# YuePanEdward/MULLS

Hardware: AMD Instinct MI355X
Metric: scan-pair registrations/sec (64-beam ~120k pts, 20 ICP iters); dT vs ref (higher is better)
Workload: dtype f32

## Files before the change

include/mulls_hip.h:

```cpp
#ifndef MULLS_HIP_H
#define MULLS_HIP_H

#include <stddef.h>
#include <stdint.h>

#ifdef __cplusplus
extern "C" {
#endif

#define MULLS_NCLASS 6
#define MULLS_POINT_BYTES 48

enum mulls_class
{
	MULLS_GROUND = 0,
	MULLS_PILLAR = 1,
	MULLS_FACADE = 2,
	MULLS_BEAM = 3,
	MULLS_ROOF = 4,
	MULLS_VERTEX = 5
};

enum mulls_error
{
	MULLS_OK = 0,
	MULLS_E_INVALID = -100,
	MULLS_E_HIP = -101,
	MULLS_E_NO_DEVICE = -102,
	MULLS_E_UNSUPPORTED = -103,
	MULLS_E_IO = -104,
	MULLS_E_NOMEM = -105
};

typedef struct mulls_cloud
{
	const void *pts;
	uint32_t n;
	uint32_t stride;
} mulls_cloud;

typedef struct mulls_pair
{
	mulls_cloud tgt[MULLS_NCLASS];
	mulls_cloud src[MULLS_NCLASS];
	mulls_cloud src_down[MULLS_NCLASS];
	double tgt_bound[6];
	double init_guess[16];
} mulls_pair;

typedef struct mulls_params
{
	int32_t max_iter_num;
	float dis_thre_unit;
	float converge_translation;
	float converge_rotation_d;
	float dis_thre_min;
	float dis_thre_update_rate;
	char used_feature_type[8];
	char weight_strategy[8];
	float z_xy_balanced_ratio;
	float pt2pt_residual_window;
	float pt2pl_residual_window;
	float pt2li_residual_window;
	uint8_t apply_intersection_filter;
	uint8_t apply_motion_undistortion;
	uint8_t normal_shooting_on;
	uint8_t use_more_points;
	float normal_bearing;
	uint8_t keep_less_source_points;
	uint8_t faithful;
	uint8_t rejector_strict;
	uint8_t reserved_;
	float sigma_thre;
	float min_neccessary_corr_ratio;
	float max_bearable_rotation_d;
	uint64_t rng_seed;
} mulls_params;

typedef struct mulls_iter_trace
{
	int32_t iter;
	uint32_t ncorr[MULLS_NCLASS];
	uint32_t nsrc[MULLS_NCLASS];
	float thr[MULLS_NCLASS];
	double atpa[36];
	double atpb[6];
	double x[6];
} mulls_iter_trace;

typedef struct mulls_result
{
	int32_t code;
	int32_t iters;
	double T[16];
	double info[36];
	float sigma;
	float confidence;
	uint32_t ncorr[MULLS_NCLASS];
	uint32_t nsrc0[MULLS_NCLASS];
	uint32_t ntgt0[MULLS_NCLASS];
	int32_t singular;
	int32_t cropped;
	double crop_box[6];
	float ms_total;
	mulls_iter_trace *trace;
	int32_t trace_cap;
	int32_t trace_len;
} mulls_result;

typedef struct mulls_profile
{
	double ms_setup;
	double ms_nn;
	double ms_filter;
	double ms_accum;
	double ms_residual;
	int32_t launches_nn;
	int32_t iterations;
	uint64_t nn_pair_evals;
	uint64_t nn_src_pts;
	uint64_t nn_tgt_pts;
	double ms_host_step;
	double ms_host_wait;
	double ms_host_launch;
	uint64_t nn_tgt_unique;
	uint64_t nn_corr_pts;
	double icp_fused_ms[6];
	double icp_search_ms[24];
	double icp_phase_ms[6];
	double ms_stage;
	double ms_stage_pack;
	uint64_t stage_bytes;
} mulls_profile;

typedef struct mulls_ctx mulls_ctx;
typedef struct mulls_batch mulls_batch;

void mulls_default_params(mulls_params *p);

int mulls_create(int device, mulls_ctx **out);
void mulls_destroy(mulls_ctx *ctx);
const char *mulls_last_error(const mulls_ctx *ctx);
int mulls_set_profiling(mulls_ctx *ctx, int on);
int mulls_get_profile(const mulls_ctx *ctx, mulls_profile *out);
int mulls_set_nn_mode(mulls_ctx *ctx, int mode);
enum mulls_option
{
	MULLS_OPT_HOST_STEP = 0,
	MULLS_OPT_FEW_LAUNCHES_MAX_PAIRS = 3,
	MULLS_OPT_SUBBATCHES = 4,
	MULLS_OPT_TWO_STREAMS = 5,
	MULLS_OPT_CERTIFICATES = 6,
	MULLS_OPT_CERT_SLACK_MIN = 7,
	MULLS_OPT_CERT_SLACK_MAX = 8,
	MULLS_OPT_CERT_SLACK_RATE = 9,
	MULLS_OPT_LDS_DEDUP = 10,
	MULLS_OPT_GRID_H0 = 11,
	MULLS_OPT_BM_H0 = 12,
	MULLS_OPT_LEAN_STAGING = 13,
	MULLS_OPT_DEBUG_STOP = 14,
	MULLS_OPT_DEBUG_TICK = 15,
	MULLS_OPT_SPLIT_MIN_PAIRS = 16,
	MULLS_OPT_SPLIT_MAX_PAIRS = 17,
	MULLS_OPT_FUSED_TGT_SETUP = 18,
	MULLS_OPT_STAGGER = 19,
	MULLS_OPT_STEP_LAUNCH_MAX_PAIRS = 20,
	MULLS_OPT_MIXED_TIERS = 21,
	MULLS_OPT_BIG_EARLY_SETS = 22,
	MULLS_OPT_KCERT = 23,
	MULLS_OPT_KCERT_MIN = 24,
	MULLS_OPT_ACCUM_WAVE_MIN_TRIPS = 25,
	MULLS_OPT_FIRST_DIRECT = 26,
	MULLS_OPT_SUM_STEP = 27,
	MULLS_OPT_COUNT = 28
};
int mulls_set_option(mulls_ctx *ctx, int option, double value);
int mulls_get_option(const mulls_ctx *ctx, int option, double *value);
void *mulls_stream(mulls_ctx *ctx);

int mulls_icp(mulls_ctx *ctx, const mulls_pair *pair, const mulls_params *params, mulls_result *result);

int mulls_icp_batch(mulls_ctx *ctx, const mulls_pair *pairs, int n, const mulls_params *params, mulls_result *results);

int mulls_icp_batch_sharded(mulls_ctx *const *ctxs, int n_ctx, const mulls_pair *pairs, int n, const mulls_params *params, mulls_result *results);

typedef struct mulls_pipe mulls_pipe;
int mulls_pipe_create(int device, int depth, mulls_pipe **out);
void mulls_pipe_destroy(mulls_pipe *pipe);
int mulls_pipe_depth(const mulls_pipe *pipe);
mulls_ctx *mulls_pipe_ctx(mulls_pipe *pipe, int lane);
int mulls_pipe_set_option(mulls_pipe *pipe, int option, double value);
int mulls_icp_batch_begin(mulls_pipe *pipe, const mulls_pair *pairs, int n, const mulls_params *params, mulls_result *results);
int mulls_icp_batch_end(mulls_pipe *pipe, int ticket);

void mulls_pack_results(const mulls_result *results, int n, double *table);

int mulls_batch_create(mulls_ctx *ctx, const mulls_pair *pairs, int n, mulls_batch **out);
int mulls_batch_run(mulls_ctx *ctx, mulls_batch *batch, const mulls_params *params, mulls_result *results);
void mulls_batch_destroy(mulls_ctx *ctx, mulls_batch *batch);


int mulls_icp_3dof_ground(mulls_ctx *ctx, const mulls_pair *pair, const mulls_params *params, mulls_result *result);
int mulls_icp_3dof_ground_batch(mulls_ctx *ctx, const mulls_pair *pairs, int n, const mulls_params *params, mulls_result *results);

int mulls_icp_4dof_global(mulls_ctx *ctx, const mulls_pair *pair, float heading_step_d, const double station[3], int max_iter_num,
						  float dis_thre_unit, float converge_translation, float converge_rotation_d, float dis_thre_min,
						  float dis_thre_update_rate, float max_bearable_rotation_d, mulls_result *result, int *success,
						  float *best_heading_d);

typedef struct mulls_map mulls_map;

typedef struct mulls_map_params
{
	float local_map_radius;
	int max_num_pts;
	int kept_vertex_num;
	float last_frame_reliable_radius;
	int map_based_dynamic_removal_on;
	char used_feature_type[8];
	float dynamic_removal_center_radius;
	float dynamic_dist_thre_min;
	float dynamic_dist_thre_max;
	float near_dist_thre;
	int recalculate_feature_on;
	uint64_t rng_seed;
	int tree_mode;
	char tree_used[8];
	double tree_box[6];
} mulls_map_params;

typedef struct mulls_map_report
{
	uint32_t n[6];
	uint32_t frame_n[6];
	int feature_point_num;
	int dynamic_removal_ran;
	double local_bound[6];
	double bound[6];
	float ms_total;
} mulls_map_report;

void mulls_map_default_params(mulls_map_params *p);
int mulls_map_create(mulls_ctx *ctx, mulls_map **out);
void mulls_map_destroy(mulls_ctx *ctx, mulls_map *map);
int mulls_map_set(mulls_ctx *ctx, mulls_map *map, const mulls_cloud clouds[6], const double pose_lo[16]);
int mulls_map_update(mulls_ctx *ctx, mulls_map *map, const mulls_cloud frame_down[6], const double frame_pose_lo[16],
					 const mulls_map_params *params, mulls_map_report *report);
int mulls_map_cloud(mulls_ctx *ctx, const mulls_map *map, int cls, mulls_cloud *out);
int mulls_map_pose(mulls_ctx *ctx, const mulls_map *map, double pose_lo[16]);
int mulls_map_download(mulls_ctx *ctx, const mulls_map *map, int cls, void *pts, uint32_t cap, uint32_t *n);
int mulls_map_frame_download(mulls_ctx *ctx, const mulls_map *map, int cls, void *pts, uint32_t cap, uint32_t *n);

int mulls_io_read_kitti_bin(const char *path, void *pts, uint32_t cap, uint32_t *n);
int mulls_io_read_pcd(const char *path, void *pts, uint32_t cap, uint32_t *n);
int mulls_io_write_pcd(const char *path, const void *pts, uint32_t n, uint32_t stride, int as_binary);
int mulls_io_write_pose(const char *path, const double T[16], int append);


typedef struct mulls_ground_params
{
	int32_t min_grid_pt_num;
	float grid_resolution;
	float max_height_difference;
	float neighbor_height_diff;
	float max_ground_height;
	int32_t ground_random_down_rate;
	int32_t ground_random_down_down_rate;
	int32_t nonground_random_down_rate;
	int32_t reliable_neighbor_grid_num_thre;
	int32_t estimate_ground_normal_method;
	int32_t distance_weight_downsampling_method;
	float standard_distance;
	uint8_t fixed_num_downsampling;
	uint8_t apply_grid_wise_outlier_filter;
	uint8_t reserved_[2];
	int32_t down_ground_fixed_num;
	float intensity_thre;
	float outlier_std_scale;
	float normal_estimation_radius;
	uint32_t reserved2_;
	uint64_t rng_seed;
} mulls_ground_params;

void mulls_ground_default_params(mulls_ground_params *p);

int mulls_ground_filter(mulls_ctx *ctx, const void *pts, uint32_t n, uint32_t stride, const mulls_ground_params *params, void *ground, uint32_t cap_ground,
						void *ground_down, uint32_t cap_ground_down, void *unground, uint32_t cap_unground, uint32_t n_out[3]);


typedef struct mulls_classify_params
{
	float neighbor_searching_radius;
	int32_t neighbor_k;
	int32_t neigh_k_min;
	int32_t pca_down_rate;
	float edge_thre, planar_thre;
	float edge_thre_down, planar_thre_down;
	int32_t extract_vertex_points_method;
	float curvature_thre;
	float vertex_curvature_non_max_radius;
	float linear_vertical_sin_high_thre, linear_vertical_sin_low_thre;
	float planar_vertical_sin_high_thre, planar_vertical_sin_low_thre;
	uint8_t fixed_num_downsampling;
	uint8_t sharpen_with_nms;
	uint8_t use_distance_adaptive_pca;
	uint8_t reserved_;
	int32_t pillar_down_fixed_num, facade_down_fixed_num, beam_down_fixed_num, roof_down_fixed_num, unground_down_fixed_num;
	float beam_height_max, roof_height_min;
	float feature_pts_ratio_guess;
	uint64_t rng_seed;
} mulls_classify_params;

void mulls_classify_default_params(mulls_classify_params *p);

enum mulls_classify_cloud
{
	MULLS_CL_PILLAR = 0,
	MULLS_CL_BEAM = 1,
	MULLS_CL_FACADE = 2,
	MULLS_CL_ROOF = 3,
	MULLS_CL_PILLAR_DOWN = 4,
	MULLS_CL_BEAM_DOWN = 5,
	MULLS_CL_FACADE_DOWN = 6,
	MULLS_CL_ROOF_DOWN = 7,
	MULLS_CL_VERTEX = 8,
	MULLS_CL_COUNT = 9
};
// ... 67 lines not shown
```

mulls_amd/abi.py:

```python
import ctypes as C

import numpy as np

NCLASS = 6
POINT_BYTES = 48
GROUND, PILLAR, FACADE, BEAM, ROOF, VERTEX = range(6)
CLASS_NAMES = ("ground", "pillar", "facade", "beam", "roof", "vertex")

MULLS_OK = 0
MULLS_E_INVALID = -100
MULLS_E_HIP = -101
MULLS_E_NO_DEVICE = -102
MULLS_E_UNSUPPORTED = -103
MULLS_E_IO = -104
MULLS_E_NOMEM = -105

(OPT_HOST_STEP, _OPT_RESERVED_1, _OPT_RESERVED_2, OPT_FEW_LAUNCHES_MAX_PAIRS, OPT_SUBBATCHES, OPT_TWO_STREAMS, OPT_CERTIFICATES, OPT_CERT_SLACK_MIN,
 OPT_CERT_SLACK_MAX, OPT_CERT_SLACK_RATE, OPT_LDS_DEDUP, OPT_GRID_H0, OPT_BM_H0, OPT_LEAN_STAGING, OPT_DEBUG_STOP, OPT_DEBUG_TICK, OPT_SPLIT_MIN_PAIRS, OPT_SPLIT_MAX_PAIRS,
 OPT_FUSED_TGT_SETUP, OPT_STAGGER, OPT_STEP_LAUNCH_MAX_PAIRS, OPT_MIXED_TIERS, OPT_BIG_EARLY_SETS, OPT_KCERT, OPT_KCERT_MIN, OPT_ACCUM_WAVE_MIN_TRIPS, OPT_FIRST_DIRECT, OPT_SUM_STEP, OPT_COUNT) = range(29)

POINT_DTYPE = np.dtype(
    {
        "names": ["x", "y", "z", "nx", "ny", "nz", "intensity", "curvature"],
        "formats": [np.float32] * 8,
        "offsets": [0, 4, 8, 16, 20, 24, 32, 36],
        "itemsize": POINT_BYTES,
    }
)


class Cloud(C.Structure):
    _fields_ = [("pts", C.c_void_p), ("n", C.c_uint32), ("stride", C.c_uint32)]


class Pair(C.Structure):
    _fields_ = [
        ("tgt", Cloud * NCLASS),
        ("src", Cloud * NCLASS),
        ("src_down", Cloud * NCLASS),
        ("tgt_bound", C.c_double * 6),
        ("init_guess", C.c_double * 16),
    ]


class Params(C.Structure):
    _fields_ = [
        ("max_iter_num", C.c_int32),
        ("dis_thre_unit", C.c_float),
        ("converge_translation", C.c_float),
        ("converge_rotation_d", C.c_float),
        ("dis_thre_min", C.c_float),
        ("dis_thre_update_rate", C.c_float),
        ("used_feature_type", C.c_char * 8),
        ("weight_strategy", C.c_char * 8),
        ("z_xy_balanced_ratio", C.c_float),
        ("pt2pt_residual_window", C.c_float),
        ("pt2pl_residual_window", C.c_float),
        ("pt2li_residual_window", C.c_float),
        ("apply_intersection_filter", C.c_uint8),
        ("apply_motion_undistortion", C.c_uint8),
        ("normal_shooting_on", C.c_uint8),
        ("use_more_points", C.c_uint8),
        ("normal_bearing", C.c_float),
        ("keep_less_source_points", C.c_uint8),
        ("faithful", C.c_uint8),
        ("rejector_strict", C.c_uint8),
        ("reserved_", C.c_uint8),
        ("sigma_thre", C.c_float),
        ("min_neccessary_corr_ratio", C.c_float),
        ("max_bearable_rotation_d", C.c_float),
        ("rng_seed", C.c_uint64),
    ]


class IterTrace(C.Structure):
    _fields_ = [
        ("iter", C.c_int32),
        ("ncorr", C.c_uint32 * NCLASS),
        ("nsrc", C.c_uint32 * NCLASS),
        ("thr", C.c_float * NCLASS),
        ("atpa", C.c_double * 36),
        ("atpb", C.c_double * 6),
        ("x", C.c_double * 6),
    ]


class Result(C.Structure):
    _fields_ = [
        ("code", C.c_int32),
        ("iters", C.c_int32),
        ("T", C.c_double * 16),
        ("info", C.c_double * 36),
        ("sigma", C.c_float),
        ("confidence", C.c_float),
        ("ncorr", C.c_uint32 * NCLASS),
        ("nsrc0", C.c_uint32 * NCLASS),
        ("ntgt0", C.c_uint32 * NCLASS),
        ("singular", C.c_int32),
        ("cropped", C.c_int32),
        ("crop_box", C.c_double * 6),
        ("ms_total", C.c_float),
        ("trace", C.POINTER(IterTrace)),
        ("trace_cap", C.c_int32),
        ("trace_len", C.c_int32),
    ]

    def T_matrix(self):
        return np.array(self.T[:], dtype=np.float64).reshape(4, 4).T.copy()

    def info_matrix(self):
        return np.array(self.info[:], dtype=np.float64).reshape(6, 6).T.copy()



class MapParams(C.Structure):
    _fields_ = [
        ("local_map_radius", C.c_float),
        ("max_num_pts", C.c_int32),
        ("kept_vertex_num", C.c_int32),
        ("last_frame_reliable_radius", C.c_float),
        ("map_based_dynamic_removal_on", C.c_int32),
        ("used_feature_type", C.c_char * 8),
        ("dynamic_removal_center_radius", C.c_float),
        ("dynamic_dist_thre_min", C.c_float),
        ("dynamic_dist_thre_max", C.c_float),
        ("near_dist_thre", C.c_float),
        ("recalculate_feature_on", C.c_int32),
        ("rng_seed", C.c_uint64),
        ("tree_mode", C.c_int32),
        ("tree_used", C.c_char * 8),
        ("tree_box", C.c_double * 6),
    ]


class MapReport(C.Structure):
    _fields_ = [
        ("n", C.c_uint32 * NCLASS),
        ("frame_n", C.c_uint32 * NCLASS),
        ("feature_point_num", C.c_int32),
        ("dynamic_removal_ran", C.c_int32),
        ("local_bound", C.c_double * 6),
        ("bound", C.c_double * 6),
        ("ms_total", C.c_float),
    ]


def map_params(**kw):
    p = MapParams()
    p.local_map_radius, p.max_num_pts, p.kept_vertex_num, p.last_frame_reliable_radius = 80.0, 20000, 800, 60.0
    p.map_based_dynamic_removal_on = 0
    p.used_feature_type = b"111110"
    p.dynamic_removal_center_radius, p.dynamic_dist_thre_min, p.dynamic_dist_thre_max, p.near_dist_thre = 30.0, 0.3, 3.0, 0.03
    p.recalculate_feature_on, p.rng_seed, p.tree_mode, p.tree_used = 0, 0, 0, b"000000"
    for k, v in kw.items():
        if k == "tree_box":
            for i in range(6):
                p.tree_box[i] = float(v[i])
        elif k in ("used_feature_type", "tree_used"):
            setattr(p, k, v.encode() if isinstance(v, str) else v)
        else:
            setattr(p, k, v)
    return p


def colmajor16(M):
    return (C.c_double * 16)(*np.asarray(M, dtype=np.float64).T.reshape(-1))

class GroundParams(C.Structure):
    _fields_ = [
        ("min_grid_pt_num", C.c_int32),
        ("grid_resolution", C.c_float),
        ("max_height_difference", C.c_float),
# ... 312 lines not shown
```

mulls_amd/csrc/accum.h:

```cpp
#pragma once
#include "device_util.h"

namespace
{
__device__ __forceinline__ float w_dist_adaptive(float dist, int iter_num)
{
	const float unit_dist = 30.0f, b_min = 0.7f, b_max = 1.3f, b_step = 0.05f;
	float t = b_min + b_step * iter_num;
	float b_current = (t < b_max) ? t : b_max;
	float temp = (float)(b_current + (1.0 - b_current) * dist / unit_dist);
	temp = (float)((temp > 0.01) ? (double)temp : 0.01);
	return temp;
}
__device__ __forceinline__ float w_intensity(float i1, float i2)
{
	float ratio = fabsf(i1 - i2) / 255.0f;
	return (float)exp(-1.0 * ratio);
}
__device__ __forceinline__ float w_residual(float res, float thre)
{
	return (res > thre) ? ((2 * res * thre + (1 * 1 - 2 * 1) * (thre * thre)) / res / res) : 1.0f;
}
__device__ __forceinline__ int metric_of(int cls) { return (cls == 1 || cls == 3) ? 1 : (cls == 5 ? 2 : 0); }
}
// ... 165 lines not shown
			ACC(1, 3.0);
		}
		return;
	}

	if (metric == 0)
	{
		float ntx = N.x, nty = N.y, ntz = N.z;
		float a = ntz * py - nty * pz;
		float b = ntx * pz - ntz * px;
		float c = nty * px - ntx * py;
		float dd = ntx * qx + nty * qy + ntz * qz - ntx * px - nty * py - ntz * pz;
		const float w = wpre ? *wpre : corr_weight(A, 0, P, Q, N, wi);
		wdg = w;
		ACC(0, w * ntx * ntx);
		ACC(1, w * ntx * nty);
		ACC(2, w * ntx * ntz);
		ACC(3, w * a * ntx);
		ACC(4, w * b * ntx);
		ACC(5, w * c * ntx);
		ACC(6, w * nty * nty);
		ACC(7, w * nty * ntz);
		ACC(8, w * a * nty);
		ACC(9, w * b * nty);
		ACC(10, w * c * nty);
		ACC(11, w * ntz * ntz);
		ACC(12, w * a * ntz);
		ACC(13, w * b * ntz);
		ACC(14, w * c * ntz);
		ACC(15, w * a * a);
		ACC(16, w * a * b);
		ACC(17, w * a * c);
		ACC(18, w * b * b);
		ACC(19, w * b * c);
		ACC(20, w * c * c);
		ACC(21, w * dd * ntx);
		ACC(22, w * dd * nty);
		ACC(23, w * dd * ntz);
		ACC(24, w * dd * a);
		ACC(25, w * dd * b);
		ACC(26, w * dd * c);
	}
	else if (metric == 1)
	{
		const float wx = wpre ? *wpre : corr_weight(A, 1, P, Q, N, wi);
		float vx = N.x, vy = N.y, vz = N.z;
		float dx = px - qx, dy = py - qy, dz = pz - qz;
		double A[3][6], bv[3];
		A[0][0] = 0;
		A[0][1] = -vz;
		A[0][2] = vy;
		A[0][3] = vy * py + vz * pz;
		A[0][4] = -vy * px;
		A[0][5] = -vz * px;
		A[1][0] = vz;
		A[1][1] = 0;
		A[1][2] = -vx;
		A[1][3] = -vx * py;
		A[1][4] = vz * pz + vx * px;
		A[1][5] = -vz * py;
		A[2][0] = -vy;
		A[2][1] = vx;
		A[2][2] = 0;
		A[2][3] = -vx * pz;
		A[2][4] = -vy * pz;
		A[2][5] = vx * px + vy * py;
		bv[0] = -vy * dz + vz * dy;
		bv[1] = -vz * dx + vx * dz;
		bv[2] = -vx * dy + vy * dx;
		wdg = wx;
		const double sw = (double)sqrtf(wx);
		for (int r = 0; r < 3; r++)
		{
			for (int c = 0; c < 6; c++)
				A[r][c] = sw * A[r][c];
			bv[r] = sw * bv[r];
		}
		int k = 0;
#pragma unroll
		for (int j = 0; j < 6; j++)
#pragma unroll
			for (int c = j; c < 6; c++)
				{
					ACC(k, (A[0][j] * A[0][c] + A[1][j] * A[1][c]) + A[2][j] * A[2][c]);
					k++;
				}
#pragma unroll
		for (int j = 0; j < 6; j++)
			ACC(21 + j, (A[0][j] * bv[0] + A[1][j] * bv[1]) + A[2][j] * bv[2]);
	}
	else
	{
		float dx = px - qx, dy = py - qy, dz = pz - qz;
		const float wx = wpre ? *wpre : corr_weight(A, 2, P, Q, N, wi);
		const float wy = wx, wz = wx;
		if (!faithful)
			wdg = wx;
		ACC(0, wx);
		ACC(4, wx * pz);
		ACC(5, (-wx * py));
		ACC(6, wy);
		ACC(8, (-wy * pz));
		ACC(10, wy * px);
		ACC(11, wz);
		ACC(12, wz * py);
		ACC(13, (-wz * px));
		ACC(15, wy * pz * pz + wz * py * py);
		ACC(16, (-wz * px * py));
		ACC(17, (-wy * px * pz));
		ACC(18, wx * pz * pz + wz * px * px);
		ACC(19, (-wx * py * pz));
		ACC(20, wx * py * py + wy * px * px);
		ACC(21, (-wx * dx));
		ACC(22, (-wy * dy));
		ACC(23, (-wz * dz));
		ACC(24, wy * pz * dy - wz * py * dz);
		ACC(25, wz * px * dz - wx * pz * dx);
		ACC(26, wx * py * dx - wy * px * dy);
	}
}
#undef ACC

#define MULLS_ACC_LANES 1024
#define MULLS_RED_BYTES ((size_t)27 * MULLS_ACC_LANES * sizeof(float))
#define MULLS_RED_BYTES_HALF ((size_t)14 * MULLS_ACC_LANES * sizeof(float))

namespace
{
template <int CTRL>
__device__ __forceinline__ double dpp_add_f64(double v)
{
	const unsigned long long b = (unsigned long long)__double_as_longlong(v);
	const uint32_t lo = (uint32_t)__builtin_amdgcn_update_dpp(0, (int)(uint32_t)b, CTRL, 0xf, 0xf, false);
	const uint32_t hi = (uint32_t)__builtin_amdgcn_update_dpp(0, (int)(uint32_t)(b >> 32), CTRL, 0xf, 0xf, false);
	return v + __longlong_as_double((long long)(((unsigned long long)hi << 32) | lo));
}
template <int CTRL, int ROWS>
__device__ __forceinline__ double dpp_add_f64_rows(double v)
{
	const unsigned long long b = (unsigned long long)__double_as_longlong(v);
	const uint32_t lo = (uint32_t)__builtin_amdgcn_update_dpp(0, (int)(uint32_t)b, CTRL, ROWS, 0xf, false);
	const uint32_t hi = (uint32_t)__builtin_amdgcn_update_dpp(0, (int)(uint32_t)(b >> 32), CTRL, ROWS, 0xf, false);
	return v + __longlong_as_double((long long)(((unsigned long long)hi << 32) | lo));
}
__device__ __forceinline__ double readlane_f64(double v, int lane)
{
	const unsigned long long b = (unsigned long long)__double_as_longlong(v);
	const uint32_t lo = (uint32_t)__builtin_amdgcn_readlane((int)(uint32_t)b, lane);
	const uint32_t hi = (uint32_t)__builtin_amdgcn_readlane((int)(uint32_t)(b >> 32), lane);
	return __longlong_as_double((long long)(((unsigned long long)hi << 32) | lo));
}
}

template <typename TS, int T0, int NT, int MODE = 0, int LANES = MULLS_ACC_LANES>
__device__ __forceinline__ void slot_terms(const AccumCtx &A, const double *x, bool valid, const float4 P, const float4 Q, const float4 N, float wi, float &wdg, TS *R)
{
	static_assert(sizeof(TS) * NT * LANES <= MULLS_RED_BYTES, "the term buffer holds NT terms of LANES slots");
	TS t[NT];
#pragma unroll
	for (int k = 0; k < NT; k++)
		t[k] = (TS)0;
	if (valid)
		point_terms<TS, T0, NT, MODE>(A, x, P, Q, N, wi, wdg, t);
#pragma unroll
	for (int k = 0; k < NT; k++)
		R[k * LANES + threadIdx.x] = t[k];
}
template <typename TS, int T0, int NT, int MODE = 0, int LANES = MULLS_ACC_LANES>
__device__ __forceinline__ void reduce_terms(const TS *R, double *part)
{
	const int lane = threadIdx.x & 63, wave = threadIdx.x >> 6;
#pragma unroll
	for (int k0 = 0; k0 < NT; k0 += LANES / 64)
	{
		const int k = k0 + wave;
		if (k < NT)
		{
			const TS *r = R + k * LANES;
			double sum = (double)r[lane];
#pragma unroll
			for (int i = 1; i < LANES / 64; i++)
				sum += (double)r[lane + 64 * i];
			sum = dpp_add_f64<0xB1>(sum);
			sum = dpp_add_f64<0x4E>(sum);
			sum = dpp_add_f64<0x141>(sum);
			sum = dpp_add_f64<0x140>(sum);
			const double r0 = readlane_f64(sum, 0), r1 = readlane_f64(sum, 16), r2 = readlane_f64(sum, 32), r3 = readlane_f64(sum, 48);
			if (lane == 0)
				part[MODE == 1 ? li_term(T0 + k) : T0 + k] = (r0 + r1) + (r2 + r3);
		}
	}
}

template <bool HALF = false, int LANES = MULLS_ACC_LANES>
__device__ __forceinline__ void trip_sum_regs(const AccumCtx &A, const double *x, bool valid, const float4 P, const float4 Q, const float4 N, float &wdg, void *R,
											   double *part)
{
	const float wi = (valid && A.inten_w && !A.residual_pass) ? point_wi(P, Q) : 1.0f;
	if (A.residual_pass)
	{
		__syncthreads();
		slot_terms<double, 0, 2, 0, LANES>(A, x, valid, P, Q, N, wi, wdg, static_cast<double *>(R));
		__syncthreads();
		reduce_terms<double, 0, 2, 0, LANES>(static_cast<const double *>(R), part);
		if (threadIdx.x >= 2 && threadIdx.x < MULLS_NTERM)
			part[threadIdx.x] = 0.0;
	}
	else if (A.li_diag)
	{
		__syncthreads();
		if (threadIdx.x < 21 && li_slot((int)threadIdx.x) < 0)
			part[threadIdx.x] = 0.0;
		if (HALF)
		{
			slot_terms<double, 0, 6, 1, LANES>(A, x, valid, P, Q, N, wi, wdg, static_cast<double *>(R));
			__syncthreads();
			reduce_terms<double, 0, 6, 1, LANES>(static_cast<const double *>(R), part);
			__syncthreads();
			slot_terms<double, 6, 6, 1, LANES>(A, x, valid, P, Q, N, wi, wdg, static_cast<double *>(R));
			__syncthreads();
			reduce_terms<double, 6, 6, 1, LANES>(static_cast<const double *>(R), part);
		}
		else
		{
			slot_terms<double, 0, 12, 1, LANES>(A, x, valid, P, Q, N, wi, wdg, static_cast<double *>(R));
			__syncthreads();
			reduce_terms<double, 0, 12, 1, LANES>(static_cast<const double *>(R), part);
		}
	}
	else if (A.metric == 1 && HALF)
	{
		__syncthreads();
		slot_terms<double, 0, 7, 0, LANES>(A, x, valid, P, Q, N, wi, wdg, static_cast<double *>(R));
		__syncthreads();
		reduce_terms<double, 0, 7, 0, LANES>(static_cast<const double *>(R), part);
		__syncthreads();
		slot_terms<double, 7, 7, 0, LANES>(A, x, valid, P, Q, N, wi, wdg, static_cast<double *>(R));
		__syncthreads();
		reduce_terms<double, 7, 7, 0, LANES>(static_cast<const double *>(R), part);
		__syncthreads();
		slot_terms<double, 14, 7, 0, LANES>(A, x, valid, P, Q, N, wi, wdg, static_cast<double *>(R));
		__syncthreads();
		reduce_terms<double, 14, 7, 0, LANES>(static_cast<const double *>(R), part);
		__syncthreads();
		slot_terms<double, 21, 6, 0, LANES>(A, x, valid, P, Q, N, wi, wdg, static_cast<double *>(R));
		__syncthreads();
		reduce_terms<double, 21, 6, 0, LANES>(static_cast<const double *>(R), part);
	}
	else if (A.metric == 1)
	{
		__syncthreads();
		slot_terms<double, 0, 13, 0, LANES>(A, x, valid, P, Q, N, wi, wdg, static_cast<double *>(R));
		__syncthreads();
		reduce_terms<double, 0, 13, 0, LANES>(static_cast<const double *>(R), part);
		__syncthreads();
		slot_terms<double, 13, 13, 0, LANES>(A, x, valid, P, Q, N, wi, wdg, static_cast<double *>(R));
		__syncthreads();
		reduce_terms<double, 13, 13, 0, LANES>(static_cast<const double *>(R), part);
		__syncthreads();
		slot_terms<double, 26, 1, 0, LANES>(A, x, valid, P, Q, N, wi, wdg, static_cast<double *>(R));
		__syncthreads();
		reduce_terms<double, 26, 1, 0, LANES>(static_cast<const double *>(R), part);
	}
	else if (HALF)
	{
		__syncthreads();
		slot_terms<float, 0, 14, 0, LANES>(A, x, valid, P, Q, N, wi, wdg, static_cast<float *>(R));
		__syncthreads();
		reduce_terms<float, 0, 14, 0, LANES>(static_cast<const float *>(R), part);
		__syncthreads();
		slot_terms<float, 14, 13, 0, LANES>(A, x, valid, P, Q, N, wi, wdg, static_cast<float *>(R));
		__syncthreads();
		reduce_terms<float, 14, 13, 0, LANES>(static_cast<const float *>(R), part);
	}
	else
	{
		__syncthreads();
		slot_terms<float, 0, 27, 0, LANES>(A, x, valid, P, Q, N, wi, wdg, static_cast<float *>(R));
		__syncthreads();
		reduce_terms<float, 0, 27, 0, LANES>(static_cast<const float *>(R), part);
	}
	__syncthreads();
}

template <bool HALF = false, int LANES = MULLS_ACC_LANES>
__device__ __forceinline__ void trip_sum(const AccumCtx &A, const double *x, const CloudDesc &d, uint32_t trip0, const float4 *__restrict__ spos,
										  const float4 *__restrict__ mq, const uint8_t *__restrict__ flag, float *__restrict__ wd, void *R, double *part)
{
	const uint32_t s = trip0 + threadIdx.x;
	bool valid = false;
	float4 P = make_float4(0.0f, 0.0f, 0.0f, 0.0f), Q = P, N = P;
	float w = 0.0f, w0 = 0.0f;
	uint32_t g = 0;
	if (s < d.src_n)
	{
		g = d.src_off + s;
		const uint32_t f = flag[g];
		P = spos[g], Q = mq[2u * g], N = mq[2u * g + 1u];
		w = w0 = wd[g];
		valid = (f & (MULLS_F_ALIVE | MULLS_F_VALID)) == (MULLS_F_ALIVE | MULLS_F_VALID);
	}
	trip_sum_regs<HALF, LANES>(A, x, valid, P, Q, N, w, R, part);
	if (valid && __float_as_uint(w) != __float_as_uint(w0))
		wd[g] = w;
}

// ... 45 lines not shown
```

mulls_amd/csrc/batch.cpp:

```cpp
#include "batch.h"

namespace mulls_drv
{
void rows12(const double colmajor[16], double out[12])
{
	for (int r = 0; r < 3; r++)
		for (int c = 0; c < 4; c++)
			out[r * 4 + c] = colmajor[r + 4 * c];
}


void fill_crop_box(const RunParams &rp, const double tgt_bound[6], const uint32_t keys[6], mulls_result &R)
{
	R.cropped = rp.crop ? 1 : 0;
	for (int k = 0; k < 3 && rp.crop; k++)
	{
		const uint32_t kmin = keys[k], kmax = keys[3 + k];
		const bool none = kmin == 0xffffffffu && kmax == 0u;
		const double mmin = none ? 1.7976931348623157e308 : (double)ord_to_float(kmin);
		const double mmax = none ? -1.7976931348623157e308 : (double)ord_to_float(kmax);
		const double b1min = tgt_bound[k], b1max = tgt_bound[3 + k];
		const float pad = 1.0f;
		R.crop_box[k] = ((b1min > mmin) ? b1min : mmin) - pad;
		R.crop_box[3 + k] = ((b1max < mmax) ? b1max : mmax) + pad;
	}
}

int check_params(mulls_ctx *ctx, const mulls_params *P)
{
	if (!P)
		return MULLS_E_INVALID;
	if (std::strlen(P->used_feature_type) < 6 || std::strlen(P->weight_strategy) < 4)
	{
		ctx->err = "used_feature_type needs 6 characters and weight_strategy 4";
		return MULLS_E_INVALID;
	}
	return MULLS_OK;
}

void init_cert(const mulls_ctx *ctx, RunParams &rp)
{
	rp.cert = ctx->opt[MULLS_OPT_CERTIFICATES] != 0.0 ? 1u : 0u;
	rp.cert_slack_min = (float)ctx->opt[MULLS_OPT_CERT_SLACK_MIN];
	rp.cert_slack_max = (float)ctx->opt[MULLS_OPT_CERT_SLACK_MAX];
	rp.cert_slack_rate = (float)ctx->opt[MULLS_OPT_CERT_SLACK_RATE];
	rp.kcert = rp.cert && ctx->opt[MULLS_OPT_KCERT] != 0.0 ? 1u : 0u;
	rp.kcert_min = (uint32_t)ctx->opt[MULLS_OPT_KCERT_MIN];
}

int subbatch_count(const mulls_ctx *ctx, int n)
{
	int nsub = n >= 2048 ? 2 : 1;
	if (ctx->opt[MULLS_OPT_SUBBATCHES] >= 1.0)
		nsub = std::max(1, std::min(2, (int)ctx->opt[MULLS_OPT_SUBBATCHES]));
	return n < 2 ? 1 : nsub;
}

bool option_value_ok(int option, double *value)
{
	const double v = *value;
	if (!(v == v) || v > 1.0e15 || v < -1.0e15)
		return false;
	switch (option)
	{
	case MULLS_OPT_STAGGER:
		if (v < 0.0 || v > 65536.0)
			return false;
		*value = (double)((uint64_t)v & ~(uint64_t)255);
		return true;
	case MULLS_OPT_GRID_H0:
	case MULLS_OPT_BM_H0:
		return v >= 0.0 && v <= 1.0e4;
	case MULLS_OPT_CERT_SLACK_MIN:
	case MULLS_OPT_CERT_SLACK_MAX:
		return v >= 0.0 && v <= 1.0e3;
	case MULLS_OPT_CERT_SLACK_RATE:
		return v >= 0.0 && v <= 1.0e3;
	case MULLS_OPT_DEBUG_TICK:
		return v >= 0.0 && v <= 4294967295.0;
	default:
		return v >= 0.0 && v <= 2147483647.0;
	}
}

}
int SegCopier::flush(hipStream_t st)
{
	using namespace mulls;
	size_t total = 0;
	for (const Pending &h : host)
		total += (h.bytes + 255u) & ~(size_t)255;
	bool direct = false;
	for (const Pending &h : host)
		direct = direct || (h.bytes & 3u) || ((uintptr_t)h.dst & 15u) || h.bytes > 0xfffffff0ull;
	for (const CopySeg &g : segs)
		direct = direct || (g.bytes & 3u) || (g.dst & 15ull) || (g.src & 15ull);
	if (direct)
	{
		for (const CopySeg &g : segs)
			HIPCHK(ctx, hipMemcpyAsync((void *)(uintptr_t)g.dst, (const void *)(uintptr_t)g.src, g.bytes, hipMemcpyDeviceToDevice, st));
		for (const Pending &h : host)
			HIPCHK(ctx, hipMemcpyAsync(h.dst, h.src, h.bytes, hipMemcpyHostToDevice, st));
		segs.clear(), host.clear();
		return MULLS_OK;
	}
	if (total > ctx->mail_cap)
	{
		HIPCHK(ctx, hipStreamSynchronize(st));
		if (ctx->mail_h)
			(void)hipHostFree(ctx->mail_h);
		ctx->mail_h = nullptr, ctx->mail_cap = 0;
		const size_t want = std::max<size_t>(total + total / 2, (size_t)1 << 20);
		HIPCHK(ctx, hipHostMalloc((void **)&ctx->mail_h, want, hipHostMallocMapped));
		ctx->mail_cap = want;
	}
	unsigned char *mail_d = nullptr;
	if (total)
		HIPCHK(ctx, hipHostGetDevicePointer((void **)&mail_d, ctx->mail_h, 0));
	size_t off = 0;
	for (const Pending &h : host)
	{
		std::memcpy(ctx->mail_h + off, h.src, h.bytes);
		segs.push_back({(unsigned long long)(uintptr_t)h.dst, (unsigned long long)(uintptr_t)(mail_d + off), (uint32_t)h.bytes, 0u});
		off += (h.bytes + 255u) & ~(size_t)255;
	}
	if (!segs.empty())
	{
		launch_copy_segs(st, segs.data(), (uint32_t)segs.size());
		HIPCHK(ctx, hipGetLastError());
	}
	segs.clear(), host.clear();
	return MULLS_OK;
}
namespace mulls_drv
{
void options_init(mulls_ctx *ctx)
{
	double *o = ctx->opt;
	o[MULLS_OPT_HOST_STEP] = 0, o[MULLS_OPT_FEW_LAUNCHES_MAX_PAIRS] = 640;
	o[MULLS_OPT_SUBBATCHES] = 0, o[MULLS_OPT_TWO_STREAMS] = 0, o[MULLS_OPT_CERTIFICATES] = 1;
	o[MULLS_OPT_CERT_SLACK_MIN] = 0.02, o[MULLS_OPT_CERT_SLACK_MAX] = 0.10, o[MULLS_OPT_CERT_SLACK_RATE] = 1.0;
	o[MULLS_OPT_SPLIT_MIN_PAIRS] = 96, o[MULLS_OPT_SPLIT_MAX_PAIRS] = 1 << 30, o[MULLS_OPT_FUSED_TGT_SETUP] = 1, o[MULLS_OPT_STAGGER] = 4352, o[MULLS_OPT_STEP_LAUNCH_MAX_PAIRS] = 640, o[MULLS_OPT_LDS_DEDUP] = 1, o[MULLS_OPT_GRID_H0] = 0, o[MULLS_OPT_BM_H0] = 0, o[MULLS_OPT_LEAN_STAGING] = 0, o[MULLS_OPT_DEBUG_STOP] = 0, o[MULLS_OPT_DEBUG_TICK] = 0, o[MULLS_OPT_MIXED_TIERS] = 1, o[MULLS_OPT_BIG_EARLY_SETS] = 5, o[MULLS_OPT_KCERT] = 1, o[MULLS_OPT_KCERT_MIN] = 64, o[MULLS_OPT_ACCUM_WAVE_MIN_TRIPS] = 768;
	o[MULLS_OPT_FIRST_DIRECT] = 1;
	o[MULLS_OPT_SUM_STEP] = 1;
	static const struct
	{
		const char *name;
		int opt;
	} env[] = {{"MULLS_HOST_STEP", MULLS_OPT_HOST_STEP}, {"MULLS_FEW_LAUNCHES_MAX_PAIRS", MULLS_OPT_FEW_LAUNCHES_MAX_PAIRS}, {"MULLS_SUBBATCHES", MULLS_OPT_SUBBATCHES}, {"MULLS_TWO_STREAMS", MULLS_OPT_TWO_STREAMS},
			   {"MULLS_CERTIFICATES", MULLS_OPT_CERTIFICATES}, {"MULLS_LDS_DEDUP", MULLS_OPT_LDS_DEDUP}, {"MULLS_GRID_H0", MULLS_OPT_GRID_H0}, {"MULLS_BM_H0", MULLS_OPT_BM_H0},
			   {"MULLS_LEAN_STAGING", MULLS_OPT_LEAN_STAGING}, {"MULLS_FUSED_TGT_SETUP", MULLS_OPT_FUSED_TGT_SETUP}, {"MULLS_STAGGER", MULLS_OPT_STAGGER}, {"MULLS_STEP_LAUNCH_MAX_PAIRS", MULLS_OPT_STEP_LAUNCH_MAX_PAIRS}, {"MULLS_SPLIT_MIN_PAIRS", MULLS_OPT_SPLIT_MIN_PAIRS}, {"MULLS_SPLIT_MAX_PAIRS", MULLS_OPT_SPLIT_MAX_PAIRS}, {"MULLS_DEBUG_STOP", MULLS_OPT_DEBUG_STOP}, {"MULLS_DEBUG_TICK", MULLS_OPT_DEBUG_TICK}, {"MULLS_MIXED_TIERS", MULLS_OPT_MIXED_TIERS}, {"MULLS_BIG_EARLY_SETS", MULLS_OPT_BIG_EARLY_SETS}, {"MULLS_KCERT", MULLS_OPT_KCERT}, {"MULLS_KCERT_MIN", MULLS_OPT_KCERT_MIN}, {"MULLS_ACCUM_WAVE_MIN_TRIPS", MULLS_OPT_ACCUM_WAVE_MIN_TRIPS}, {"MULLS_FIRST_DIRECT", MULLS_OPT_FIRST_DIRECT}, {"MULLS_SUM_STEP", MULLS_OPT_SUM_STEP}};
	for (const auto &e : env)
		if (const char *v = std::getenv(e.name))
		{
			double x = std::strtod(v, nullptr);
			if (option_value_ok(e.opt, &x))
				o[e.opt] = x;
		}
	if (std::getenv("MULLS_NO_CERT"))
		o[MULLS_OPT_CERTIFICATES] = 0;
	if (std::getenv("MULLS_NO_LDS_DEDUP"))
		o[MULLS_OPT_LDS_DEDUP] = 0;
	if (const char *e = std::getenv("MULLS_CERT_SLACK"))
	{
		float a = 0, b = 0, c = 0;
		if (std::sscanf(e, "%f,%f,%f", &a, &b, &c) == 3 && a >= 0.0f && b >= a && c >= 0.0f)
			o[MULLS_OPT_CERT_SLACK_MIN] = a, o[MULLS_OPT_CERT_SLACK_MAX] = b, o[MULLS_OPT_CERT_SLACK_RATE] = c;
	}
}

uint32_t lds_dedup_max_pts()
{
	const long room = 160L * 1024L - 64L - (long)MULLS_LDS_CELL_RESERVE - (long)MULLS_LDS_QCHUNK * 16L - (long)MULLS_LDS_AUX - 2L * (4096L + 8L);
	return (uint32_t)((room / 18L) & ~7L);
}

void assign_tiers(mulls_batch *B, const uint8_t used[MULLS_NC], int mode)
{
	B->lclouds_h.clear();
	B->tier_mode = mode;
	uint32_t n_used = 0;
	for (int c = 0; c < MULLS_NC; c++)
		n_used += used[c] ? 1u : 0u;
	const uint32_t s_max = lds_dedup_max_pts();
	for (int p = 0; p < B->n; p++)
	{
		uint64_t src_small = 0, src_big = 0;
		for (int c = 0; c < MULLS_NC && mode == 3; c++)
		{
			const CloudDesc &d = B->descs_h[(size_t)p * MULLS_NC + c];
			if (used[c])
				((d.tgt_n0 <= s_max && d.src_cap <= MULLS_SMALL_SRC_MAX) ? src_small : src_big) += d.src_cap;
		}
		const bool all_big = src_big >= 4u * src_small && src_big > 0;
		uint32_t rank = 0;
		for (int c = 0; c < MULLS_NC; c++)
		{
			CloudDesc &d = B->descs_h[(size_t)p * MULLS_NC + c];
			uint32_t t = (uint32_t)mode;
			if (mode == 3)
			{
				if (used[c])
					t = (d.tgt_n0 <= s_max && d.src_cap <= MULLS_SMALL_SRC_MAX && !all_big) ? MULLS_TIER_LDS : MULLS_TIER_BM;
				else
					t = d.tgt_n0 <= MULLS_LDS_MAXPTS ? MULLS_TIER_LDS : MULLS_TIER_BM;
			}
			d.tier = t;
			d.grid_slot = (uint32_t)p * n_used + rank;
			if (t == MULLS_TIER_BM)
			{
				d.grid_slot = used[c] ? (uint32_t)B->lclouds_h.size() : 0u;
				if (used[c])
					B->lclouds_h.push_back((uint32_t)p * MULLS_NC + (uint32_t)c);
			}
			rank += used[c] ? 1u : 0u;
		}
	}
}

void build_jobs(mulls_batch *B, const mulls_params *P, int nsub, int mode)
{
	std::string key(P->used_feature_type, 6);
	key += (char)('0' + nsub);
	key += (char)('a' + mode);
	if (key == B->jobs_key)
		return;
	uint8_t used[MULLS_NC];
	for (int c = 0; c < MULLS_NC; c++)
		used[c] = P->used_feature_type[c] == '1';
	assign_tiers(B, used, mode);
	B->nsub = nsub;
	B->jobs_h.clear();
	for (int p = 0; p < B->n; p++)
		for (int c = 0; c < MULLS_NC; c++)
		{
			CloudDesc &d = B->descs_h[p * MULLS_NC + c];
			d.job_begin = (uint32_t)B->jobs_h.size();
			if (P->used_feature_type[c] == '1')
				for (uint32_t s = 0; s < d.src_cap; s += MULLS_SRC_PER_BLOCK)
				{
					Job j = {(uint32_t)p, (uint32_t)c, s, 0};
					B->jobs_h.push_back(j);
				}
			d.job_end = (uint32_t)B->jobs_h.size();
		}
	B->cjobs_h.clear();
	for (int p = 0; p < B->n; p++)
		for (int c = 0; c < MULLS_NC; c++)
		{
			const CloudDesc &d = B->descs_h[p * MULLS_NC + c];
			if (used[c] && d.src_cap > 0 && d.tier == MULLS_TIER_LDS)
			{
				Job j = {(uint32_t)p, (uint32_t)c, 0u, d.src_cap};
				B->cjobs_h.push_back(j);
			}
		}
	uint32_t max_src_cap = 0;
	for (const Job &j : B->cjobs_h)
		max_src_cap = std::max(max_src_cap, j.count);
	if (mode == 2 && ((B->cjobs_h.size() < 512 && max_src_cap > 4096u) || max_src_cap > 65534u))
	{
		B->cjobs_h.clear();
		for (int p = 0; p < B->n; p++)
			for (int c = 0; c < MULLS_NC; c++)
				if (P->used_feature_type[c] == '1')
					for (uint32_t s = 0; s < B->descs_h[p * MULLS_NC + c].src_cap; s += MULLS_SRC_PER_BLOCK)
					{
						Job j = {(uint32_t)p, (uint32_t)c, s, MULLS_SRC_PER_BLOCK};
						B->cjobs_h.push_back(j);
					}
	}
	B->bjobs_h.clear();
	B->fjobs_h.clear();
	B->ejobs_h.clear();
	bool any_class_job = false;
	for (int p = 0; p < B->n; p++)
		for (int c = 0; c < MULLS_NC; c++)
		{
			const CloudDesc &d = B->descs_h[p * MULLS_NC + c];
			if (!used[c] || d.src_cap == 0 || d.tier != MULLS_TIER_BM)
				continue;
			const bool whole = mode == 3 && d.src_cap <= MULLS_BIG_CLASS_MAX;
			if (whole)
			{
				Job j = {(uint32_t)p, (uint32_t)c, 0u, d.src_cap | MULLS_JOB_CLASS};
				B->bjobs_h.push_back(j);
				any_class_job = true;
			}
			for (uint32_t s = 0; s < d.src_cap; s += MULLS_SRC_PER_BLOCK)
			{
				Job j = {(uint32_t)p, (uint32_t)c, s, MULLS_SRC_PER_BLOCK};
				B->ejobs_h.push_back(j);
				if (!whole)
				{
					B->bjobs_h.push_back(j);
					B->fjobs_h.push_back(j);
				}
			}
		}
	if (!any_class_job)
		B->ejobs_h.clear();
	B->cjobs_dev_h = B->cjobs_h;
	{
		auto first_of = [&](uint32_t pair) {
// ... 612 lines not shown
```

mulls_amd/csrc/device_types.h:

```cpp
#pragma once
#include <stdint.h>

#define MULLS_NC 6
#define MULLS_NTERM 27
#define MULLS_BLOCK 256
#define MULLS_SRC_PER_THREAD 2
#define MULLS_SRC_PER_BLOCK (MULLS_BLOCK * MULLS_SRC_PER_THREAD)
#define MULLS_NN_BLOCK 128
#define MULLS_NN_PTS 4
#define MULLS_TILE 2048

#define MULLS_MAXCELLS 65536u
#define MULLS_BM_MAXWORDS (1u << 22)
#define MULLS_BM_TOTALWORDS (1u << 28)
#define MULLS_BM_H0 0.25f
#define MULLS_LDS_BLOCK 1024
#define MULLS_LDS_MAXPTS 9728u
#define MULLS_ACC_BLOCK 128
#define MULLS_LDS_QCHUNK 1024u
#define MULLS_LDS_AUX (320u + 2u * MULLS_LDS_QCHUNK)
#define MULLS_CERT_BLOCK 512
#define MULLS_CERT_SMALL 64u
#define MULLS_CERT_SMALL_LOCKSTEP 512u
#define MULLS_LDS_CELL_RESERVE 9216
#ifndef MULLS_LDS_GROUP
#define MULLS_LDS_GROUP 8u
#endif
#define MULLS_BIG_CLOUD 16384u
#define MULLS_BIG_SRC_SIDE 0x100u
#define MULLS_SEG 4096u
#define MULLS_GRID_GROUP 16u
#define MULLS_BIG_BLOCK 512
#define MULLS_BIG_CLASS_MAX (3u * MULLS_BIG_BLOCK)
#define MULLS_JOB_CLASS 0x80000000u
#define MULLS_SMALL_SRC_MAX 4096u
#define MULLS_TIER_BRUTE 0u
#define MULLS_TIER_BM 1u
#define MULLS_TIER_LDS 2u
#define MULLS_GRID_H0 1.3f

#define MULLS_F_ALIVE 1u
#define MULLS_F_VALID 2u

struct CloudDesc
{
	uint32_t src_stage;
	uint32_t tgt_stage;
	uint32_t src_n0;
	uint32_t tgt_n0;
	uint32_t src_off;
	uint32_t tgt_off;
	uint32_t src_n;
	uint32_t tgt_n;
	uint32_t alive_cur;
	uint32_t alive_next;
	uint32_t n_matched;
	uint32_t valid_next;
	uint32_t n_valid;
	uint32_t job_begin;
	uint32_t job_end;
	uint32_t sd_stage;
	uint32_t sd_n0;
	uint32_t src_cap;
	uint32_t big_slot;
	uint32_t src_big_slot;
	uint32_t n_search;
	uint32_t stage_fmt;
	uint32_t tier;
	uint32_t grid_slot;
};
#define MULLS_STAGE_AOS48 0u
#define MULLS_STAGE_PACK32 1u
#define MULLS_STAGE_PACK28 2u

struct GridDesc
{
	float ox, oy, oz;
	float inv_h, h;
	uint32_t nx, ny, nz;
	uint32_t ncell;
	uint32_t cell_off;
	uint32_t wpr;
	uint32_t nocc;
};

struct PairState
{
	double T[12];
	double x[6];
	float thr[MULLS_NC];
	int32_t iter;
	int32_t active;
	int32_t want_residual;
	int32_t pad_[3];
};

struct PairSetup
{
	double guess[12];
	double tgt_bound[6];
	double inv_q[4];
	double inv_t[4];
};

#define MULLS_NTERM_PAD 28
struct PairOut
{
	double sums[MULLS_NC][MULLS_NTERM_PAD];
	double comb[MULLS_NTERM_PAD];
	uint32_t n_valid[MULLS_NC];
	uint32_t n_alive[MULLS_NC];
	uint32_t src_n[MULLS_NC];
	uint32_t tgt_n[MULLS_NC];
	uint32_t bbox[6];
	uint32_t pad_[2];
};

struct IcpOut
{
	double T[16];
	double info[36];
	double sigma2;
	unsigned long long src_pts, tgt_pts, corr_pts;
	float ratio;
	int32_t code, iters, singular, trace_len;
	uint32_t ncorr[MULLS_NC], nsrc0[MULLS_NC], ntgt0[MULLS_NC], bbox[6];
	uint32_t pad_;
	unsigned long long tgt_job_pts, pair_evals;
};

struct Job
{
	uint32_t pair;
	uint32_t cls;
	uint32_t start;
	uint32_t count;
};

#define MULLS_COPY_SEGS 24
struct CopySeg
{
	unsigned long long dst, src;
	uint32_t bytes, pad_;
};
struct CopyArgs
{
	CopySeg seg[MULLS_COPY_SEGS];
};

struct RunParams
{
	uint8_t used[MULLS_NC];
	uint8_t w_balance, w_resid, w_dist, w_inten;
	uint8_t crop;
	uint8_t undistort;
	uint8_t normal_shooting;
	uint8_t faithful;
	uint8_t rej_strict;
	float z_xy_ratio;
	float win_pt, win_pl, win_li;
	uint8_t force_class_w;
	uint8_t bm_auto;
	float class_w_value;
	double cos_bearing;
	int32_t resid_from_iter;
	uint32_t debug_stop;
	uint32_t cell_stride;
	uint32_t grid_maxcells;
	float grid_h0;
	float bm_h0;
	uint32_t bm_maxwords;
	uint32_t bm_stride;
	uint32_t pull_comb;
	uint32_t lds_dedup;
	uint32_t tick_base;
	uint32_t cert;
	float cert_slack_min, cert_slack_max, cert_slack_rate;
	uint32_t kcert;
	uint32_t kcert_min;
	uint4 *cand;
	const float4 *tgt_stage;
	const uint16_t *tgt_map;
	unsigned long long *dbg_ticks;
};
```

mulls_amd/csrc/k_reduce.hip:

```cpp
#include "device_util.h"
#include "accum.h"
#include "solve_wave.h"

template <int LANES, int MIN_WG>
__global__ __launch_bounds__(LANES, MIN_WG) void k_accum(const uint32_t *__restrict__ leaders, const Job *__restrict__ jobs, const CloudDesc *__restrict__ descs,
														 const PairState *__restrict__ states, RunParams rp, const float4 *__restrict__ spos,
														 const float4 *__restrict__ mq, const uint8_t *__restrict__ flag, float *__restrict__ wd,
														 double *__restrict__ partial)
{
	extern __shared__ __attribute__((aligned(16))) unsigned char lds_raw[];
	__shared__ double part[MULLS_NTERM_PAD];
	const uint32_t job_idx = leaders[xcd_job(blockIdx.x, gridDim.x)];
	const Job job = jobs[job_idx];
	const PairState &ps = states[job.pair];
	if (!ps.active && !ps.want_residual)
		return;
	const CloudDesc *pd = descs + job.pair * MULLS_NC;
	const bool residual_pass = ps.want_residual != 0;
	int cnt[MULLS_NC];
	for (int c = 0; c < MULLS_NC; c++)
		cnt[c] = (int)(class_called(rp, pd[c], c) ? pd[c].valid_next : pd[c].n_valid);
	const AccumCtx A = accum_ctx(rp, job.cls, ps.iter, residual_pass, class_weight(rp, job.cls, residual_pass, cnt));
	trip_sum<true, LANES>(A, ps.x, pd[job.cls], job.start, spos, mq, flag, wd, lds_raw, part);
	if (threadIdx.x < MULLS_NTERM)
		partial[(size_t)job_idx * MULLS_NTERM + threadIdx.x] = part[threadIdx.x];
}

namespace
{
template <typename TS, int W0, int WIN, int MODE, int METRIC, int A0>
__device__ __forceinline__ void add_window(const AccumCtx &A, const double *x, const float4 P, const float4 Q, const float4 N, float wi, float &w, double *acc, const float *wpre)
{
	TS t[WIN];
#pragma unroll
	for (int k = 0; k < WIN; k++)
		t[k] = (TS)0;
	point_terms<TS, W0, WIN, MODE, METRIC>(A, x, P, Q, N, wi, w, t, wpre);
#pragma unroll
	for (int k = 0; k < WIN; k++)
		acc[W0 - A0 + k] += (double)t[k];
}
#ifndef MULLS_ACCW_WIN
#define MULLS_ACCW_WIN 9
#endif
#ifndef MULLS_ACCW_WIN_D
#define MULLS_ACCW_WIN_D 12
#endif
template <typename TS, int W0, int REM, int MODE, int METRIC, int A0>
__device__ __forceinline__ void add_windows(const AccumCtx &A, const double *x, const float4 P, const float4 Q, const float4 N, float wi, float &w, double *acc, const float *wpre)
{
	constexpr int WMAX = sizeof(TS) == 8 ? MULLS_ACCW_WIN_D : MULLS_ACCW_WIN;
	constexpr int WIN = REM < WMAX ? REM : WMAX;
	add_window<TS, W0, WIN, MODE, METRIC, A0>(A, x, P, Q, N, wi, w, acc, wpre);
	if constexpr (REM > WIN)
		add_windows<TS, W0 + WIN, REM - WIN, MODE, METRIC, A0>(A, x, P, Q, N, wi, w, acc, wpre);
}
template <typename TS, int NT, int MODE, int METRIC, int T0, int NTW>
__device__ __forceinline__ void wave_trip(const AccumCtx &A, const double *x, const CloudDesc &d, uint32_t trip0, const float4 *__restrict__ spos, const float4 *__restrict__ mq,
										   const uint8_t *__restrict__ flag, float *__restrict__ wd, double *__restrict__ out, bool owner)
{
	const uint32_t lane = threadIdx.x & 63u;
	const uint32_t src_n = d.src_n, src_off = d.src_off;
	const uint32_t n_here = min(src_n - trip0, (uint32_t)MULLS_ACC_LANES), iters = (n_here + 63u) >> 6;
	const uint32_t last = src_off + src_n - 1u;
	struct Rec
	{
		uint32_t f;
		float4 P, Q;
		float3 N;
		float w;
	};
	const bool need_w = A.residual_pass, writes_w = !A.residual_pass && (METRIC != 2 || !A.faithful);
	auto load = [&](uint32_t i) {
		Rec r;
		const uint32_t g = min(src_off + trip0 + lane + 64u * i, last);
		r.f = flag[g];
		r.P = spos[g], r.Q = mq[2u * g], r.N = *reinterpret_cast<const float3 *>(mq + 2u * g + 1u);
		r.w = need_w ? wd[g] : 0.0f;
		return r;
	};
	double acc[NTW];
#pragma unroll
	for (int k = 0; k < NTW; k++)
		acc[k] = -0.0;
#define MULLS_PIN_REC(r) asm volatile("" : "+v"((r).f), "+v"((r).P.x), "+v"((r).Q.x), "+v"((r).N.x), "+v"((r).w))
#if MULLS_ACCW_PREFETCH
	Rec cur = load(0);
#endif
	for (uint32_t i = 0; i < iters; i++)
	{
#if MULLS_ACCW_PREFETCH
		MULLS_PIN_REC(cur);
		Rec nxt = cur;
		if (i + 1u < iters)
			nxt = load(i + 1u);
#else
		Rec cur = load(i);
		MULLS_PIN_REC(cur);
#endif
		const uint32_t s = trip0 + lane + 64u * i;
		const bool valid = s < src_n && (cur.f & (MULLS_F_ALIVE | MULLS_F_VALID)) == (MULLS_F_ALIVE | MULLS_F_VALID);
		if (valid)
		{
			float w = cur.w;
			const float4 N4 = make_float4(cur.N.x, cur.N.y, cur.N.z, 0.0f);
			const float wi = (A.inten_w && !A.residual_pass) ? point_wi(cur.P, cur.Q) : 1.0f;
			const float wpre = A.residual_pass ? 0.0f : corr_weight(A, METRIC, cur.P, cur.Q, N4, wi);
			add_windows<TS, T0, NTW, MODE, METRIC, T0>(A, x, cur.P, cur.Q, N4, wi, w, acc, A.residual_pass ? nullptr : &wpre);
			if (owner && writes_w)
				wd[src_off + s] = w;
		}
#if MULLS_ACCW_PREFETCH
		cur = nxt;
#endif
	}
	if (NTW == NT && lane < MULLS_NTERM)
	{
		const bool has = MODE == 1 ? li_slot((int)lane) >= 0 : (int)lane < NT;
		if (!has)
			out[lane] = 0.0;
	}
#pragma unroll
	for (int k = 0; k < NTW; k++)
	{
		double sum = acc[k];
		sum = dpp_add_f64<0xB1>(sum);
		sum = dpp_add_f64<0x4E>(sum);
		sum = dpp_add_f64<0x141>(sum);
		sum = dpp_add_f64<0x140>(sum);
		sum = dpp_add_f64_rows<0x142, 0xa>(sum);
		sum = dpp_add_f64_rows<0x143, 0xc>(sum);
		acc[k] = sum;
	}
	if (lane == 63u)
	{
#pragma unroll
		for (int k = 0; k < NTW; k++)
			out[MODE == 1 ? li_term(T0 + k) : T0 + k] = acc[k];
	}
}
}

#ifndef MULLS_ACCW_SPLIT
#define MULLS_ACCW_SPLIT 1
#endif
#ifndef MULLS_ACCW_PREFETCH
#define MULLS_ACCW_PREFETCH 0
#endif
#ifndef MULLS_ACCW_OCC
#define MULLS_ACCW_OCC 4
#endif
#define MULLS_ACCW_WAVES 4
__global__ __launch_bounds__(64 * MULLS_ACCW_WAVES, MULLS_ACCW_OCC) void k_accum_wave(const uint32_t *__restrict__ leaders, uint32_t n_trips, const Job *__restrict__ jobs,
																					   const CloudDesc *__restrict__ descs, const PairState *__restrict__ states, RunParams rp,
																					   const float4 *__restrict__ spos, const float4 *__restrict__ mq, const uint8_t *__restrict__ flag,
																					   float *__restrict__ wd, double *__restrict__ partial)
{
	const uint32_t wave = threadIdx.x >> 6, part = wave % MULLS_ACCW_SPLIT;
	const uint32_t trip = blockIdx.x * (MULLS_ACCW_WAVES / MULLS_ACCW_SPLIT) + wave / MULLS_ACCW_SPLIT;
	if (trip >= n_trips)
		return;
	const uint32_t job_idx = leaders[trip];
	const Job job = jobs[job_idx];
	const PairState &ps = states[job.pair];
	if (!ps.active && !ps.want_residual)
		return;
	const CloudDesc *pd = descs + job.pair * MULLS_NC;
	const bool residual_pass = ps.want_residual != 0;
	int cnt[MULLS_NC];
	for (int c = 0; c < MULLS_NC; c++)
		cnt[c] = (int)(class_called(rp, pd[c], c) ? pd[c].valid_next : pd[c].n_valid);
	const AccumCtx A = accum_ctx(rp, job.cls, ps.iter, residual_pass, class_weight(rp, job.cls, residual_pass, cnt));
	const CloudDesc &d = pd[job.cls];
	double *out = partial + (size_t)job_idx * MULLS_NTERM;
	if (d.src_n <= job.start)
	{
		if (part == 0u && (threadIdx.x & 63u) < MULLS_NTERM)
			out[threadIdx.x & 63u] = 0.0;
		return;
	}
	if (residual_pass || A.metric == 1)
	{
		if (part)
			return;
		if (!residual_pass)
			wave_trip<double, 12, 1, 1, 0, 12>(A, ps.x, d, job.start, spos, mq, flag, wd, out, true);
		else if (A.metric == 0)
			wave_trip<double, 2, 0, 0, 0, 2>(A, ps.x, d, job.start, spos, mq, flag, wd, out, true);
		else if (A.metric == 1)
			wave_trip<double, 2, 0, 1, 0, 2>(A, ps.x, d, job.start, spos, mq, flag, wd, out, true);
		else
			wave_trip<double, 2, 0, 2, 0, 2>(A, ps.x, d, job.start, spos, mq, flag, wd, out, true);
	}
#if MULLS_ACCW_SPLIT == 2
	else if (A.metric == 0)
	{
		if (part == 0u)
			wave_trip<float, 27, 0, 0, 0, 14>(A, ps.x, d, job.start, spos, mq, flag, wd, out, true);
		else
			wave_trip<float, 27, 0, 0, 14, 13>(A, ps.x, d, job.start, spos, mq, flag, wd, out, false);
	}
	else
	{
		if (part == 0u)
			wave_trip<float, 27, 0, 2, 0, 14>(A, ps.x, d, job.start, spos, mq, flag, wd, out, true);
		else
			wave_trip<float, 27, 0, 2, 14, 13>(A, ps.x, d, job.start, spos, mq, flag, wd, out, false);
	}
#else
	else if (A.metric == 0)
		wave_trip<float, 27, 0, 0, 0, 27>(A, ps.x, d, job.start, spos, mq, flag, wd, out, true);
	else
		wave_trip<float, 27, 0, 2, 0, 27>(A, ps.x, d, job.start, spos, mq, flag, wd, out, true);
#endif
}

namespace
{
struct FinishLds
{
	double sums[MULLS_NC][MULLS_NTERM_PAD], comb[MULLS_NTERM_PAD];
	uint32_t cnt[32];
};
__device__ __forceinline__ void finish_pair(CloudDesc *pd, const PairState &ps, const RunParams &rp, const double *__restrict__ partial,
											 PairOut &o, const uint32_t *__restrict__ pair_bbox, FinishLds *M = nullptr)
{
	if (threadIdx.x >= 192 && threadIdx.x < 198)
	{
		const uint32_t v = pair_bbox[threadIdx.x - 192];
		o.bbox[threadIdx.x - 192] = v;
		if (M)
			M->cnt[24 + threadIdx.x - 192] = v;
	}
	if (threadIdx.x < MULLS_NC * MULLS_NTERM)
	{
		const int c = threadIdx.x / MULLS_NTERM, t = threadIdx.x % MULLS_NTERM;
		if (rp.used[c])
		{
			constexpr uint32_t STEP = MULLS_ACC_LANES / MULLS_SRC_PER_BLOCK;
			double sum = 0.0;
			uint32_t j = pd[c].job_begin;
			const uint32_t je = pd[c].job_end;
			for (; j + 32u * STEP <= je; j += 32u * STEP)
			{
				double v[32];
#pragma unroll
				for (uint32_t k = 0; k < 32u; k++)
					v[k] = partial[(size_t)(j + k * STEP) * MULLS_NTERM + t];
#pragma unroll
				for (uint32_t k = 0; k < 32u; k++)
					sum += v[k];
			}
			for (; j + 16u * STEP <= je; j += 16u * STEP)
			{
				double v[16];
#pragma unroll
				for (uint32_t k = 0; k < 16u; k++)
					v[k] = partial[(size_t)(j + k * STEP) * MULLS_NTERM + t];
#pragma unroll
				for (uint32_t k = 0; k < 16u; k++)
					sum += v[k];
			}
			for (; j < je; j += STEP)
				sum += partial[(size_t)j * MULLS_NTERM + t];
			o.sums[c][t] = sum;
			if (M)
				M->sums[c][t] = sum;
		}
	}
	__syncthreads();
	if (rp.pull_comb && threadIdx.x >= 64 && threadIdx.x < 64 + MULLS_NTERM)
	{
		if (M)
		{
			combine_rows(rp, ps.want_residual != 0, M->sums, M->comb, (int)threadIdx.x - 64);
			o.comb[threadIdx.x - 64] = M->comb[threadIdx.x - 64];
		}
		else
			combine_rows(rp, ps.want_residual != 0, o.sums, o.comb, (int)threadIdx.x - 64);
	}
	if (threadIdx.x < MULLS_NC)
	{
		const int c = threadIdx.x;
		CloudDesc &d = pd[c];
		if (ps.active)
		{
			if (class_called(rp, d, c))
			{
				d.n_valid = d.valid_next;
				d.alive_cur = d.alive_next;
			}
			d.alive_next = 0;
			d.valid_next = 0;
			d.n_matched = 0;
		}
		o.n_valid[c] = d.n_valid;
		o.n_alive[c] = d.alive_cur;
		o.src_n[c] = d.src_n;
		o.tgt_n[c] = d.tgt_n;
		if (M)
			M->cnt[c] = d.n_valid, M->cnt[6 + c] = d.alive_cur, M->cnt[12 + c] = d.src_n, M->cnt[18 + c] = d.tgt_n;
	}
}
__device__ __forceinline__ void finish_pair_wave(CloudDesc *pd, const PairState &ps, const RunParams &rp, const double *__restrict__ partial, PairOut &o,
												  const uint32_t *__restrict__ pair_bbox, FinishLds &M)
{
	const uint32_t l = threadIdx.x;
	constexpr uint32_t STEP = MULLS_ACC_LANES / MULLS_SRC_PER_BLOCK;
	if (l >= 32u && l < 38u)
	{
		const uint32_t v = pair_bbox[l - 32u];
		o.bbox[l - 32u] = v;
		M.cnt[24u + l - 32u] = v;
	}
	double sum[3] = {0.0, 0.0, 0.0};
	uint32_t j[3], je[3];
	bool on[3];
#pragma unroll
	for (int u = 0; u < 3; u++)
	{
		const uint32_t idx = l + 64u * (uint32_t)u, c = idx / MULLS_NTERM;
		on[u] = idx < MULLS_NC * MULLS_NTERM && rp.used[c < MULLS_NC ? c : 0u];
		j[u] = on[u] ? pd[c].job_begin : 0u;
		je[u] = on[u] ? pd[c].job_end : 0u;
	}
	double v[3][4];
#pragma unroll
	for (int u = 0; u < 3; u++)
	{
		const uint32_t t = (l + 64u * (uint32_t)u) % MULLS_NTERM;
#pragma unroll
		for (uint32_t k = 0; k < 4u; k++)
			v[u][k] = j[u] + k * STEP < je[u] ? partial[(size_t)(j[u] + k * STEP) * MULLS_NTERM + t] : 0.0;
// ... 598 lines not shown
```

mulls_amd/csrc/k_search.hip:

```cpp
#include "device_util.h"
#include "lds_tier.h"
#include "big_tier.h"

template <int NPTS>
__device__ __forceinline__ void nn_scan_group(const float *__restrict__ X, const float *__restrict__ Y, const float *__restrict__ Z, uint32_t j,
											   const float (&px)[NPTS], const float (&py)[NPTS], const float (&pz)[NPTS], float (&best)[NPTS],
											   uint32_t (&grp)[NPTS], uint32_t gidx)
{
	const float4 x0 = *reinterpret_cast<const float4 *>(X + j), x1 = *reinterpret_cast<const float4 *>(X + j + 4);
	const float4 y0 = *reinterpret_cast<const float4 *>(Y + j), y1 = *reinterpret_cast<const float4 *>(Y + j + 4);
	const float4 z0 = *reinterpret_cast<const float4 *>(Z + j), z1 = *reinterpret_cast<const float4 *>(Z + j + 4);
	const float tx[8] = {x0.x, x0.y, x0.z, x0.w, x1.x, x1.y, x1.z, x1.w};
	const float ty[8] = {y0.x, y0.y, y0.z, y0.w, y1.x, y1.y, y1.z, y1.w};
	const float tz[8] = {z0.x, z0.y, z0.z, z0.w, z1.x, z1.y, z1.z, z1.w};
#pragma unroll
	for (int u = 0; u < NPTS; u++)
	{
		float dd[8];
#pragma unroll
		for (int v = 0; v < 8; v++)
		{
			const float dx = px[u] - tx[v], dy = py[u] - ty[v], dz = pz[u] - tz[v];
			dd[v] = (dx * dx + dy * dy) + dz * dz;
		}
// ... 47 lines not shown
	}
	if (!called)
		return;

	const float INF = __builtin_inff();
	float best[MULLS_NN_PTS];
	uint32_t grp[MULLS_NN_PTS];
#pragma unroll
	for (int u = 0; u < MULLS_NN_PTS; u++)
	{
		best[u] = INF;
		grp[u] = 0;
	}

	for (uint32_t base = 0; base < tgt_n; base += MULLS_TILE)
	{
		const uint32_t nt = min((uint32_t)MULLS_TILE, tgt_n - base);
		const uint32_t nt8 = (nt + 7u) & ~7u;
		__syncthreads();
		for (uint32_t k = threadIdx.x; k < nt8; k += MULLS_NN_BLOCK)
		{
			const float4 t = (k < nt) ? tpos[d.tgt_off + base + k] : make_float4(INF, INF, INF, 0.0f);
			tileX[k] = t.x;
			tileY[k] = t.y;
			tileZ[k] = t.z;
		}
		__syncthreads();
		for (uint32_t j = 0; j < nt8; j += 8)
			nn_scan_group<MULLS_NN_PTS>(tileX, tileY, tileZ, j, px, py, pz, best, grp, base + j);
	}

	const float r = 2.5f * ps.thr[job.cls];
	const double maxd = (double)r;
	const double max_dist_sqr = maxd * maxd;
	const bool gate = alive_cur >= 500u;
	const unsigned long long key_hi = (unsigned long long)(0xffffffffu - (rp.tick_base + (uint32_t)ps.iter)) << 32;
	uint32_t matched_cnt = 0;
#pragma unroll
	for (int u = 0; u < MULLS_NN_PTS; u++)
	{
		if (!alive[u])
			continue;
		int idx = -1;
		for (int v = 7; v >= 0; v--)
		{
			const uint32_t t = grp[u] + v;
			if (t < tgt_n)
			{
				float ddx = px[u] - tp[4 * t], ddy = py[u] - tp[4 * t + 1], ddz = pz[u] - tp[4 * t + 2];
				float dist = (ddx * ddx + ddy * ddy) + ddz * ddz;
				if (dist == best[u])
					idx = (int)t;
			}
		}
		const bool matched = idx >= 0 && !((double)best[u] > max_dist_sqr);
		nn_idx[d.src_off + s[u]] = matched ? idx : -1;
		nn_d2[d.src_off + s[u]] = best[u];
		if (matched)
		{
			matched_cnt++;
			if (gate)
				atomicMin(&winner[d.tgt_off + idx], key_hi | (unsigned long long)s[u]);
		}
	}
	for (int off = 32; off > 0; off >>= 1)
		matched_cnt += __shfl_down(matched_cnt, off);
	if ((threadIdx.x & 63) == 0 && matched_cnt)
		atomicAdd(&d.n_matched, matched_cnt);
}

__global__ __launch_bounds__(MULLS_BIG_BLOCK, 4) void k_cert_big(const Job *__restrict__ jobs, CloudDesc *__restrict__ descs, const PairState *__restrict__ states, RunParams rp,
																 float4 *__restrict__ spos, float4 *__restrict__ snrm, const GridDesc *__restrict__ grids,
																 const unsigned long long *__restrict__ bm, const uint32_t *__restrict__ pf, const uint32_t *__restrict__ cs,
																 const float4 *__restrict__ tsorted, uint8_t *flag, int32_t *__restrict__ nn_idx, float *__restrict__ nn_d2,
																 unsigned long long *__restrict__ winner, uint32_t split, const float4 *__restrict__ tpos,
																 const float4 *__restrict__ tnrm, int32_t *__restrict__ nn_hint, int32_t *__restrict__ match, float *__restrict__ wd,
																 float4 *__restrict__ mq)
{
	__shared__ BigLds<MULLS_BIG_BLOCK * 3> s_big;
	const uint32_t wg = xcd_job(blockIdx.x, gridDim.x);
	const Job job = jobs[wg / split];
	const uint32_t part = wg % split;
	const PairState &ps = states[job.pair];
	if (!ps.active || (rp.normal_shooting && (job.cls == 0 || job.cls == 2 || job.cls == 4)))
		return;
	const uint32_t ci = job.pair * MULLS_NC + job.cls;
	CloudDesc &d = descs[ci];
	const bool class_level = (job.count & MULLS_JOB_CLASS) != 0u;
	const uint32_t cnt = (job.count & ~MULLS_JOB_CLASS) ? (job.count & ~MULLS_JOB_CLASS) : (uint32_t)MULLS_SRC_PER_BLOCK;
	uint32_t q0, q1;
	if (class_level)
	{
		if (part)
			return;
		q0 = 0u, q1 = min(d.src_n, cnt);
	}
	else
	{
		const uint32_t per = cnt / split;
		q0 = job.start + part * per, q1 = min(d.src_n, q0 + per);
		if (q0 >= q1)
			return;
	}
	const GridDesc g = grids[ci];
	const BmGrid B = {bm + g.cell_off, pf + g.cell_off, cs + d.tgt_off + ci};
	cert_big<MULLS_BIG_BLOCK, 3>(s_big, rp, ps, job.cls, q0, q1, class_level, d, g, B, tsorted + d.tgt_off, spos, snrm, flag, nn_idx, nn_d2, winner, tnrm, match, wd, tpos,
								 reinterpret_cast<int2 *>(nn_hint), mq);
}

__global__ __launch_bounds__(MULLS_BLOCK) void k_filter(const Job *__restrict__ jobs, CloudDesc *__restrict__ descs,
														 const PairState *__restrict__ states, RunParams rp,
														 const float4 *__restrict__ snrm, const float4 *__restrict__ tnrm, uint8_t *__restrict__ flag,
														 const int32_t *__restrict__ nn_idx, const float *__restrict__ nn_d2,
														 int32_t *__restrict__ match, float *__restrict__ wd,
														 const unsigned long long *__restrict__ winner, const float4 *__restrict__ tpos,
														 float4 *__restrict__ mq, uint32_t big)
{
	__shared__ uint32_t red4[4];
	const Job job = jobs[xcd_job(blockIdx.x, gridDim.x)];
	const PairState &ps = states[job.pair];
	if (!ps.active)
		return;
	CloudDesc &d = descs[job.pair * MULLS_NC + job.cls];
	if (!class_called(rp, d, job.cls))
		return;
	const float thr = ps.thr[job.cls];
	const FilterCtx F = {d.alive_cur >= 500u, d.n_matched > 0u, job.cls != 5, rp.lds_dedup != 0u && !big, rp.rej_strict != 0, thr * thr, rp.cos_bearing,
						 (unsigned long long)(0xffffffffu - (rp.tick_base + (uint32_t)ps.iter)) << 32, big ? nullptr : rp.tgt_stage, big ? nullptr : rp.tgt_map};
	uint32_t n_alive = 0, n_valid = 0;
#pragma unroll
	for (int u = 0; u < MULLS_SRC_PER_THREAD; u++)
	{
		const uint32_t s = job.start + threadIdx.x + u * MULLS_BLOCK;
		if (s < d.src_n)
			filter_point(F, d, s, snrm, tnrm, flag, nn_idx, nn_d2, match, wd, winner, tpos, mq, n_alive, n_valid);
	}
	const uint32_t ta = block_sum_u32(n_alive, red4);
	const uint32_t tv = block_sum_u32(n_valid, red4);
	if (threadIdx.x == 0)
	{
		if (ta)
			atomicAdd(&d.alive_next, ta);
		if (tv)
			atomicAdd(&d.valid_next, tv);
	}
}


__device__ __forceinline__ bool first_goes_direct(const RunParams &rp, const CloudDesc &d, int cls)
{
	return class_called(rp, d, cls);
}

template <int BLK, int SMALL, bool PARK = false, int FLAT_TRIPS = (BLK == 512 ? 3 : 2)>
__device__ __forceinline__ bool cert_job(CertLds<SMALL> &CL, const RunParams &rp, const PairState &ps, const Job &job, CloudDesc &d, const GridDesc &g, uint32_t *W, float4 *__restrict__ spos,
										  float4 *__restrict__ snrm, const uint32_t *__restrict__ cell_start, const float4 *__restrict__ tsorted, uint8_t *flag,
										  int32_t *__restrict__ nn_idx, float *__restrict__ nn_d2, unsigned long long *__restrict__ winner, const float4 *__restrict__ tnrm,
										  int32_t *__restrict__ match, float *__restrict__ wd, const float4 *__restrict__ tpos, int32_t *__restrict__ nn_hint,
										  float4 *__restrict__ mq, uint32_t *park = nullptr)
{
	const bool flat = rp.lds_dedup != 0u && rp.debug_stop != 9u && job.start == 0u && job.count >= d.src_n && d.src_n <= (uint32_t)(BLK * FLAT_TRIPS) && class_called(rp, d, job.cls);
	return flat ? cert_class_flat<BLK, FLAT_TRIPS, true, SMALL, PARK>(CL, rp, ps, job, d, g, W, spos, snrm, cell_start, tsorted, flag, nn_idx, nn_d2, winner, tnrm, match, wd, tpos, nn_hint, mq, park)
				: cert_class<BLK, true, SMALL>(CL, rp, ps, job, d, g, W, spos, snrm, cell_start, tsorted, flag, nn_idx, nn_d2, winner, tnrm, match, wd, tpos, nn_hint, mq);
}

template <int BLK, int TRIPS = (BLK == 512 ? 3 : 2), int SMALL = MULLS_CERT_SMALL_LOCKSTEP>
__global__ __launch_bounds__(BLK, BLK == 512 ? 8 : 4) void k_cert(const Job *__restrict__ cjobs, CloudDesc *__restrict__ descs,
															const PairState *__restrict__ states, RunParams rp, float4 *__restrict__ spos,
															float4 *__restrict__ snrm, const GridDesc *__restrict__ grids,
															const uint32_t *__restrict__ cell_start, const float4 *__restrict__ tsorted, uint8_t *flag,
															int32_t *__restrict__ nn_idx, float *__restrict__ nn_d2, unsigned long long *__restrict__ winner,
															const float4 *__restrict__ tnrm, int32_t *__restrict__ match, float *__restrict__ wd,
															const float4 *__restrict__ tpos, int32_t *__restrict__ nn_hint, float4 *__restrict__ mq,
															uint32_t *__restrict__ wl, uint32_t *__restrict__ wl_ctr, uint32_t parity)
{
	extern __shared__ __attribute__((aligned(16))) unsigned char lds_raw[];
	uint32_t *W = reinterpret_cast<uint32_t *>(lds_raw);
	if (blockIdx.x == 0 && threadIdx.x == 0)
		wl_ctr[2u * (parity ^ 1u)] = wl_ctr[2u * (parity ^ 1u) + 1u] = 0u;
	const Job job = cjobs[blockIdx.x];
	const PairState &ps = states[job.pair];
	if (!ps.active || (rp.normal_shooting && (job.cls == 0 || job.cls == 2 || job.cls == 4)))
		return;
	CloudDesc &d = descs[job.pair * MULLS_NC + job.cls];
	const GridDesc g = grids[job.pair * MULLS_NC + job.cls];
	__shared__ CertLds<SMALL> s_cert;
	constexpr bool PARK = BLK == 512;
	__shared__ uint32_t s_park[PARK ? 2 * TRIPS * BLK : 1];
	if (!cert_job<BLK, SMALL, PARK, TRIPS>(s_cert, rp, ps, job, d, g, W, spos, snrm, cell_start, tsorted, flag, nn_idx, nn_d2, winner, tnrm, match, wd, tpos, nn_hint, mq, s_park))
		if (threadIdx.x == 0)
			wl[atomicAdd(&wl_ctr[2u * parity], 1u)] = blockIdx.x;
}

#define MULLS_FUSED_PARK_BYTES (2u * 3u * MULLS_LDS_BLOCK * 4u)
__device__ __forceinline__ uint32_t *fused_park(unsigned char *lds_raw, uint32_t cap) { return reinterpret_cast<uint32_t *>(lds_raw + (((size_t)cap * 2u + 15u) & ~(size_t)15)); }

__global__ __launch_bounds__(MULLS_LDS_BLOCK) void k_cert_nn(const Job *__restrict__ cjobs, CloudDesc *__restrict__ descs, const PairState *__restrict__ states,
															  RunParams rp, float4 *__restrict__ spos, float4 *__restrict__ snrm, const GridDesc *__restrict__ grids,
															  const uint32_t *__restrict__ cell_start, const float4 *__restrict__ tsorted, uint8_t *flag,
															  int32_t *__restrict__ nn_idx, float *__restrict__ nn_d2, unsigned long long *__restrict__ winner,
															  const float4 *__restrict__ tnrm, int32_t *__restrict__ match, float *__restrict__ wd,
															  const float4 *__restrict__ tpos, int32_t *__restrict__ nn_hint, float4 *__restrict__ mq, uint32_t cap, uint32_t first)
{
	extern __shared__ __attribute__((aligned(16))) unsigned char lds_raw[];
	const Job job = cjobs[blockIdx.x];
	const PairState &ps = states[job.pair];
	if (!ps.active || (rp.normal_shooting && (job.cls == 0 || job.cls == 2 || job.cls == 4)))
		return;
	CloudDesc &d = descs[job.pair * MULLS_NC + job.cls];
	const GridDesc g = grids[job.pair * MULLS_NC + job.cls];
	__shared__ CertLds<MULLS_CERT_SMALL> s_cert;
	const bool direct = first && first_goes_direct(rp, d, job.cls);
	if (!direct)
	{
		if (cert_job<MULLS_LDS_BLOCK, MULLS_CERT_SMALL, true, 3>(s_cert, rp, ps, job, d, g, reinterpret_cast<uint32_t *>(lds_raw), spos, snrm, cell_start, tsorted, flag, nn_idx, nn_d2, winner,
																 tnrm, match, wd, tpos, nn_hint, mq, fused_park(lds_raw, cap)))
			return;
		__syncthreads();
	}
	lds_search_class(rp, ps, job, d, g, lds_layout(lds_raw, cap, rp.grid_maxcells), lds_raw, spos, snrm, cell_start, tsorted, flag, nn_idx, nn_d2, winner, tnrm, match,
					 wd, tpos, nn_hint, mq, direct);
}

__global__ __launch_bounds__(MULLS_LDS_BLOCK) void k_cert_mixed(uint32_t n_lds, const Job *__restrict__ cjobs, const Job *__restrict__ bjobs, uint32_t split,
																 CloudDesc *__restrict__ descs, const PairState *__restrict__ states, RunParams rp, float4 *__restrict__ spos,
																 float4 *__restrict__ snrm, const GridDesc *__restrict__ grids, const uint32_t *__restrict__ cell_start,
																 const unsigned long long *__restrict__ bm, const uint32_t *__restrict__ pf, const uint32_t *__restrict__ cs,
																 const float4 *__restrict__ tsorted, uint8_t *flag, int32_t *__restrict__ nn_idx, float *__restrict__ nn_d2,
																 unsigned long long *__restrict__ winner, const float4 *__restrict__ tnrm, int32_t *__restrict__ match,
																 float *__restrict__ wd, const float4 *__restrict__ tpos, int32_t *__restrict__ nn_hint, float4 *__restrict__ mq, uint32_t cap,
																 uint32_t first)
{
	extern __shared__ __attribute__((aligned(16))) unsigned char lds_raw[];
	if (blockIdx.x < n_lds)
	{
		const Job job = cjobs[blockIdx.x];
		const PairState &ps = states[job.pair];
		if (!ps.active)
			return;
		CloudDesc &d = descs[job.pair * MULLS_NC + job.cls];
		const GridDesc g = grids[job.pair * MULLS_NC + job.cls];
		__shared__ CertLds<MULLS_CERT_SMALL> s_cert;
		const bool direct = first && first_goes_direct(rp, d, job.cls);
		if (!direct)
		{
			if (cert_job<MULLS_LDS_BLOCK, MULLS_CERT_SMALL, true, 3>(s_cert, rp, ps, job, d, g, reinterpret_cast<uint32_t *>(lds_raw), spos, snrm, cell_start, tsorted, flag, nn_idx, nn_d2,
																	 winner, tnrm, match, wd, tpos, nn_hint, mq, fused_park(lds_raw, cap)))
				return;
			__syncthreads();
		}
		lds_search_class(rp, ps, job, d, g, lds_layout(lds_raw, cap, rp.grid_maxcells), lds_raw, spos, snrm, cell_start, tsorted, flag, nn_idx, nn_d2, winner, tnrm, match, wd, tpos,
						 nn_hint, mq, direct);
		return;
	}
	if (threadIdx.x >= MULLS_BIG_BLOCK)
		return;
	const uint32_t wg = blockIdx.x - n_lds;
	const Job job = bjobs[wg / split];
	const uint32_t part = wg % split;
	const PairState &ps = states[job.pair];
	if (!ps.active)
		return;
	const uint32_t ci = job.pair * MULLS_NC + job.cls;
	CloudDesc &d = descs[ci];
	const bool class_level = (job.count & MULLS_JOB_CLASS) != 0u;
	const uint32_t cnt = (job.count & ~MULLS_JOB_CLASS) ? (job.count & ~MULLS_JOB_CLASS) : (uint32_t)MULLS_SRC_PER_BLOCK;
	uint32_t q0, q1;
	if (class_level)
	{
		if (part)
			return;
		q0 = 0u, q1 = min(d.src_n, cnt);
	}
	else
	{
		const uint32_t per = cnt / split;
		q0 = job.start + part * per, q1 = min(d.src_n, q0 + per);
		if (q0 >= q1)
			return;
	}
	const GridDesc g = grids[ci];
	const BmGrid B = {bm + g.cell_off, pf + g.cell_off, cs + d.tgt_off + ci};
	cert_big<MULLS_BIG_BLOCK, 3>(*reinterpret_cast<BigLds<MULLS_BIG_BLOCK * 3> *>(lds_raw), rp, ps, job.cls, q0, q1, class_level, d, g, B, tsorted + d.tgt_off, spos, snrm, flag, nn_idx,
								 nn_d2, winner, tnrm, match, wd, tpos, reinterpret_cast<int2 *>(nn_hint), mq);
}

__global__ __launch_bounds__(MULLS_LDS_BLOCK) void k_nn_lds(const Job *__restrict__ cjobs, CloudDesc *__restrict__ descs,
															 const PairState *__restrict__ states, RunParams rp, const float4 *__restrict__ spos,
															 const float4 *__restrict__ snrm, const GridDesc *__restrict__ grids,
															 const uint32_t *__restrict__ cell_start, const float4 *__restrict__ tsorted,
															 uint8_t *flag, int32_t *__restrict__ nn_idx, float *__restrict__ nn_d2,
															 unsigned long long *__restrict__ winner, const float4 *__restrict__ tnrm, int32_t *__restrict__ match,
															 float *__restrict__ wd, const float4 *__restrict__ tpos, int32_t *__restrict__ nn_hint, float4 *__restrict__ mq,
															 uint32_t cap, const uint32_t *__restrict__ wl, uint32_t *__restrict__ wl_ctr, uint32_t parity, uint32_t first_njobs)
{
	extern __shared__ __attribute__((aligned(16))) unsigned char lds_raw[];
	const LdsLayout Y = lds_layout(lds_raw, cap, rp.grid_maxcells);

	const uint32_t n_queued = first_njobs ? first_njobs : wl_ctr[2u * parity];
	for (;;)
	{
		__syncthreads();
		if (threadIdx.x == 0)
			Y.HIST[65] = atomicAdd(&wl_ctr[2u * parity + 1u], 1u);
		__syncthreads();
		const uint32_t ticket = Y.HIST[65];
		if (ticket >= n_queued)
			return;
		const Job job = cjobs[first_njobs ? ticket : wl[ticket]];
		CloudDesc &d = descs[job.pair * MULLS_NC + job.cls];
		if (first_njobs && !(states[job.pair].active && first_goes_direct(rp, d, job.cls)))
			continue;
		lds_search_class(rp, states[job.pair], job, d, grids[job.pair * MULLS_NC + job.cls], Y, lds_raw, spos, snrm, cell_start, tsorted, flag, nn_idx, nn_d2, winner, tnrm,
						 match, wd, tpos, nn_hint, mq, first_njobs != 0u);
	}
}

__global__ __launch_bounds__(MULLS_BLOCK) void k_nn_shoot(const Job *__restrict__ jobs, CloudDesc *__restrict__ descs,
														   const PairState *__restrict__ states, RunParams rp, float4 *__restrict__ spos,
														   float4 *__restrict__ snrm, const float4 *__restrict__ tpos,
														   const uint8_t *__restrict__ flag, int32_t *__restrict__ nn_idx, float *__restrict__ nn_d2,
														   unsigned long long *__restrict__ winner)
{
	__shared__ float4 tile[1024];
	const Job job = jobs[blockIdx.x];
	if (!(job.cls == 0 || job.cls == 2 || job.cls == 4))
		return;
	const PairState &ps = states[job.pair];
	if (!ps.active)
		return;
	CloudDesc &d = descs[job.pair * MULLS_NC + job.cls];
	const uint32_t src_n = d.src_n, tgt_n = d.tgt_n, alive_cur = d.alive_cur;
	const bool called = class_called(rp, d, job.cls);
	const float r = 2.5f * ps.thr[job.cls];
	const double max_distance = (double)r;
	const bool gate = alive_cur >= 500u;
	const unsigned long long key_hi = (unsigned long long)(0xffffffffu - (rp.tick_base + (uint32_t)ps.iter)) << 32;
	uint32_t matched_cnt = 0;
	for (int u = 0; u < MULLS_SRC_PER_THREAD; u++)
	{
		const uint32_t s = job.start + threadIdx.x + u * MULLS_BLOCK;
		const bool alive = s < src_n && (flag[d.src_off + s] & MULLS_F_ALIVE);
		float px = 0, py = 0, pz = 0, nx = 0, ny = 0, nz = 0;
		if (alive)
		{
			const float4 p = spos[d.src_off + s], n = snrm[d.src_off + s];
			const double *T = ps.T;
			const double x = p.x, y = p.y, z = p.z, ax = n.x, ay = n.y, az = n.z;
			px = (float)(T[0] * x + T[1] * y + T[2] * z + T[3]);
			py = (float)(T[4] * x + T[5] * y + T[6] * z + T[7]);
			pz = (float)(T[8] * x + T[9] * y + T[10] * z + T[11]);
			nx = (float)(T[0] * ax + T[1] * ay + T[2] * az);
			ny = (float)(T[4] * ax + T[5] * ay + T[6] * az);
			nz = (float)(T[8] * ax + T[9] * ay + T[10] * az);
			spos[d.src_off + s] = make_float4(px, py, pz, p.w);
			snrm[d.src_off + s] = make_float4(nx, ny, nz, n.w);
		}
		if (!called)
			continue;
		float kd[10];
		int ki[10];
#pragma unroll
		for (int j = 0; j < 10; j++)
		{
			kd[j] = __builtin_inff();
			ki[j] = 0x7fffffff;
		}
		for (uint32_t base = 0; base < tgt_n; base += 1024)
		{
			const uint32_t nt = min(1024u, tgt_n - base);
			__syncthreads();
			for (uint32_t k = threadIdx.x; k < nt; k += MULLS_BLOCK)
				tile[k] = tpos[d.tgt_off + base + k];
			__syncthreads();
			for (uint32_t j = 0; j < nt; j++)
			{
				const float4 t = tile[j];
				const float dx = px - t.x, dy = py - t.y, dz = pz - t.z;
				float dist = (dx * dx + dy * dy) + dz * dz;
				int idx = (int)(base + j);
				if (dist < kd[9])
				{
#pragma unroll
					for (int q = 0; q < 10; q++)
					{
						const bool lt = dist < kd[q];
						const float td = kd[q];
						const int ti = ki[q];
						kd[q] = lt ? dist : td;
						ki[q] = lt ? idx : ti;
						dist = lt ? td : dist;
						idx = lt ? ti : idx;
					}
				}
			}
		}
		if (!alive)
			continue;
		double min_dist = 1.7976931348623157e308;
		int min_index = 0;
		int found = 0;
#pragma unroll
		for (int j = 0; j < 10; j++)
			found += ki[j] != 0x7fffffff ? 1 : 0;
#pragma unroll
		for (int j = 0; j < 10; j++)
			if (j < found)
			{
				const float4 t = tpos[d.tgt_off + (uint32_t)ki[j]];
				const float ptx = px - t.x, pty = py - t.y, ptz = pz - t.z;
				const double Vx = ptx, Vy = pty, Vz = ptz, Nx = nx, Ny = ny, Nz = nz;
				const double cx = Ny * Vz - Nz * Vy, cy = Nz * Vx - Nx * Vz, cz = Nx * Vy - Ny * Vx;
				const double dist = cx * cx + cy * cy + cz * cz;
				if (dist < min_dist)
				{
					min_dist = dist;
					min_index = j;
				}
			}
		float sel_d = 0.0f;
		int sel_i = -1;
#pragma unroll
		for (int j = 0; j < 10; j++)
			if (j == min_index)
			{
				sel_d = kd[j];
				sel_i = ki[j];
			}
		const bool matched = found > 0 && !(min_dist > max_distance);
		nn_idx[d.src_off + s] = matched ? sel_i : -1;
		nn_d2[d.src_off + s] = sel_d;
		if (matched)
		{
			matched_cnt++;
			if (gate)
				atomicMin(&winner[d.tgt_off + sel_i], key_hi | (unsigned long long)s);
		}
	}
	for (int off = 32; off > 0; off >>= 1)
		matched_cnt += __shfl_down(matched_cnt, off);
	if ((threadIdx.x & 63) == 0 && matched_cnt)
		atomicAdd(&d.n_matched, matched_cnt);
}

#include "launch.h"

static size_t fused_lds_bytes(uint32_t cap, uint32_t maxcells, bool dedup)
{
	const size_t heavy = nn_lds_bytes(cap, maxcells, dedup), light = (((size_t)cap * 2u + 15u) & ~(size_t)15) + MULLS_FUSED_PARK_BYTES;
	return heavy > light ? heavy : light;
}
size_t nn_lds_bytes(uint32_t cap, uint32_t maxcells, bool dedup)
{
	return (size_t)MULLS_LDS_QCHUNK * 16u + (size_t)MULLS_LDS_AUX + (size_t)cap * 14u + (((size_t)maxcells + 8u) & ~(size_t)1) * 2u + (dedup ? (size_t)cap * 4u : 0u);
}

int launch_nn_lds(hipStream_t st, uint32_t njobs, const Job *jobs, CloudDesc *descs, const PairState *states, const RunParams &rp, float4 *spos,
				  float4 *snrm, const GridDesc *grids, const uint32_t *cell_start, const float4 *tsorted, uint8_t *flag, int32_t *nn_idx,
				  float *nn_d2, unsigned long long *winner, const float4 *tnrm, int32_t *match, float *wd, const float4 *tpos, int32_t *nn_hint, float4 *mq, uint32_t cap, uint32_t maxcells,
				  uint32_t *wl, uint32_t *wl_ctr, uint32_t parity, bool first)
{
	const DevLaunch D = dev_launch<0>([](DevLaunch &d) {
		if (hipFuncSetAttribute(reinterpret_cast<const void *>(k_nn_lds), hipFuncAttributeMaxDynamicSharedMemorySize, 160 * 1024) != hipSuccess)
			return false;
		hipFuncAttributes fa;
		d.dyn_max[0] = 1;
		d.dyn_max[1] = 0;
		if (hipFuncGetAttributes(&fa, reinterpret_cast<const void *>(k_cert<MULLS_CERT_BLOCK, 3, 768>)) == hipSuccess)
			d.dyn_max[1] = fa.sharedSizeBytes;
		if (hipFuncGetAttributes(&fa, reinterpret_cast<const void *>(k_cert_nn)) == hipSuccess && fa.sharedSizeBytes < 160u * 1024u)
		{
			const size_t room = 160u * 1024u - fa.sharedSizeBytes;
			if (hipFuncSetAttribute(reinterpret_cast<const void *>(k_cert_nn), hipFuncAttributeMaxDynamicSharedMemorySize, (int)room) == hipSuccess)
				d.dyn_max[0] = room;
		}
		return true;
	});
	if (!D.ok)
		return -1;
	const uint32_t n_cu = D.n_cu;
	const size_t fused_dyn_max = D.dyn_max[0];
	if (!njobs)
		return 0;
	const bool dedup = rp.lds_dedup != 0u;
	if (njobs <= 2u * n_cu && rp.debug_stop != 10u && fused_lds_bytes(cap, maxcells, dedup) <= fused_dyn_max)
	{
		hipLaunchKernelGGL(k_cert_nn, dim3(njobs), dim3(MULLS_LDS_BLOCK), fused_lds_bytes(cap, maxcells, dedup), st, jobs, descs, states, rp, spos, snrm, grids, cell_start,
						   tsorted, flag, nn_idx, nn_d2, winner, tnrm, match, wd, tpos, nn_hint, mq, cap, first ? 1u : 0u);
		return 0;
	}
	if (first)
		;
	else if (njobs <= 2u * n_cu)
		hipLaunchKernelGGL(k_cert<1024>, dim3(njobs), dim3(1024), dedup ? ((size_t)cap * 2u + 3u) & ~(size_t)3 : 0u, st, jobs, descs, states, rp, spos, snrm, grids, cell_start, tsorted,
						   flag, nn_idx, nn_d2, winner, tnrm, match, wd, tpos, nn_hint, mq, wl, wl_ctr, parity & 1u);
	else if (dedup && MULLS_CERT_BLOCK == 512 && D.dyn_max[1] && (((size_t)cap * 2u + 3u) & ~(size_t)3) + D.dyn_max[1] <= 40u * 1024u)
		hipLaunchKernelGGL((k_cert<MULLS_CERT_BLOCK, 3, 768>), dim3(njobs), dim3(MULLS_CERT_BLOCK), ((size_t)cap * 2u + 3u) & ~(size_t)3, st, jobs, descs, states, rp, spos, snrm, grids,
						   cell_start, tsorted, flag, nn_idx, nn_d2, winner, tnrm, match, wd, tpos, nn_hint, mq, wl, wl_ctr, parity & 1u);
	else
		hipLaunchKernelGGL(k_cert<MULLS_CERT_BLOCK>, dim3(njobs), dim3(MULLS_CERT_BLOCK), dedup ? ((size_t)cap * 2u + 3u) & ~(size_t)3 : 0u, st, jobs, descs, states, rp, spos, snrm, grids,
						   cell_start, tsorted, flag, nn_idx, nn_d2, winner, tnrm, match, wd, tpos, nn_hint, mq, wl, wl_ctr, parity & 1u);
	hipLaunchKernelGGL(k_nn_lds, dim3(njobs < n_cu ? njobs : n_cu), dim3(MULLS_LDS_BLOCK), nn_lds_bytes(cap, maxcells, dedup), st, jobs, descs, states, rp, spos, snrm,
					   grids, cell_start, tsorted, flag, nn_idx, nn_d2, winner, tnrm, match, wd, tpos, nn_hint, mq, cap, wl, wl_ctr, parity & 1u, first ? njobs : 0u);
	return 0;
}

int launch_cert_mixed(hipStream_t st, uint32_t n_lds, const Job *cjobs, uint32_t n_big, const Job *bjobs, uint32_t max_wgs, uint32_t rounds, CloudDesc *descs, const PairState *states,
					  const RunParams &rp, float4 *spos, float4 *snrm, const GridDesc *grids, const uint32_t *cell_start, const unsigned long long *bm, const uint32_t *pf,
					  const uint32_t *cs, const float4 *tsorted, uint8_t *flag, int32_t *nn_idx, float *nn_d2, unsigned long long *winner, const float4 *tnrm, int32_t *match,
					  float *wd, const float4 *tpos, int32_t *nn_hint, float4 *mq, uint32_t cap, uint32_t maxcells, bool first)
{
	const DevLaunch D = dev_launch<1>([](DevLaunch &d) {
		hipFuncAttributes fa;
		d.dyn_max[0] = 1;
		if (hipFuncGetAttributes(&fa, reinterpret_cast<const void *>(k_cert_mixed)) == hipSuccess && fa.sharedSizeBytes < 160u * 1024u)
		{
			const size_t room = 160u * 1024u - fa.sharedSizeBytes;
			if (hipFuncSetAttribute(reinterpret_cast<const void *>(k_cert_mixed), hipFuncAttributeMaxDynamicSharedMemorySize, (int)room) == hipSuccess)
				d.dyn_max[0] = room;
		}
		return true;
	});
	const size_t dyn_max = D.dyn_max[0];
	const uint32_t n_cu = D.n_cu;
	if (!n_lds || !n_big || rp.normal_shooting || rp.debug_stop == 10u || rp.debug_stop == 22u)
		return 0;
	uint32_t split = 1;
	while (split < 16 && n_big * split * 2u <= max_wgs)
		split <<= 1;
	if (n_lds + n_big > n_cu)
		rounds = 1u;
	while (split > 1 && n_lds + n_big * split > n_cu * rounds)
		split >>= 1;
	const bool dedup = rp.lds_dedup != 0u;
	const size_t dyn = fused_lds_bytes(cap, maxcells, dedup) > sizeof(BigLds<MULLS_BIG_BLOCK * 3>) ? fused_lds_bytes(cap, maxcells, dedup) : sizeof(BigLds<MULLS_BIG_BLOCK * 3>);
	if (n_lds + n_big * split > n_cu * rounds || n_lds > n_cu || dyn > dyn_max)
		return 0;
	hipLaunchKernelGGL(k_cert_mixed, dim3(n_lds + n_big * split), dim3(MULLS_LDS_BLOCK), dyn, st, n_lds, cjobs, bjobs, split, descs, states, rp, spos, snrm, grids, cell_start, bm, pf, cs,
					   tsorted, flag, nn_idx, nn_d2, winner, tnrm, match, wd, tpos, nn_hint, mq, cap, first ? 1u : 0u);
	return 1;
}

void launch_cert_big(hipStream_t st, uint32_t njobs, const Job *jobs, uint32_t max_wgs, CloudDesc *descs, const PairState *states, const RunParams &rp, float4 *spos, float4 *snrm,
					 const GridDesc *grids, const unsigned long long *bm, const uint32_t *pf, const uint32_t *cs, const float4 *tsorted, uint8_t *flag, int32_t *nn_idx,
					 float *nn_d2, unsigned long long *winner, const float4 *tpos, const float4 *tnrm, int32_t *nn_hint, int32_t *match, float *wd, float4 *mq)
{
	if (!njobs)
		return;
	uint32_t split = 1;
	while (split < 16 && njobs * split * 2u <= max_wgs)
		split <<= 1;
	hipLaunchKernelGGL(k_cert_big, dim3(njobs * split), dim3(MULLS_BIG_BLOCK), 0, st, jobs, descs, states, rp, spos, snrm, grids, bm, pf, cs, tsorted, flag, nn_idx, nn_d2, winner,
					   split, tpos, tnrm, nn_hint, match, wd, mq);
}

void launch_nn(hipStream_t st, uint32_t njobs, const Job *jobs, CloudDesc *descs, const PairState *states, const RunParams &rp, float4 *spos,
			   float4 *snrm, const float4 *tpos, const uint8_t *flag, int32_t *nn_idx, float *nn_d2, unsigned long long *winner)
{
	if (njobs)
		hipLaunchKernelGGL(k_nn, dim3(njobs), dim3(MULLS_NN_BLOCK), 0, st, jobs, descs, states, rp, spos, snrm, tpos, flag, nn_idx, nn_d2, winner);
}

void launch_nn_shoot(hipStream_t st, uint32_t njobs, const Job *jobs, CloudDesc *descs, const PairState *states, const RunParams &rp,
					 float4 *spos, float4 *snrm, const float4 *tpos, const uint8_t *flag, int32_t *nn_idx, float *nn_d2, unsigned long long *winner)
{
	if (njobs)
		hipLaunchKernelGGL(k_nn_shoot, dim3(njobs), dim3(MULLS_BLOCK), 0, st, jobs, descs, states, rp, spos, snrm, tpos, flag, nn_idx, nn_d2,
						   winner);
}

void launch_filter(hipStream_t st, uint32_t njobs, const Job *jobs, CloudDesc *descs, const PairState *states, const RunParams &rp,
				   const float4 *snrm, const float4 *tnrm, uint8_t *flag, const int32_t *nn_idx, const float *nn_d2, int32_t *match, float *wd,
				   const unsigned long long *winner, const float4 *tpos, float4 *mq, bool big)
{
	if (njobs)
		hipLaunchKernelGGL(k_filter, dim3(njobs), dim3(MULLS_BLOCK), 0, st, jobs, descs, states, rp, snrm, tnrm, flag, nn_idx, nn_d2, match, wd,
						   winner, tpos, mq, big ? 1u : 0u);
}
```

mulls_amd/csrc/launch.h:

```cpp
#pragma once
#include <hip/hip_runtime_api.h>
#include <stdint.h>

#include "device_types.h"

#include <hip/hip_vector_types.h>
#include <mutex>

struct DevLaunch
{
	bool ready = false, ok = false;
	size_t dyn_max[2] = {0, 0};
	uint32_t n_cu = 256;
};
template <int TAG, class Init>
inline DevLaunch dev_launch(Init init)
{
	static std::mutex mu;
	static DevLaunch table[64];
	int dev = 0;
	if (hipGetDevice(&dev) != hipSuccess || dev < 0 || dev >= 64)
		dev = 0;
	std::lock_guard<std::mutex> lock(mu);
	DevLaunch &D = table[dev];
	if (!D.ready)
	{
		int cus = 0;
		if (hipDeviceGetAttribute(&cus, hipDeviceAttributeMultiprocessorCount, dev) == hipSuccess && cus > 0)
			D.n_cu = (uint32_t)cus;
		D.ok = init(D);
		D.ready = true;
	}
	return D;
}
void launch_clone_src(hipStream_t st, uint32_t njobs, const Job *jobs, const CloudDesc *descs, const PairSetup *setup, const float4 *stage,
					  float4 *tmp_pos, float4 *tmp_nrm, uint32_t *bbox, const RunParams &rp);
void launch_crop(hipStream_t st, uint32_t npairs, CloudDesc *descs, const PairSetup *setup, const uint32_t *bbox, const float4 *stage,
				 const float4 *tmp_pos, const float4 *tmp_nrm, float4 *spos, float4 *snrm, float4 *tpos, float4 *tnrm, uint8_t *flag,
				 int32_t *match, float *wd, const RunParams &rp, GridDesc *grids, uint32_t nbig_segs, const Job *big_segs, uint32_t nbig_clouds,
				 const Job *big_clouds, uint32_t *seg_cnt, uint32_t *big_box);
void launch_copy_segs(hipStream_t st, const CopySeg *segs, uint32_t n);
void launch_motion_comp(hipStream_t st, float4 *recs, uint32_t n, const double q[4], const double t[3], float thre);
void launch_thin(hipStream_t st, uint32_t npairs, CloudDesc *descs, const uint8_t *src_keep, const uint8_t *tgt_keep, float4 *spos, float4 *snrm,
				 float4 *tpos, float4 *tnrm);
int launch_tgt_grid(hipStream_t st, uint32_t npairs, CloudDesc *descs, const PairSetup *setup, const uint32_t *bbox, const float4 *stage, const RunParams &rp,
					GridDesc *grids, uint16_t *tmap, uint32_t *cell_start, float4 *tsorted);
void launch_grid_build_sort(hipStream_t st, uint32_t npairs, const CloudDesc *descs, GridDesc *grids, const RunParams &rp, const float4 *tpos, uint32_t *cell_start,
							float4 *tsorted);
void launch_bm_build(hipStream_t st, uint32_t nl, const uint32_t *lclouds, uint32_t ntjobs, const Job *tjobs, const CloudDesc *descs, GridDesc *grids, const float4 *tpos,
					 unsigned long long *bm, uint32_t *pf, uint32_t *cnt, uint32_t *cs, float4 *tsorted, uint32_t *rank);
size_t nn_lds_bytes(uint32_t cap, uint32_t maxcells, bool dedup);
int launch_nn_lds(hipStream_t st, uint32_t njobs, const Job *jobs, CloudDesc *descs, const PairState *states, const RunParams &rp, float4 *spos,
				  float4 *snrm, const GridDesc *grids, const uint32_t *cell_start, const float4 *tsorted, uint8_t *flag, int32_t *nn_idx,
				  float *nn_d2, unsigned long long *winner, const float4 *tnrm, int32_t *match, float *wd, const float4 *tpos, int32_t *nn_hint, float4 *mq, uint32_t cap, uint32_t maxcells,
				  uint32_t *wl, uint32_t *wl_ctr, uint32_t parity, bool first = false);
int launch_cert_mixed(hipStream_t st, uint32_t n_lds, const Job *cjobs, uint32_t n_big, const Job *bjobs, uint32_t max_wgs, uint32_t rounds, CloudDesc *descs, const PairState *states,
					  const RunParams &rp, float4 *spos, float4 *snrm, const GridDesc *grids, const uint32_t *cell_start, const unsigned long long *bm, const uint32_t *pf,
					  const uint32_t *cs, const float4 *tsorted, uint8_t *flag, int32_t *nn_idx, float *nn_d2, unsigned long long *winner, const float4 *tnrm, int32_t *match,
					  float *wd, const float4 *tpos, int32_t *nn_hint, float4 *mq, uint32_t cap, uint32_t maxcells, bool first = false);
void launch_cert_big(hipStream_t st, uint32_t njobs, const Job *jobs, uint32_t max_wgs, CloudDesc *descs, const PairState *states, const RunParams &rp, float4 *spos, float4 *snrm,
					 const GridDesc *grids, const unsigned long long *bm, const uint32_t *pf, const uint32_t *cs, const float4 *tsorted, uint8_t *flag, int32_t *nn_idx,
					 float *nn_d2, unsigned long long *winner, const float4 *tpos, const float4 *tnrm, int32_t *nn_hint, int32_t *match, float *wd, float4 *mq);
void launch_nn(hipStream_t st, uint32_t njobs, const Job *jobs, CloudDesc *descs, const PairState *states, const RunParams &rp, float4 *spos,
			   float4 *snrm, const float4 *tpos, const uint8_t *flag, int32_t *nn_idx, float *nn_d2, unsigned long long *winner);
void launch_nn_shoot(hipStream_t st, uint32_t njobs, const Job *jobs, CloudDesc *descs, const PairState *states, const RunParams &rp,
					 float4 *spos, float4 *snrm, const float4 *tpos, const uint8_t *flag, int32_t *nn_idx, float *nn_d2, unsigned long long *winner);
void launch_filter(hipStream_t st, uint32_t njobs, const Job *jobs, CloudDesc *descs, const PairState *states, const RunParams &rp,
				   const float4 *snrm, const float4 *tnrm, uint8_t *flag, const int32_t *nn_idx, const float *nn_d2, int32_t *match, float *wd,
				   const unsigned long long *winner, const float4 *tpos, float4 *mq, bool big = false);
void launch_accum(hipStream_t st, const uint32_t *leaders, const uint32_t split[4], const Job *jobs, const CloudDesc *descs, const PairState *states, const RunParams &rp,
				  const float4 *spos, const float4 *mq, const uint8_t *flag, float *wd, double *partial, bool single = false, uint32_t wave_min_trips = 0);
void launch_finish(hipStream_t st, uint32_t npairs, CloudDesc *descs, const PairState *states, const RunParams &rp, const double *partial,
				   PairOut *out, PairOut *out_host, const uint32_t *bbox, uint32_t *ticket, volatile uint32_t *host_epoch, uint32_t epoch,
				   uint32_t pair_base);
void launch_push_states(hipStream_t st, const PairState *host_states, PairState *dev_states, uint32_t npairs);
namespace mulls
{
struct IcpConst;
struct StepState;
}
void launch_step_init(hipStream_t st, uint32_t npairs, const PairSetup *setup, const mulls::IcpConst &K, mulls::StepState *steps, PairState *states);
void launch_finish_step(hipStream_t st, uint32_t pair_base, uint32_t npairs, CloudDesc *descs, PairState *states, const RunParams &rp, const mulls::IcpConst &K, const double *partial,
						PairOut *out, const uint32_t *bbox, mulls::StepState *steps, IcpOut *results, unsigned long long *host_word, uint32_t epoch, int brute,
						uint32_t *ticket = nullptr, bool sum_step = false);
void launch_transform_aos(hipStream_t st, float4 *recs, uint32_t n, const double *T12);
void launch_transform_clouds(hipStream_t st, float4 *const recs[], const uint32_t n[], int count, const double T12[12]);
void launch_set_corr(hipStream_t st, uint32_t src_off, const int32_t *cs, const int32_t *ct, const float *cd, uint32_t n, uint8_t *flag,
					 int32_t *match, float *wd, uint32_t tgt_off, const float4 *tpos, const float4 *tnrm, float4 *mq);
```

mulls_amd/csrc/lds_tier.h:

```cpp
#pragma once
#include "device_util.h"
struct FilterCtx
{
	bool gate, any_match, normal_check, dedup_done, strict;
	float max_sqr;
	double cos_thre;
	unsigned long long key_hi;
	const float4 *tgt_stage;
	const uint16_t *tgt_map;
};
__device__ __forceinline__ void filter_point(const FilterCtx &F, const CloudDesc &d, uint32_t s, const float4 *__restrict__ snrm,
											  const float4 *__restrict__ tnrm, uint8_t *__restrict__ flag, const int32_t *__restrict__ nn_idx,
											  const float *__restrict__ nn_d2, int32_t *__restrict__ match, float *__restrict__ wd,
											  const unsigned long long *__restrict__ winner, const float4 *__restrict__ tpos,
											  float4 *__restrict__ mq, uint32_t &n_alive, uint32_t &n_valid)
{
	const uint32_t g = d.src_off + s;
	const uint32_t f = flag[g];
	if (!(f & MULLS_F_ALIVE))
		return;
	bool alive = true, valid, fresh = false;
	int m;
	float4 n2 = make_float4(0.0f, 0.0f, 0.0f, 0.0f);
	if (F.any_match)
	{
		m = nn_idx[g];
		valid = m >= 0;
		if (F.gate && (m < 0 || (!F.dedup_done && winner[d.tgt_off + m] != (F.key_hi | (unsigned long long)s))))
		{
			alive = false;
			valid = false;
		}
		if (valid)
		{
			const float dist = nn_d2[g];
			valid = F.strict ? dist < F.max_sqr : !(dist > F.max_sqr);
			if (valid)
			{
				wd[g] = dist;
				if (match[g] == m)
					n2 = mq[2u * g + 1u];
				else
				{
					match[g] = m;
					float4 q2;
					tgt_record(F.tgt_stage, F.tgt_map, d, (uint32_t)m, tpos, tnrm, q2, n2);
					mq[2u * g] = q2;
					mq[2u * g + 1u] = n2;
				}
				fresh = true;
			}
		}
	}
	else if (F.gate)
	{
		alive = false;
		valid = false;
		m = -1;
	}
	else
	{
		valid = (f & MULLS_F_VALID) != 0;
		m = match[g];
	}
	if (valid && F.normal_check)
	{
		const float4 n1 = snrm[g];
		if (!fresh)
			n2 = mq[2u * g + 1u];
		const double dot = (double)n1.x * (double)n2.x + (double)n1.y * (double)n2.y + (double)n1.z * (double)n2.z;
		const float c = (float)fabs(dot);
		if ((double)c < F.cos_thre)
			valid = false;
	}
	flag[g] = (uint8_t)((alive ? MULLS_F_ALIVE : 0u) | (valid ? MULLS_F_VALID : 0u));
	n_alive += alive ? 1u : 0u;
	n_valid += valid ? 1u : 0u;
}
namespace
{
typedef unsigned long long nnkey;
#define NNKEY_NONE 0x7f800000ffffffffull
__device__ __forceinline__ nnkey nn_key(float dist, uint32_t idx) { return ((nnkey)__float_as_uint(dist) << 32) | idx; }
__device__ __forceinline__ float key_dist(nnkey k) { return __uint_as_float((uint32_t)(k >> 32)); }
__device__ __forceinline__ bool key_found(nnkey k) { return (uint32_t)k != 0xffffffffu; }

struct LdsGrid
{
	const float *P;
	const uint16_t *IDX, *CS;
	__device__ __forceinline__ uint32_t cs(uint32_t i) const { return CS[i]; }
	__device__ __forceinline__ void cand(uint32_t t, float &x, float &y, float &z, uint32_t &i) const
	{
		const float *p = P + 3u * t;
		x = p[0], y = p[1], z = p[2];
		i = IDX[t];
	}
};
struct GlobGrid
{
	const float4 *ts;
	const uint16_t *CS;
	__device__ __forceinline__ uint32_t cs(uint32_t i) const { return CS[i]; }
	__device__ __forceinline__ void cand(uint32_t t, float &x, float &y, float &z, uint32_t &i) const
	{
		const float4 v = ts[t];
		x = v.x, y = v.y, z = v.z;
		i = __float_as_uint(v.w);
	}
};

template <int CTRL>
__device__ __forceinline__ void dpp_min_step(nnkey &bk)
{
	const uint32_t oh = (uint32_t)__builtin_amdgcn_update_dpp(0, (int)(uint32_t)(bk >> 32), CTRL, 0xf, 0xf, false);
	const uint32_t ol = (uint32_t)__builtin_amdgcn_update_dpp(0, (int)(uint32_t)bk, CTRL, 0xf, 0xf, false);
	const nnkey o = ((nnkey)oh << 32) | ol;
	bk = o < bk ? o : bk;
}
#define MULLS_LDS_GSH (MULLS_LDS_GROUP == 16u ? 4 : (MULLS_LDS_GROUP == 8u ? 3 : 2))
template <int GSH>
__device__ __forceinline__ uint32_t sub_lanes(uint32_t gsh) { return GSH >= 0 ? (1u << (GSH >= 0 ? GSH : 0)) : (1u << gsh); }
template <int GSH = MULLS_LDS_GSH>
__device__ __forceinline__ void row16_min(nnkey &bk, uint32_t gsh = 0u)
{
	const uint32_t GL = sub_lanes<GSH>(gsh);
	dpp_min_step<0xB1>(bk);
	if (GL >= 4u)
		dpp_min_step<0x4E>(bk);
	if (GL >= 8u)
		dpp_min_step<0x141>(bk);
	if (GL >= 16u)
		dpp_min_step<0x140>(bk);
}
template <int CTRL>
__device__ __forceinline__ void dpp_fmin_step(float &v)
{
	const float o = __int_as_float(__builtin_amdgcn_update_dpp(0, __float_as_int(v), CTRL, 0xf, 0xf, false));
	v = fminf(o, v);
}
template <int GSH = MULLS_LDS_GSH>
__device__ __forceinline__ void row16_min2(nnkey &bk, float &sec, uint32_t gsh = 0u)
{
	const uint32_t GL = sub_lanes<GSH>(gsh);
	nnkey g = bk;
	row16_min<GSH>(g, gsh);
	float c = (bk == g) ? sec : key_dist(bk);
	dpp_fmin_step<0xB1>(c);
	if (GL >= 4u)
		dpp_fmin_step<0x4E>(c);
	if (GL >= 8u)
		dpp_fmin_step<0x141>(c);
	if (GL >= 16u)
		dpp_fmin_step<0x140>(c);
// ... 692 lines not shown
	{
		const uint32_t c = CL.red[w];
		base += w < wave ? c : 0u;
		total += c;
	}
	if (keep)
	{
		const uint32_t k = base + (uint32_t)__popcll(bal & ((1ull << lane) - 1ull));
		CL.uq[k] = e;
		CL.us[k] = es;
	}
	__syncthreads();
	return total;
}

template <int BLK, bool W16, int SMALL>
__device__ __forceinline__ bool cert_class(CertLds<SMALL> &CL, const RunParams &rp, const PairState &ps, const Job &job, CloudDesc &d, const GridDesc &g, uint32_t *W,
											float4 *__restrict__ spos, float4 *__restrict__ snrm, const uint32_t *__restrict__ cell_start,
											const float4 *__restrict__ tsorted, uint8_t *flag, int32_t *__restrict__ nn_idx, float *__restrict__ nn_d2,
											unsigned long long *__restrict__ winner, const float4 *__restrict__ tnrm, int32_t *__restrict__ match,
											float *__restrict__ wd, const float4 *__restrict__ tpos, int32_t *__restrict__ nn_hint, float4 *__restrict__ mq)
{
	float4 *uq = CL.uq;
	uint32_t *us = CL.us, *red = CL.red;
	uint32_t &ucount = CL.ucount;
	int2 *__restrict__ hint2 = reinterpret_cast<int2 *>(nn_hint);

	const uint32_t src_n = d.src_n, tgt_n = d.tgt_n;
	const bool called = class_called(rp, d, job.cls);
	const ClassCtx C = class_ctx(rp, ps, g, job.cls, d.alive_cur, called);
	const bool have_prev = ps.iter > 0;
	const bool use_hint = called && have_prev;
	const bool kc = CertLds<SMALL>::LOOK && rp.kcert != 0u && use_hint && C.cand != nullptr;
	const uint32_t q_end = min(src_n, job.start + (job.count ? job.count : (uint32_t)MULLS_SRC_PER_BLOCK));
	if (C.dedup)
		dedup_init<W16>(W, tgt_n, BLK);
	if (threadIdx.x == 0)
		ucount = 0u;
	__syncthreads();

	uint32_t matched_cnt = 0;
	for (uint32_t s = job.start + threadIdx.x; s < q_end; s += BLK)
	{
		const uint32_t gi = d.src_off + s;
		const uint32_t fl = flag[gi];
		const float4 p = spos[gi], n = snrm[gi];
		const int2 h = hint2[gi];
		const int32_t pm0 = match[gi];
		const float4 q0 = mq[2u * gi];
		if (!(fl & MULLS_F_ALIVE))
			continue;
		uint32_t hv = 0xffffu;
		float lb = 0.0f;
		int32_t pm = -1;
		if (have_prev)
		{
			lb = __int_as_float(h.y);
			if (use_hint)
			{
				hv = (uint32_t)h.x;
				pm = pm0;
			}
		}
		const uint32_t hj = hv & 0xffffu;
		float4 tj = make_float4(0.0f, 0.0f, 0.0f, 0.0f);
		if (hj < tgt_n)
			tj = (int32_t)hj == pm ? q0 : tgt_point(rp.tgt_stage, rp.tgt_map, d, hj, tpos);
		const double *T = ps.T;
		const double x = p.x, y = p.y, z = p.z, nx = n.x, ny = n.y, nz = n.z;
		float4 out;
		out.x = (float)(T[0] * x + T[1] * y + T[2] * z + T[3]);
		out.y = (float)(T[4] * x + T[5] * y + T[6] * z + T[7]);
		out.z = (float)(T[8] * x + T[9] * y + T[10] * z + T[11]);
		const float onx = (float)(T[0] * nx + T[1] * ny + T[2] * nz);
		const float ony = (float)(T[4] * nx + T[5] * ny + T[6] * nz);
		const float onz = (float)(T[8] * nx + T[9] * ny + T[10] * nz);
		spos[gi] = make_float4(out.x, out.y, out.z, p.w);
		snrm[gi] = make_float4(onx, ony, onz, n.w);
		const float mx = out.x - p.x, my = out.y - p.y, mz = out.z - p.z;
		const float moved = sqrtf((mx * mx + my * my) + mz * mz);
		const float lb_next = lb - moved * 1.00001f;
		if (!called)
		{
			nn_hint[2u * gi + 1u] = __float_as_int(have_prev ? lb_next : 0.0f);
			continue;
		}
		out.w = __builtin_inff();
		bool certified = false;
		if (hj < tgt_n)
		{
			const float dx = out.x - tj.x, dy = out.y - tj.y, dz = out.z - tj.z;
			const float d0 = (dx * dx + dy * dy) + dz * dz;
			if (d0 >= 0.0f)
			{
				const float dh = sqrtf(d0);
				certified = rp.cert != 0u && (dh * 1.00001f + moved * 1.00001f < lb * 0.99999f);
				out.w = dh + fminf(fmaxf(rp.cert_slack_rate * moved, rp.cert_slack_min), rp.cert_slack_max);
				if (certified)
				{
					const bool matched = !((double)d0 > C.max_dist_sqr);
					nn_idx[gi] = matched ? (int32_t)hj : -1;
					nn_d2[gi] = d0;
					hint2[gi] = make_int2((int32_t)hj, __float_as_int(lb_next));
					if (matched)
					{
						matched_cnt++;
						if (C.dedup)
							dedup_min<W16>(W, hj, s);
						else if (C.gate)
							atomicMin(&winner[d.tgt_off + hj], C.key_hi | (unsigned long long)s);
					}
				}
			}
		}
		if (!certified)
		{
			nn_idx[gi] = MULLS_NEEDS_SEARCH;
			nn_d2[gi] = out.w;
			const uint32_t k = atomicAdd(&ucount, 1u);
			if (k < (uint32_t)SMALL)
			{
				const bool second = kc && hj < tgt_n;
				uq[k] = out;
				us[k] = second ? s | MULLS_US_KCERT : s;
				if (CertLds<SMALL>::LOOK)
					CL.um[k] = moved;
			}
		}
	}
	if (!called)
		return true;
	__syncthreads();
	uint32_t U = ucount;
	if (kc && U >= rp.kcert_min && U <= (uint32_t)SMALL)
		U = kcert_list<BLK, W16, SMALL>(CL, rp, ps, C, d, U, nn_idx, nn_d2, hint2, W, winner, tpos, matched_cnt);
	if (U > (uint32_t)SMALL)
		return false;
	const GlobGrid L = {tsorted + d.tgt_off, reinterpret_cast<const uint16_t *>(cell_start) + g.cell_off};
	const uint32_t sub = threadIdx.x & (MULLS_LDS_GROUP - 1u), grp = threadIdx.x / MULLS_LDS_GROUP;
	for (uint32_t i = grp; i < U; i += BLK / MULLS_LDS_GROUP)
	{
		nnkey bk;
		float sec, Rfin;
		uint32_t trips;
		CandOut co = {0xffffffffu, 0xffffffffu, 0.0f};
		search_query<MULLS_GLOB_CHUNK>(g, L, uq[i], C.r, C.m, sub, bk, sec, Rfin, trips, co);
		if (sub == 0 && commit_search<W16>(C, d, us[i] & ~MULLS_US_KCERT, bk, sec, Rfin, trips, co, nn_idx, nn_d2, hint2, W, winner))
			matched_cnt++;
	}
	class_tail<BLK, W16>(rp, ps, C, d, job, q_end, matched_cnt, U, W, red, snrm, tnrm, flag, nn_idx, nn_d2, match, wd, winner, tpos, mq);
	return true;
}

template <int BLK, int TRIPS, bool W16, int SMALL, bool PARK = false>
__device__ __forceinline__ bool cert_class_flat(CertLds<SMALL> &CL, const RunParams &rp, const PairState &ps, const Job &job, CloudDesc &d, const GridDesc &g, uint32_t *W,
												 float4 *__restrict__ spos, float4 *__restrict__ snrm, const uint32_t *__restrict__ cell_start,
												 const float4 *__restrict__ tsorted, uint8_t *flag, int32_t *__restrict__ nn_idx, float *__restrict__ nn_d2,
												 unsigned long long *__restrict__ winner, const float4 *__restrict__ tnrm, int32_t *__restrict__ match,
												 float *__restrict__ wd, const float4 *__restrict__ tpos, int32_t *__restrict__ nn_hint, float4 *__restrict__ mq, uint32_t *park = nullptr)
{
	float4 *uq = CL.uq;
	uint32_t *us = CL.us, *red = CL.red;
	uint32_t &ucount = CL.ucount;
	int2 *__restrict__ hint2 = reinterpret_cast<int2 *>(nn_hint);
	const uint32_t src_n = d.src_n, tgt_n = d.tgt_n;
	const ClassCtx C = class_ctx(rp, ps, g, job.cls, d.alive_cur, true);
	const bool have_prev = ps.iter > 0;
	const bool normal_check = job.cls != 5;
	const bool kc = CertLds<SMALL>::LOOK && rp.kcert != 0u && have_prev && C.cand != nullptr;
	const uint32_t q_end = src_n;
	unsigned long long t_prev = rp.dbg_ticks ? wall_clock64() : 0ull;
#define FLAT_TICK(k)                                                  \
	if (rp.dbg_ticks)                                                 \
	{                                                                 \
		const unsigned long long now_ = wall_clock64();               \
		if (threadIdx.x == 0)                                         \
			atomicAdd(&rp.dbg_ticks[k], now_ - t_prev);               \
		t_prev = now_;                                                \
	}

	struct Rec
	{
		uint32_t fl;
		int32_t pm;
		float3 p, n, q, t;
		int2 h;
	};
	const uint32_t last = d.src_off + (q_end ? q_end - 1u : 0u);
	auto load = [&](int k) {
		Rec r;
		const uint32_t gi = min(d.src_off + threadIdx.x + (uint32_t)k * BLK, last);
		r.fl = flag[gi];
		r.p = *reinterpret_cast<const float3 *>(spos + gi), r.n = *reinterpret_cast<const float3 *>(snrm + gi);
		r.h = hint2[gi];
		r.pm = match[gi];
		r.q = *reinterpret_cast<const float3 *>(mq + 2u * gi), r.t = *reinterpret_cast<const float3 *>(mq + 2u * gi + 1u);
		return r;
	};
	uint32_t STr[PARK ? 1 : TRIPS];
	int32_t Mr[PARK ? 1 : TRIPS];
	float D0r[PARK ? 1 : TRIPS];
	auto setSM = [&](int k, uint32_t st, int32_t m) {
		if (PARK)
			park[(uint32_t)k * BLK + threadIdx.x] = (st << 24) | (uint32_t)(m + 2);
		else
			STr[PARK ? 0 : k] = st, Mr[PARK ? 0 : k] = m;
	};
	auto getST = [&](int k) -> uint32_t { return PARK ? park[(uint32_t)k * BLK + threadIdx.x] >> 24 : STr[PARK ? 0 : k]; };
	auto getM = [&](int k) -> int32_t { return PARK ? (int32_t)(park[(uint32_t)k * BLK + threadIdx.x] & 0xffffffu) - 2 : Mr[PARK ? 0 : k]; };
	auto setD0 = [&](int k, float v) {
		if (PARK)
			park[(uint32_t)(TRIPS + k) * BLK + threadIdx.x] = __float_as_uint(v);
		else
			D0r[PARK ? 0 : k] = v;
	};
	auto getD0 = [&](int k) -> float { return PARK ? __uint_as_float(park[(uint32_t)(TRIPS + k) * BLK + threadIdx.x]) : D0r[PARK ? 0 : k]; };
	auto waits = [&](int k) -> bool { return PARK ? (getST(k) & MULLS_FS_SEARCH) != 0u : getM(k) == MULLS_NEEDS_SEARCH; };
	uint32_t matched_cnt = 0;
	auto cert = [&](int k, const Rec &r) {
		const uint32_t s = threadIdx.x + (uint32_t)k * BLK, gi = d.src_off + s;
		uint32_t st_k = 0u;
		int32_t m_k = -1;
		setSM(k, 0u, -1), setD0(k, 0.0f);
		if (s >= q_end || !(r.fl & MULLS_F_ALIVE))
			return;
		st_k = r.fl & (MULLS_FS_ALIVE | MULLS_FS_VALID);
		const float3 p = r.p, n = r.n;
		uint32_t hv = 0xffffu;
		float lb = 0.0f;
		int32_t pm = -1;
		if (have_prev)
		{
			lb = __int_as_float(r.h.y);
			hv = (uint32_t)r.h.x;
			pm = r.pm;
		}
		const uint32_t hj = hv & 0xffffu;
		float4 tj = make_float4(0.0f, 0.0f, 0.0f, 0.0f);
		if (hj < tgt_n)
			tj = (int32_t)hj == pm ? make_float4(r.q.x, r.q.y, r.q.z, 0.0f) : tgt_point(rp.tgt_stage, rp.tgt_map, d, hj, tpos);
		const double *T = ps.T;
		const double x = p.x, y = p.y, z = p.z, nx = n.x, ny = n.y, nz = n.z;
		float4 out;
		out.x = (float)(T[0] * x + T[1] * y + T[2] * z + T[3]);
		out.y = (float)(T[4] * x + T[5] * y + T[6] * z + T[7]);
		out.z = (float)(T[8] * x + T[9] * y + T[10] * z + T[11]);
		const float onx = (float)(T[0] * nx + T[1] * ny + T[2] * nz);
		const float ony = (float)(T[4] * nx + T[5] * ny + T[6] * nz);
		const float onz = (float)(T[8] * nx + T[9] * ny + T[10] * nz);
		*reinterpret_cast<float3 *>(spos + gi) = make_float3(out.x, out.y, out.z);
		*reinterpret_cast<float3 *>(snrm + gi) = make_float3(onx, ony, onz);
		{
			const double dot = (double)onx * (double)r.t.x + (double)ony * (double)r.t.y + (double)onz * (double)r.t.z;
			const float c = (float)fabs(dot);
			if (!((double)c < rp.cos_bearing))
				st_k |= MULLS_FS_DIR_OK;
		}
		const float mx = out.x - p.x, my = out.y - p.y, mz = out.z - p.z;
		const float moved = sqrtf((mx * mx + my * my) + mz * mz);
		const float lb_next = lb - moved * 1.00001f;
		out.w = __builtin_inff();
		bool certified = false;
		if (hj < tgt_n)
		{
			const float dx = out.x - tj.x, dy = out.y - tj.y, dz = out.z - tj.z;
			const float d0 = (dx * dx + dy * dy) + dz * dz;
			if (d0 >= 0.0f)
			{
				const float dh = sqrtf(d0);
				certified = rp.cert != 0u && (dh * 1.00001f + moved * 1.00001f < lb * 0.99999f);
				out.w = dh + fminf(fmaxf(rp.cert_slack_rate * moved, rp.cert_slack_min), rp.cert_slack_max);
				if (certified)
				{
					const bool matched = !((double)d0 > C.max_dist_sqr);
					m_k = matched ? (int32_t)hj : -1;
					setD0(k, d0);
					hint2[gi] = make_int2((int32_t)hj, __float_as_int(lb_next));
					if (matched)
					{
						matched_cnt++;
						if ((int32_t)hj == r.pm)
							st_k |= MULLS_FS_STANDING;
						if (C.dedup)
							dedup_min<W16>(W, hj, s);
					}
				}
			}
		}
		if (!certified)
		{
			setD0(k, out.w);
			if (PARK)
			{
				st_k |= MULLS_FS_SEARCH;
				m_k = r.pm;
			}
			else
			{
				m_k = MULLS_NEEDS_SEARCH;
				nn_idx[gi] = MULLS_NEEDS_SEARCH;
				nn_d2[gi] = out.w;
			}
			const uint32_t u = atomicAdd(&ucount, 1u);
			if (u < (uint32_t)SMALL)
			{
				const bool second = kc && hj < tgt_n;
				uq[u] = out;
				us[u] = second ? s | MULLS_US_KCERT : s;
				if (CertLds<SMALL>::LOOK)
					CL.um[u] = moved;
			}
		}
		setSM(k, st_k, m_k);
	};

	static_assert(TRIPS == 2 || TRIPS == 3, "two trips' loads in flight");
	Rec r0 = load(0), r1 = load(1);
	if (C.dedup)
		dedup_init<W16>(W, tgt_n, BLK);
	if (threadIdx.x == 0)
		ucount = 0u;
	__syncthreads();
	FLAT_TICK(0)
	{
		const bool third = TRIPS == 3 && q_end > 2u * (uint32_t)BLK;
		cert(0, r0);
		if (third)
		{
			r0 = load(2);
			cert(1, r1);
			cert(2, r0);
		}
		else
		{
			cert(1, r1);
			if (TRIPS == 3)
				setSM(2, 0u, -1), setD0(2, 0.0f);
		}
	}
	__syncthreads();
	FLAT_TICK(2)
	uint32_t U = ucount;
	const uint32_t U0 = U;
	if (kc && U >= rp.kcert_min && U <= (uint32_t)SMALL)
		U = kcert_list<BLK, W16, SMALL>(CL, rp, ps, C, d, U, nn_idx, nn_d2, hint2, W, winner, tpos, matched_cnt);
	FLAT_TICK(1)
	if (rp.dbg_ticks && threadIdx.x == 0)
	{
		atomicAdd(&rp.dbg_ticks[13], (unsigned long long)U0);
		atomicAdd(&rp.dbg_ticks[7], (unsigned long long)U);
	}
	if (U > (uint32_t)SMALL)
	{
#pragma unroll
		for (int k = 0; k < TRIPS; k++)
			if ((getST(k) & MULLS_FS_ALIVE) && (PARK || !waits(k)))
			{
				const uint32_t gi = d.src_off + threadIdx.x + (uint32_t)k * BLK;
				nn_idx[gi] = waits(k) ? MULLS_NEEDS_SEARCH : getM(k);
				nn_d2[gi] = getD0(k);
			}
		return false;
	}
	if (U)
	{
		const GlobGrid L = {tsorted + d.tgt_off, reinterpret_cast<const uint16_t *>(cell_start) + g.cell_off};
		const uint32_t sub = threadIdx.x & (MULLS_LDS_GROUP - 1u), grp = threadIdx.x / MULLS_LDS_GROUP;
		for (uint32_t i = grp; i < U; i += BLK / MULLS_LDS_GROUP)
		{
			nnkey bk;
			float sec, Rfin;
			uint32_t trips;
			CandOut co = {0xffffffffu, 0xffffffffu, 0.0f};
			search_query<MULLS_GLOB_CHUNK>(g, L, uq[i], C.r, C.m, sub, bk, sec, Rfin, trips, co);
			if (sub == 0 && (PARK ? commit_search_park<W16, BLK * TRIPS>(C, d, us[i] & ~MULLS_US_KCERT, bk, sec, Rfin, trips, co, hint2, W, park)
								  : commit_search<W16>(C, d, us[i] & ~MULLS_US_KCERT, bk, sec, Rfin, trips, co, nn_idx, nn_d2, hint2, W, winner)))
				matched_cnt++;
		}
	}
	for (int off = 32; off > 0; off >>= 1)
		matched_cnt += __shfl_down(matched_cnt, off);
	if ((threadIdx.x & 63) == 0)
		red[threadIdx.x >> 6] = matched_cnt;
	__threadfence_block();
	__syncthreads();
	uint32_t total_matched = 0;
	for (int w = 0; w < BLK / 64; w++)
		total_matched += red[w];
	FLAT_TICK(3)

	const float thr = ps.thr[job.cls], max_sqr = thr * thr;
	const bool any_match = total_matched > 0u, strict = rp.rej_strict != 0;
	uint32_t n_alive = 0, n_valid = 0;
#pragma unroll
	for (int k = 0; k < TRIPS; k++)
	{
		const uint32_t st = getST(k);
		if (!(st & MULLS_FS_ALIVE))
			continue;
		const uint32_t s = threadIdx.x + (uint32_t)k * BLK, gi = d.src_off + s;
		int32_t m = getM(k);
		float dist = getD0(k);
		bool standing = (st & MULLS_FS_STANDING) != 0;
		if (PARK ? (st & MULLS_FS_SEARCH) != 0u : m == MULLS_NEEDS_SEARCH)
		{
			m = nn_idx[gi];
			dist = nn_d2[gi];
			standing = m >= 0 && match[gi] == m;
		}
		if (C.dedup && m >= 0 && !dedup_holds<W16>(W, (uint32_t)m, s))
			m = -1;
		bool alive = true, valid, dir_ok = (st & MULLS_FS_DIR_OK) != 0;
		if (any_match)
		{
			valid = m >= 0;
			if (C.gate && m < 0)
			{
				alive = false;
				valid = false;
			}
			if (valid)
			{
				if (!standing)
				{
					match[gi] = m;
					float4 q2, n2;
					tgt_record(rp.tgt_stage, rp.tgt_map, d, (uint32_t)m, tpos, tnrm, q2, n2);
					mq[2u * gi] = q2;
					mq[2u * gi + 1u] = n2;
					if (normal_check)
					{
						const float3 n1 = *reinterpret_cast<const float3 *>(snrm + gi);
						const double dot = (double)n1.x * (double)n2.x + (double)n1.y * (double)n2.y + (double)n1.z * (double)n2.z;
						const float c = (float)fabs(dot);
						dir_ok = !((double)c < rp.cos_bearing);
					}
				}
				valid = strict ? dist < max_sqr : !(dist > max_sqr);
				if (valid)
					wd[gi] = dist;
			}
		}
		else if (C.gate)
		{
			alive = false;
			valid = false;
		}
		else
			valid = (st & MULLS_FS_VALID) != 0;
		if (valid && normal_check && !dir_ok)
			valid = false;
		const uint32_t nf = (alive ? MULLS_F_ALIVE : 0u) | (valid ? MULLS_F_VALID : 0u);
		if (nf != (st & (MULLS_FS_ALIVE | MULLS_FS_VALID)))
			flag[gi] = (uint8_t)nf;
		n_alive += alive ? 1u : 0u;
		n_valid += valid ? 1u : 0u;
	}
	for (int off = 32; off > 0; off >>= 1)
	{
		n_alive += __shfl_down(n_alive, off);
		n_valid += __shfl_down(n_valid, off);
	}
	if ((threadIdx.x & 63) == 0)
	{
		red[BLK / 64 + (threadIdx.x >> 6)] = n_alive;
		red[2 * (BLK / 64) + (threadIdx.x >> 6)] = n_valid;
	}
	__syncthreads();
	if (threadIdx.x == 0)
	{
		uint32_t ta = 0, tv = 0;
		for (int w = 0; w < BLK / 64; w++)
		{
			ta += red[BLK / 64 + w];
			tv += red[2 * (BLK / 64) + w];
		}
		d.n_matched = total_matched;
		d.alive_next = ta;
		d.valid_next = tv;
		d.n_search = U;
	}
	FLAT_TICK(4)
	if (rp.dbg_ticks && threadIdx.x == 0)
		atomicAdd(&rp.dbg_ticks[6], 1ull);
#undef FLAT_TICK
	return true;
}

struct LdsLayout
{
	float4 *qpos;
	uint32_t *HIST;
	uint16_t *ORDER;
	float *P;
	uint16_t *IDX;
	uint16_t *CS;
	uint32_t *W;
};
__device__ __forceinline__ LdsLayout lds_layout(unsigned char *lds_raw, uint32_t cap, uint32_t grid_maxcells)
{
	LdsLayout L;
	L.qpos = reinterpret_cast<float4 *>(lds_raw);
	L.HIST = reinterpret_cast<uint32_t *>(L.qpos + MULLS_LDS_QCHUNK);
	L.ORDER = reinterpret_cast<uint16_t *>(L.HIST + 80);
	L.P = reinterpret_cast<float *>(reinterpret_cast<unsigned char *>(L.HIST) + MULLS_LDS_AUX);
	L.IDX = reinterpret_cast<uint16_t *>(L.P + 3u * cap);
	L.CS = L.IDX + cap;
	L.W = reinterpret_cast<uint32_t *>(L.CS + ((grid_maxcells + 8u) & ~1u));
	return L;
}

__device__ __forceinline__ void lds_search_class(const RunParams &rp, const PairState &ps, const Job &job, CloudDesc &d, const GridDesc &g,
												  const LdsLayout &Y, unsigned char *lds_raw, const float4 *__restrict__ spos,
												  const float4 *__restrict__ snrm, const uint32_t *__restrict__ cell_start,
												  const float4 *__restrict__ tsorted, uint8_t *flag, int32_t *__restrict__ nn_idx, float *__restrict__ nn_d2,
												  unsigned long long *__restrict__ winner, const float4 *__restrict__ tnrm, int32_t *__restrict__ match,
												  float *__restrict__ wd, const float4 *__restrict__ tpos, int32_t *__restrict__ nn_hint, float4 *__restrict__ mq,
												  bool first = false)
{
	unsigned long long t_prev = rp.dbg_ticks ? wall_clock64() : 0ull;
#define HEAVY_TICK(k)                                                 \
	if (rp.dbg_ticks)                                                 \
	{                                                                 \
		const unsigned long long now_ = wall_clock64();               \
		if (threadIdx.x == 0)                                         \
			atomicAdd(&rp.dbg_ticks[k], now_ - t_prev);               \
		t_prev = now_;                                                \
	}
	float4 *qpos = Y.qpos;
	uint32_t *HIST = Y.HIST;
	uint16_t *ORDER = Y.ORDER;
	float *P = Y.P;
	uint16_t *IDX = Y.IDX, *CS = Y.CS;
	uint32_t *W = Y.W;
	int2 *__restrict__ hint2 = reinterpret_cast<int2 *>(nn_hint);
	const uint32_t src_n = d.src_n, tgt_n = d.tgt_n;
	const ClassCtx C = class_ctx(rp, ps, g, job.cls, d.alive_cur, true);
	const uint32_t q_end = min(src_n, job.start + (job.count ? job.count : (uint32_t)MULLS_SRC_PER_BLOCK));
	const uint32_t q_cnt = q_end > job.start ? q_end - job.start : 0u, n_chunks = (q_cnt + MULLS_LDS_QCHUNK - 1u) / MULLS_LDS_QCHUNK;
	const uint32_t q_step = n_chunks ? (q_cnt + n_chunks - 1u) / n_chunks : 1u;

	float4 pf_p = make_float4(0.0f, 0.0f, 0.0f, 0.0f);
	float pf_w = 0.0f;
	uint32_t pf_hv = 0u, pf_f = 0u;
	int32_t pf_i = -1;
	auto prefetch = [&](uint32_t chunk) {
		const uint32_t s = chunk + threadIdx.x, gi = d.src_off + s;
		pf_f = 0u;
		pf_i = -1;
		if (chunk < q_end && s < min(q_end, chunk + q_step))
		{
			pf_f = flag[gi];
			pf_p = spos[gi];
			if (first)
				pf_i = MULLS_NEEDS_SEARCH, pf_w = __builtin_inff(), pf_hv = 0u;
			else
			{
				pf_i = nn_idx[gi];
				pf_w = nn_d2[gi];
				pf_hv = (uint32_t)hint2[gi].x;
			}
		}
	};
	prefetch(job.start);

	{
		const float4 *__restrict__ ts = tsorted + d.tgt_off;
		for (uint32_t k0 = threadIdx.x; k0 < tgt_n; k0 += 8 * MULLS_LDS_BLOCK)
		{
			float4 t[8];
#pragma unroll
			for (int u = 0; u < 8; u++)
			{
				const uint32_t k = k0 + u * MULLS_LDS_BLOCK;
				if (k < tgt_n)
					t[u] = ts[k];
			}
#pragma unroll
			for (int u = 0; u < 8; u++)
			{
				const uint32_t k = k0 + u * MULLS_LDS_BLOCK;
				if (k < tgt_n)
				{
					P[3u * k] = t[u].x;
					P[3u * k + 1u] = t[u].y;
					P[3u * k + 2u] = t[u].z;
					IDX[k] = (uint16_t)__float_as_int(t[u].w);
				}
			}
		}
		const uint4 *__restrict__ cs4 = reinterpret_cast<const uint4 *>(reinterpret_cast<const uint16_t *>(cell_start) + g.cell_off);
		const uint32_t nw = (g.ncell + 1u + 7u) >> 3;
		for (uint32_t w0 = threadIdx.x; w0 < nw; w0 += 2 * MULLS_LDS_BLOCK)
		{
			const uint32_t w1 = w0 + MULLS_LDS_BLOCK;
			const uint4 va = cs4[w0], vb = cs4[min(w1, nw - 1u)];
			reinterpret_cast<uint4 *>(CS)[w0] = va;
			if (w1 < nw)
				reinterpret_cast<uint4 *>(CS)[w1] = vb;
		}
	}
	if (C.dedup)
		for (uint32_t t = threadIdx.x; t < tgt_n; t += MULLS_LDS_BLOCK)
			W[t] = 0xffffffffu;
	const LdsGrid L = {P, IDX, CS};
	const uint32_t sub = threadIdx.x & (MULLS_LDS_GROUP - 1u);
	uint32_t matched_cnt = 0, searched = 0;

	if (threadIdx.x < 32u)
		HIST[threadIdx.x] = 0u;
	for (uint32_t chunk = job.start; chunk < q_end; chunk += q_step)
	{
		__syncthreads();
		HEAVY_TICK(chunk == job.start ? 8 : 10)
		uint32_t bucket = 0, rank = 0xffffffffu;
		if (threadIdx.x < MULLS_LDS_QCHUNK && (pf_f & MULLS_F_ALIVE))
		{
			if (pf_i == MULLS_NEEDS_SEARCH)
			{
				qpos[threadIdx.x] = make_float4(pf_p.x, pf_p.y, pf_p.z, pf_w);
				bucket = 31u - ((pf_hv >> 16) & 31u);
				if (!(pf_w < __builtin_inff()))
				{
					const uint32_t c = grid_cell_id(g, pf_p.x, pf_p.y, pf_p.z);
					bucket = CS[c + 1u] > CS[c] ? 8u : 0u;
				}
				rank = atomicAdd(&HIST[bucket], 1u);
			}
			else if (pf_i >= 0)
			{
				matched_cnt++;
				if (C.dedup)
					atomicMin(&W[pf_i], chunk + threadIdx.x);
			}
// ... 64 lines not shown
```

mulls_amd/csrc/loop.cpp:

```cpp
#include "batch.h"

using namespace mulls_drv;

namespace
{
struct Run
{
	mulls_ctx *ctx;
	mulls_batch *B;
	const mulls_params *P;
	mulls_result *results;
	int n;
	hipStream_t st;
	std::chrono::steady_clock::time_point wall0;
	EvTimer evt;
	RunParams rp;
	mulls::IcpConst K;
	uint32_t lds_cap = 0;
	uint32_t max_big_tgt = 0;
	int tier = 0;
	bool use_grid = false, dstep = false;
};
#define RUN_ALIASES \
	mulls_ctx *ctx = R.ctx; \
// ... 40 lines not shown
	rp.win_pt = P->pt2pt_residual_window;
	rp.win_pl = P->pt2pl_residual_window;
	rp.win_li = P->pt2li_residual_window;
	rp.cos_bearing = std::cos(P->normal_bearing / 180.0 * M_PI);
	rp.resid_from_iter = 2;
	init_cert(ctx, rp);
	if ((rc = take_epochs(ctx, B, (uint32_t)std::max(P->max_iter_num, 0) + 2u, rp)) != MULLS_OK)
		return rc;
	rp.debug_stop = (uint32_t)ctx->opt[MULLS_OPT_DEBUG_STOP];

	bool dstep = P->max_iter_num > 0;
	for (int p = 0; p < n && dstep; p++)
		dstep = !(results[p].trace && results[p].trace_cap > 0);
	dstep = dstep && ctx->opt[MULLS_OPT_HOST_STEP] == 0.0;
	uint32_t lds_cap = 0;
	int tier = 0;
	const int dstep_nsub = (ctx->profiling == 0 && n >= (int)ctx->opt[MULLS_OPT_SPLIT_MIN_PAIRS] && n <= (int)ctx->opt[MULLS_OPT_SPLIT_MAX_PAIRS]) ? 2 : 1;
	rc = prepare_run(ctx, B, P, rp, &lds_cap, &tier, dstep ? dstep_nsub : 0, true);
	if (rc != MULLS_OK)
		return rc;
	const bool use_grid = tier != 0;
	R.lds_cap = lds_cap, R.tier = tier, R.use_grid = use_grid, R.dstep = dstep;
	R.max_big_tgt = 0;
	if (tier == 3)
		for (const CloudDesc &d : B->descs_h)
			if (d.tier == MULLS_TIER_BM)
				R.max_big_tgt = std::max(R.max_big_tgt, d.tgt_n0);

	bool fused_tgt = tier == 2 && ctx->opt[MULLS_OPT_FUSED_TGT_SETUP] != 0.0 && !P->keep_less_source_points && !rp.normal_shooting && B->n_big_tgt == 0;
	for (size_t k = 0; k < B->descs_h.size() && fused_tgt; k++)
		fused_tgt = B->descs_h[k].tgt_n0 <= MULLS_LDS_MAXPTS;
	fused_tgt = fused_tgt || tier == 3;
	if (fused_tgt)
	{
		rp.tgt_stage = B->stage;
		rp.tgt_map = B->tmap;
		rp.grid_maxcells = std::min(rp.grid_maxcells, 32767u);
	}

	if (rp.debug_stop == 20u || rp.debug_stop == 21u)
	{
		if (!B->dbg && dmalloc(ctx, &B->dbg, 16) != MULLS_OK)
			return MULLS_E_HIP;
		HIPCHK(ctx, hipMemsetAsync(B->dbg, 0, 16 * sizeof(unsigned long long), st));
		rp.dbg_ticks = B->dbg;
	}

	evt.begin(&ctx->prof.ms_setup);
	launch_clone_src(st, (uint32_t)B->setup_jobs_h.size(), B->setup_jobs, B->descs, B->setup, B->stage, B->tmp_pos, B->tmp_nrm, B->bbox, rp);
	launch_crop(st, (uint32_t)n, B->descs, B->setup, B->bbox, B->stage, B->tmp_pos, B->tmp_nrm, B->spos, B->snrm, B->tpos, B->tnrm, B->flag,
				B->match, B->wd, rp, B->grids, (uint32_t)B->big_segs_h.size(), B->big_segs, (uint32_t)B->big_clouds_h.size(), B->big_clouds, B->seg_cnt,
				B->big_box);
	if (P->keep_less_source_points && !rp.undistort)
	{
		std::vector<CloudDesc> back(B->descs_h.size());
		HIPCHK(ctx, hipMemcpyAsync(back.data(), B->descs, sizeof(CloudDesc) * back.size(), hipMemcpyDeviceToHost, st));
		HIPCHK(ctx, hipStreamSynchronize(st));
		std::vector<uint8_t> skeep(std::max<size_t>(B->n_src, 1), 1), tkeep(std::max<size_t>(B->n_tgt, 1), 1);
		for (int p = 0; p < n; p++)
		{
			const CloudDesc *pd = &back[(size_t)p * MULLS_NC];
			auto T = [&](int c, int keep) { return thin_mask(tkeep.data() + pd[c].tgt_off, pd[c].tgt_n, keep, P->rng_seed, 0 * 6 + c); };
			auto S = [&](int c, int keep) { return thin_mask(skeep.data() + pd[c].src_off, pd[c].src_n, keep, P->rng_seed, 1 * 6 + c); };
			const uint32_t tg = T(MULLS_GROUND, (int)(pd[MULLS_GROUND].tgt_n / 2));
			const uint32_t tf = T(MULLS_FACADE, (int)(pd[MULLS_FACADE].tgt_n / 2));
			S(MULLS_GROUND, (int)(tg / 4));
			S(MULLS_FACADE, (int)(tf / 2));
			S(MULLS_PILLAR, (int)pd[MULLS_PILLAR].tgt_n);
			S(MULLS_BEAM, (int)pd[MULLS_BEAM].tgt_n);
			S(MULLS_ROOF, (int)pd[MULLS_ROOF].tgt_n);
			S(MULLS_VERTEX, (int)pd[MULLS_VERTEX].tgt_n);
		}
		uint8_t *d_sk = nullptr, *d_tk = nullptr;
		if (dmalloc(ctx, &d_sk, skeep.size()) != MULLS_OK || dmalloc(ctx, &d_tk, tkeep.size()) != MULLS_OK)
			return MULLS_E_HIP;
		hipError_t e = hipMemcpyAsync(d_sk, skeep.data(), skeep.size(), hipMemcpyHostToDevice, st);
		if (e == hipSuccess)
			e = hipMemcpyAsync(d_tk, tkeep.data(), tkeep.size(), hipMemcpyHostToDevice, st);
		if (e == hipSuccess)
		{
			launch_thin(st, (uint32_t)n, B->descs, d_sk, d_tk, B->spos, B->snrm, B->tpos, B->tnrm);
			e = hipStreamSynchronize(st);
		}
		(void)hipFree(d_sk);
		(void)hipFree(d_tk);
		if (e != hipSuccess)
		{
			ctx->err = std::string("keep_less_source_points: ") + hipGetErrorString(e);
			return MULLS_E_HIP;
		}
	}
	if (fused_tgt)
		(void)launch_tgt_grid(st, (uint32_t)n, B->descs, B->setup, B->bbox, B->stage, rp, B->grids, B->tmap, B->cell_start, B->tsorted);
	else if (tier == 2)
		launch_grid_build_sort(st, (uint32_t)n, B->descs, B->grids, rp, B->tpos, B->cell_start, B->tsorted);
	launch_bm_build(st, (uint32_t)B->lclouds_h.size(), B->lclouds, (uint32_t)B->tjobs_h.size(), B->tjobs, B->descs, B->grids, B->tpos, B->bm, B->pf, B->cell_cnt, B->bm_cs,
					B->tsorted, B->bm_rank);
	evt.end();

	R.K = icp_const(P);
	return MULLS_OK;
}

struct Slice
{
	uint32_t job_lo = 0, job_n = 0, cjob_lo = 0, cjob_n = 0, bjob_lo = 0, bjob_n = 0, fjob_lo = 0, fjob_n = 0, ejob_lo = 0, ejob_n = 0;
	const uint32_t *ajob_split = nullptr;
};
Slice slice_of(const mulls_batch *B, int lo, int hi, int k)
{
	auto first_of = [](const std::vector<Job> &v, uint32_t pair) {
		return (uint32_t)(std::lower_bound(v.begin(), v.end(), pair, [](const Job &j, uint32_t q) { return j.pair < q; }) - v.begin());
	};
	Slice L;
	L.job_lo = first_of(B->jobs_h, (uint32_t)lo);
	L.job_n = first_of(B->jobs_h, (uint32_t)hi) - L.job_lo;
	L.cjob_lo = first_of(B->cjobs_h, (uint32_t)lo);
	L.cjob_n = first_of(B->cjobs_h, (uint32_t)hi) - L.cjob_lo;
	L.bjob_lo = first_of(B->bjobs_h, (uint32_t)lo);
	L.bjob_n = first_of(B->bjobs_h, (uint32_t)hi) - L.bjob_lo;
	L.fjob_lo = first_of(B->fjobs_h, (uint32_t)lo);
	L.fjob_n = first_of(B->fjobs_h, (uint32_t)hi) - L.fjob_lo;
	L.ejob_lo = first_of(B->ejobs_h, (uint32_t)lo);
	L.ejob_n = first_of(B->ejobs_h, (uint32_t)hi) - L.ejob_lo;
	L.ajob_split = B->ajob_split[k];
	return L;
}

int launch_search(Run &R, hipStream_t sst, const Slice &L, uint32_t *wl, uint32_t *wl_ctr, uint32_t parity, EvTimer &ev, int iter)
{
RUN_ALIASES
	const Job *jobs = B->jobs + L.job_lo;
	ev.begin(&ctx->prof.ms_nn);
	if (tier == 0)
		launch_nn(sst, L.job_n, jobs, B->descs, B->states, rp, B->spos, B->snrm, B->tpos, B->flag, B->nn_idx, B->nn_d2, B->winner);
	const bool early = L.ejob_n && (iter < (int)ctx->opt[MULLS_OPT_BIG_EARLY_SETS] || (L.bjob_n - L.fjob_n < 64u && R.max_big_tgt > 100000u));
	const uint32_t max_wgs = iter < std::max(3, (int)ctx->opt[MULLS_OPT_BIG_EARLY_SETS]) ? 2048u : 512u;
#ifndef MULLS_MIXED_WIDE_ITERS
#define MULLS_MIXED_WIDE_ITERS 2
#endif
#ifndef MULLS_MIXED_ROUNDS
#define MULLS_MIXED_ROUNDS 3u
#endif
	const uint32_t mixed_rounds = early && iter < MULLS_MIXED_WIDE_ITERS ? MULLS_MIXED_ROUNDS : 1u;
	const uint32_t big_n = early ? L.ejob_n : L.bjob_n;
	const Job *big_jobs = early ? B->ejobs + L.ejob_lo : B->bjobs + L.bjob_lo;
	const bool first = iter == 0 && rp.lds_dedup != 0u && !rp.normal_shooting && ctx->opt[MULLS_OPT_FIRST_DIRECT] != 0.0;
	const bool together = tier == 3 && L.cjob_n && big_n &&
						  launch_cert_mixed(sst, L.cjob_n, B->cjobs + L.cjob_lo, big_n, big_jobs, max_wgs, mixed_rounds, B->descs, B->states, rp, B->spos, B->snrm, B->grids, B->cell_start, B->bm,
											B->pf, B->bm_cs, B->tsorted, B->flag, B->nn_idx, B->nn_d2, B->winner, B->tnrm, B->match, B->wd, B->tpos, B->nn_hint, B->mq, lds_cap,
											rp.grid_maxcells, first) != 0;
	if (!together && L.cjob_n &&
		launch_nn_lds(sst, L.cjob_n, B->cjobs + L.cjob_lo, B->descs, B->states, rp, B->spos, B->snrm, B->grids, B->cell_start, B->tsorted, B->flag, B->nn_idx, B->nn_d2, B->winner,
					  B->tnrm, B->match, B->wd, B->tpos, B->nn_hint, B->mq, lds_cap, rp.grid_maxcells, wl, wl_ctr, parity, first) != 0)
	{
		ctx->err = "could not raise the dynamic LDS limit of k_nn_lds";
		return MULLS_E_HIP;
	}
	if (together)
		;
	else if (early)
		launch_cert_big(sst, L.ejob_n, B->ejobs + L.ejob_lo, max_wgs, B->descs, B->states, rp, B->spos, B->snrm, B->grids, B->bm, B->pf, B->bm_cs, B->tsorted, B->flag, B->nn_idx,
						B->nn_d2, B->winner, B->tpos, B->tnrm, B->nn_hint, B->match, B->wd, B->mq);
	else if (L.bjob_n)
		launch_cert_big(sst, L.bjob_n, B->bjobs + L.bjob_lo, max_wgs, B->descs, B->states, rp, B->spos, B->snrm, B->grids, B->bm, B->pf, B->bm_cs, B->tsorted, B->flag, B->nn_idx,
						B->nn_d2, B->winner, B->tpos, B->tnrm, B->nn_hint, B->match, B->wd, B->mq);
	if (rp.normal_shooting)
		launch_nn_shoot(sst, L.job_n, jobs, B->descs, B->states, rp, B->spos, B->snrm, B->tpos, B->flag, B->nn_idx, B->nn_d2, B->winner);
	ev.end();
	ev.begin(&ctx->prof.ms_filter);
	if (tier == 0 || (tier == 2 && !rp.lds_dedup))
		launch_filter(sst, L.job_n, jobs, B->descs, B->states, rp, B->snrm, B->tnrm, B->flag, B->nn_idx, B->nn_d2, B->match, B->wd, B->winner, B->tpos, B->mq);
	else if (early)
		launch_filter(sst, L.ejob_n, B->ejobs + L.ejob_lo, B->descs, B->states, rp, B->snrm, B->tnrm, B->flag, B->nn_idx, B->nn_d2, B->match, B->wd, B->winner, B->tpos, B->mq, true);
	else if (L.fjob_n)
		launch_filter(sst, L.fjob_n, B->fjobs + L.fjob_lo, B->descs, B->states, rp, B->snrm, B->tnrm, B->flag, B->nn_idx, B->nn_d2, B->match, B->wd, B->winner, B->tpos, B->mq, true);
	ev.end();
	const hipError_t e = hipGetLastError();
	if (e != hipSuccess)
	{
		ctx->err = std::string("correspondence search launch: ") + hipGetErrorString(e);
		return MULLS_E_HIP;
	}
	return MULLS_OK;
}

int results_from_device(Run &R)
{
RUN_ALIASES
	const auto wall0 = R.wall0;

		if (grow_pinned(ctx, &B->icp_outs_pin, &B->cap_icp_pin, (size_t)n, hipHostMallocDefault) != MULLS_OK)
			return MULLS_E_NOMEM;
		HIPCHK(ctx, hipMemcpyAsync(B->icp_outs_pin, B->icp_outs, sizeof(IcpOut) * (size_t)n, hipMemcpyDeviceToHost, st));
		HIPCHK(ctx, hipStreamSynchronize(st));
		evt.collect();
		const double wall_ms = std::chrono::duration<double>(std::chrono::steady_clock::now() - wall0).count() * 1e3;
		int max_it = 0;
		for (int p = 0; p < n; p++)
		{
			const IcpOut &o = B->icp_outs_pin[p];
			mulls_result &R = results[p];
			R.code = o.code;
			R.iters = o.iters;
			std::memcpy(R.T, o.T, sizeof(R.T));
			std::memcpy(R.info, o.info, sizeof(R.info));
			R.sigma = (float)std::sqrt(o.sigma2);
			R.confidence = o.ratio;
			R.singular = o.singular;
			R.ms_total = (float)(wall_ms / n);
			for (int c = 0; c < MULLS_NC; c++)
			{
				R.ncorr[c] = o.ncorr[c];
				R.nsrc0[c] = o.nsrc0[c];
				R.ntgt0[c] = o.ntgt0[c];
			}
			R.cropped = 0;
			std::memset(R.crop_box, 0, sizeof(R.crop_box));
			fill_crop_box(rp, B->setup_h[p].tgt_bound, o.bbox, R);
			R.trace_len = 0;
			ctx->prof.nn_src_pts += o.src_pts;
			ctx->prof.nn_tgt_unique += o.tgt_pts;
			ctx->prof.nn_tgt_pts += o.tgt_job_pts;
			ctx->prof.nn_corr_pts += o.corr_pts;
			ctx->prof.nn_pair_evals += o.pair_evals;
			max_it = std::max(max_it, o.iters);
		}
		ctx->prof.iterations = max_it;
		if (rp.dbg_ticks)
		{
			unsigned long long t[16];
			HIPCHK(ctx, hipMemcpy(t, rp.dbg_ticks, sizeof(t), hipMemcpyDeviceToHost));
			if (rp.debug_stop == 21u)
			{
				ctx->prof.icp_fused_ms[0] += (double)t[13], ctx->prof.icp_fused_ms[1] += (double)t[7] * 1e-5;
				return MULLS_OK;
			}
			for (int k = 0; k < 5; k++)
				ctx->prof.icp_fused_ms[k] += (double)t[k] * 1e-5;
			ctx->prof.icp_fused_ms[5] += (double)t[6];
			ctx->prof.icp_search_ms[0] += (double)t[13], ctx->prof.icp_search_ms[1] += (double)t[14], ctx->prof.icp_search_ms[2] += (double)t[15], ctx->prof.icp_search_ms[3] += (double)t[7];
			for (int k = 0; k < 4; k++)
				ctx->prof.icp_phase_ms[k] += (double)t[8 + k] * 1e-5;
			ctx->prof.icp_phase_ms[4] += (double)t[12];
		}
		return MULLS_OK;
}

int run_device_step(Run &R)
{
RUN_ALIASES
	int rc;
	if (grow(ctx, &B->steps, &B->cap_steps, (size_t)n) != MULLS_OK || grow(ctx, &B->icp_outs, &B->cap_icp_outs, (size_t)n) != MULLS_OK)
		return MULLS_E_HIP;
	HIPCHK(ctx, hipMemsetAsync(B->icp_outs, 0, sizeof(IcpOut) * (size_t)n, st));
	launch_step_init(st, (uint32_t)n, B->setup, K, B->steps, B->states);
	const bool few_launches = n <= (int)ctx->opt[MULLS_OPT_FEW_LAUNCHES_MAX_PAIRS];
	bool sum_step = ctx->opt[MULLS_OPT_SUM_STEP] != 0.0;
	for (size_t k = 0; sum_step && k < B->descs_h.size(); k++)
		sum_step = B->descs_h[k].job_end - B->descs_h[k].job_begin <= 4u * (1024u / MULLS_SRC_PER_BLOCK);
	struct Sub
	{
		int lo = 0, hi = 0;
		Slice L;
		hipStream_t st = nullptr;
		volatile unsigned long long *word = nullptr;
		unsigned long long *word_dev = nullptr;
		uint32_t *epoch_ctr = nullptr, *ticket = nullptr, *wl = nullptr, *wl_ctr = nullptr;
		uint32_t epoch0 = 0, nn_launches = 0, left = 0;
		int s = 0;
		bool done = false;
		EvTimer ev2[2] = {EvTimer{nullptr}, EvTimer{nullptr}};
	};
	const int nsub = B->nsub;
	Sub subs[2];
	for (int k = 0; k < nsub; k++)
	{
		Sub &S = subs[k];
		S.lo = (int)((long)n * k / nsub);
		S.hi = (int)((long)n * (k + 1) / nsub);
		S.L = slice_of(B, S.lo, S.hi, k);
		S.st = k == 0 ? ctx->stream : ctx->stream2;
		S.word = reinterpret_cast<volatile unsigned long long *>(B->epoch_h + 32 + 16 * k);
		S.word_dev = reinterpret_cast<unsigned long long *>(B->epoch_dev + 32 + 16 * k);
		S.epoch_ctr = k == 0 ? &B->epoch2 : &B->epoch3;
		S.epoch0 = *S.epoch_ctr;
		S.ticket = B->ticket + 2 + 4 * k;
		S.wl = B->wl + S.L.cjob_lo;
		S.wl_ctr = B->wl_ctr + 8 * k;
		S.left = (uint32_t)(S.hi - S.lo);
		for (int e = 0; e < 2; e++)
		{
			S.ev2[e].ctx = ctx;
			S.ev2[e].base = 10 * e;
		}
	}
	subs[0].ev2[0].used = evt.used;
	for (int k = 0; k < 5; k++)
		subs[0].ev2[0].slot[k] = evt.slot[k];
	evt.used = 0;
	if (nsub == 2)
	{
		HIPCHK(ctx, hipEventRecord(ctx->ev_setup, ctx->stream));
		HIPCHK(ctx, hipStreamWaitEvent(ctx->stream2, ctx->ev_setup, 0));
	}
	struct DrainOnError
	{
// ... 430 lines not shown
```

Measured before the change: 269,900.

## Fuse normal-equation accumulation into the flat certificate kernel for small classes

When the 512-thread flat certificate path handles a whole class, it now computes the per-point ICP normal-equation terms in place. It reuses the park and LDS staging buffers, reduces the terms per wave with DPP, and writes per-job partial sums directly. An acc_epoch stamp in the cloud descriptor then lets the separate reduce kernel skip those classes, so they are not reloaded and re-accumulated. This adds LDS pressure and register use to the certificate kernel, plus epoch-matching logic that must stay consistent with the tick base and iteration.

```diff
diff --git a/include/mulls_hip.h b/include/mulls_hip.h
--- a/include/mulls_hip.h
+++ b/include/mulls_hip.h
@@ -172,7 +172,8 @@
 	MULLS_OPT_ACCUM_WAVE_MIN_TRIPS = 25,
 	MULLS_OPT_FIRST_DIRECT = 26,
 	MULLS_OPT_SUM_STEP = 27,
-	MULLS_OPT_COUNT = 28
+	MULLS_OPT_ACCUM_IN_CERT = 28,
+	MULLS_OPT_COUNT = 29
 };
 int mulls_set_option(mulls_ctx *ctx, int option, double value);
 int mulls_get_option(const mulls_ctx *ctx, int option, double *value);
diff --git a/mulls_amd/abi.py b/mulls_amd/abi.py
--- a/mulls_amd/abi.py
+++ b/mulls_amd/abi.py
@@ -17,7 +17,8 @@
 
 (OPT_HOST_STEP, _OPT_RESERVED_1, _OPT_RESERVED_2, OPT_FEW_LAUNCHES_MAX_PAIRS, OPT_SUBBATCHES, OPT_TWO_STREAMS, OPT_CERTIFICATES, OPT_CERT_SLACK_MIN,
  OPT_CERT_SLACK_MAX, OPT_CERT_SLACK_RATE, OPT_LDS_DEDUP, OPT_GRID_H0, OPT_BM_H0, OPT_LEAN_STAGING, OPT_DEBUG_STOP, OPT_DEBUG_TICK, OPT_SPLIT_MIN_PAIRS, OPT_SPLIT_MAX_PAIRS,
- OPT_FUSED_TGT_SETUP, OPT_STAGGER, OPT_STEP_LAUNCH_MAX_PAIRS, OPT_MIXED_TIERS, OPT_BIG_EARLY_SETS, OPT_KCERT, OPT_KCERT_MIN, OPT_ACCUM_WAVE_MIN_TRIPS, OPT_FIRST_DIRECT, OPT_SUM_STEP, OPT_COUNT) = range(29)
+ OPT_FUSED_TGT_SETUP, OPT_STAGGER, OPT_STEP_LAUNCH_MAX_PAIRS, OPT_MIXED_TIERS, OPT_BIG_EARLY_SETS, OPT_KCERT, OPT_KCERT_MIN, OPT_ACCUM_WAVE_MIN_TRIPS, OPT_FIRST_DIRECT, OPT_SUM_STEP,
+ OPT_ACCUM_IN_CERT, OPT_COUNT) = range(30)
 
 POINT_DTYPE = np.dtype(
     {
diff --git a/mulls_amd/csrc/accum.h b/mulls_amd/csrc/accum.h
--- a/mulls_amd/csrc/accum.h
+++ b/mulls_amd/csrc/accum.h
@@ -341,6 +341,24 @@
 }
 }
 
+__device__ __forceinline__ double wave_trip_sum(double sum)
+{
+	sum = dpp_add_f64<0xB1>(sum);
+	sum = dpp_add_f64<0x4E>(sum);
+	sum = dpp_add_f64<0x141>(sum);
+	sum = dpp_add_f64<0x140>(sum);
+	sum = dpp_add_f64_rows<0x142, 0xa>(sum);
+	sum = dpp_add_f64_rows<0x143, 0xc>(sum);
+	return sum;
+}
+template <int NT, int MODE>
+__device__ __forceinline__ void wave_zero_missing(double *__restrict__ out)
+{
+	const int lane = (int)(threadIdx.x & 63u);
+	if (lane < MULLS_NTERM && !(MODE == 1 ? li_slot(lane) >= 0 : lane < NT))
+		out[lane] = 0.0;
+}
+
 template <typename TS, int T0, int NT, int MODE = 0, int LANES = MULLS_ACC_LANES>
 __device__ __forceinline__ void slot_terms(const AccumCtx &A, const double *x, bool valid, const float4 P, const float4 Q, const float4 N, float wi, float &wdg, TS *R)
 {
diff --git a/mulls_amd/csrc/batch.cpp b/mulls_amd/csrc/batch.cpp
--- a/mulls_amd/csrc/batch.cpp
+++ b/mulls_amd/csrc/batch.cpp
@@ -143,13 +143,14 @@
 	o[MULLS_OPT_SPLIT_MIN_PAIRS] = 96, o[MULLS_OPT_SPLIT_MAX_PAIRS] = 1 << 30, o[MULLS_OPT_FUSED_TGT_SETUP] = 1, o[MULLS_OPT_STAGGER] = 4352, o[MULLS_OPT_STEP_LAUNCH_MAX_PAIRS] = 640, o[MULLS_OPT_LDS_DEDUP] = 1, o[MULLS_OPT_GRID_H0] = 0, o[MULLS_OPT_BM_H0] = 0, o[MULLS_OPT_LEAN_STAGING] = 0, o[MULLS_OPT_DEBUG_STOP] = 0, o[MULLS_OPT_DEBUG_TICK] = 0, o[MULLS_OPT_MIXED_TIERS] = 1, o[MULLS_OPT_BIG_EARLY_SETS] = 5, o[MULLS_OPT_KCERT] = 1, o[MULLS_OPT_KCERT_MIN] = 64, o[MULLS_OPT_ACCUM_WAVE_MIN_TRIPS] = 768;
 	o[MULLS_OPT_FIRST_DIRECT] = 1;
 	o[MULLS_OPT_SUM_STEP] = 1;
+	o[MULLS_OPT_ACCUM_IN_CERT] = 1;
 	static const struct
 	{
 		const char *name;
 		int opt;
 	} env[] = {{"MULLS_HOST_STEP", MULLS_OPT_HOST_STEP}, {"MULLS_FEW_LAUNCHES_MAX_PAIRS", MULLS_OPT_FEW_LAUNCHES_MAX_PAIRS}, {"MULLS_SUBBATCHES", MULLS_OPT_SUBBATCHES}, {"MULLS_TWO_STREAMS", MULLS_OPT_TWO_STREAMS},
 			   {"MULLS_CERTIFICATES", MULLS_OPT_CERTIFICATES}, {"MULLS_LDS_DEDUP", MULLS_OPT_LDS_DEDUP}, {"MULLS_GRID_H0", MULLS_OPT_GRID_H0}, {"MULLS_BM_H0", MULLS_OPT_BM_H0},
-			   {"MULLS_LEAN_STAGING", MULLS_OPT_LEAN_STAGING}, {"MULLS_FUSED_TGT_SETUP", MULLS_OPT_FUSED_TGT_SETUP}, {"MULLS_STAGGER", MULLS_OPT_STAGGER}, {"MULLS_STEP_LAUNCH_MAX_PAIRS", MULLS_OPT_STEP_LAUNCH_MAX_PAIRS}, {"MULLS_SPLIT_MIN_PAIRS", MULLS_OPT_SPLIT_MIN_PAIRS}, {"MULLS_SPLIT_MAX_PAIRS", MULLS_OPT_SPLIT_MAX_PAIRS}, {"MULLS_DEBUG_STOP", MULLS_OPT_DEBUG_STOP}, {"MULLS_DEBUG_TICK", MULLS_OPT_DEBUG_TICK}, {"MULLS_MIXED_TIERS", MULLS_OPT_MIXED_TIERS}, {"MULLS_BIG_EARLY_SETS", MULLS_OPT_BIG_EARLY_SETS}, {"MULLS_KCERT", MULLS_OPT_KCERT}, {"MULLS_KCERT_MIN", MULLS_OPT_KCERT_MIN}, {"MULLS_ACCUM_WAVE_MIN_TRIPS", MULLS_OPT_ACCUM_WAVE_MIN_TRIPS}, {"MULLS_FIRST_DIRECT", MULLS_OPT_FIRST_DIRECT}, {"MULLS_SUM_STEP", MULLS_OPT_SUM_STEP}};
+			   {"MULLS_LEAN_STAGING", MULLS_OPT_LEAN_STAGING}, {"MULLS_FUSED_TGT_SETUP", MULLS_OPT_FUSED_TGT_SETUP}, {"MULLS_STAGGER", MULLS_OPT_STAGGER}, {"MULLS_STEP_LAUNCH_MAX_PAIRS", MULLS_OPT_STEP_LAUNCH_MAX_PAIRS}, {"MULLS_SPLIT_MIN_PAIRS", MULLS_OPT_SPLIT_MIN_PAIRS}, {"MULLS_SPLIT_MAX_PAIRS", MULLS_OPT_SPLIT_MAX_PAIRS}, {"MULLS_DEBUG_STOP", MULLS_OPT_DEBUG_STOP}, {"MULLS_DEBUG_TICK", MULLS_OPT_DEBUG_TICK}, {"MULLS_MIXED_TIERS", MULLS_OPT_MIXED_TIERS}, {"MULLS_BIG_EARLY_SETS", MULLS_OPT_BIG_EARLY_SETS}, {"MULLS_KCERT", MULLS_OPT_KCERT}, {"MULLS_KCERT_MIN", MULLS_OPT_KCERT_MIN}, {"MULLS_ACCUM_WAVE_MIN_TRIPS", MULLS_OPT_ACCUM_WAVE_MIN_TRIPS}, {"MULLS_FIRST_DIRECT", MULLS_OPT_FIRST_DIRECT}, {"MULLS_SUM_STEP", MULLS_OPT_SUM_STEP}, {"MULLS_ACCUM_IN_CERT", MULLS_OPT_ACCUM_IN_CERT}};
 	for (const auto &e : env)
 		if (const char *v = std::getenv(e.name))
 		{
diff --git a/mulls_amd/csrc/device_types.h b/mulls_amd/csrc/device_types.h
--- a/mulls_amd/csrc/device_types.h
+++ b/mulls_amd/csrc/device_types.h
@@ -68,6 +68,7 @@
 	uint32_t stage_fmt;
 	uint32_t tier;
 	uint32_t grid_slot;
+	uint32_t acc_epoch;
 };
 #define MULLS_STAGE_AOS48 0u
 #define MULLS_STAGE_PACK32 1u
diff --git a/mulls_amd/csrc/k_reduce.hip b/mulls_amd/csrc/k_reduce.hip
--- a/mulls_amd/csrc/k_reduce.hip
+++ b/mulls_amd/csrc/k_reduce.hip
@@ -17,6 +17,8 @@
 		return;
 	const CloudDesc *pd = descs + job.pair * MULLS_NC;
 	const bool residual_pass = ps.want_residual != 0;
+	if (!residual_pass && pd[job.cls].acc_epoch == rp.tick_base + (uint32_t)ps.iter && job.start < pd[job.cls].src_n)
+		return;
 	int cnt[MULLS_NC];
 	for (int c = 0; c < MULLS_NC; c++)
 		cnt[c] = (int)(class_called(rp, pd[c], c) ? pd[c].valid_next : pd[c].n_valid);
@@ -114,24 +116,11 @@
 		cur = nxt;
 #endif
 	}
-	if (NTW == NT && lane < MULLS_NTERM)
-	{
-		const bool has = MODE == 1 ? li_slot((int)lane) >= 0 : (int)lane < NT;
-		if (!has)
-			out[lane] = 0.0;
-	}
+	if (NTW == NT)
+		wave_zero_missing<NT, MODE>(out);
 #pragma unroll
 	for (int k = 0; k < NTW; k++)
-	{
-		double sum = acc[k];
-		sum = dpp_add_f64<0xB1>(sum);
-		sum = dpp_add_f64<0x4E>(sum);
-		sum = dpp_add_f64<0x141>(sum);
-		sum = dpp_add_f64<0x140>(sum);
-		sum = dpp_add_f64_rows<0x142, 0xa>(sum);
-		sum = dpp_add_f64_rows<0x143, 0xc>(sum);
-		acc[k] = sum;
-	}
+		acc[k] = wave_trip_sum(acc[k]);
 	if (lane == 63u)
 	{
 #pragma unroll
@@ -179,6 +168,8 @@
 			out[threadIdx.x & 63u] = 0.0;
 		return;
 	}
+	if (!residual_pass && d.acc_epoch == rp.tick_base + (uint32_t)ps.iter)
+		return;
 	if (residual_pass || A.metric == 1)
 	{
 		if (part)
diff --git a/mulls_amd/csrc/k_search.hip b/mulls_amd/csrc/k_search.hip
--- a/mulls_amd/csrc/k_search.hip
+++ b/mulls_amd/csrc/k_search.hip
@@ -223,15 +223,16 @@
 	return class_called(rp, d, cls);
 }
 
-template <int BLK, int SMALL, bool PARK = false, int FLAT_TRIPS = (BLK == 512 ? 3 : 2)>
+template <int BLK, int SMALL, bool PARK = false, int FLAT_TRIPS = (BLK == 512 ? 3 : 2), bool ACC = false>
 __device__ __forceinline__ bool cert_job(CertLds<SMALL> &CL, const RunParams &rp, const PairState &ps, const Job &job, CloudDesc &d, const GridDesc &g, uint32_t *W, float4 *__restrict__ spos,
 										  float4 *__restrict__ snrm, const uint32_t *__restrict__ cell_start, const float4 *__restrict__ tsorted, uint8_t *flag,
 										  int32_t *__restrict__ nn_idx, float *__restrict__ nn_d2, unsigned long long *__restrict__ winner, const float4 *__restrict__ tnrm,
 										  int32_t *__restrict__ match, float *__restrict__ wd, const float4 *__restrict__ tpos, int32_t *__restrict__ nn_hint,
-										  float4 *__restrict__ mq, uint32_t *park = nullptr)
+										  float4 *__restrict__ mq, uint32_t *park = nullptr, double *__restrict__ acc_partial = nullptr)
 {
 	const bool flat = rp.lds_dedup != 0u && rp.debug_stop != 9u && job.start == 0u && job.count >= d.src_n && d.src_n <= (uint32_t)(BLK * FLAT_TRIPS) && class_called(rp, d, job.cls);
-	return flat ? cert_class_flat<BLK, FLAT_TRIPS, true, SMALL, PARK>(CL, rp, ps, job, d, g, W, spos, snrm, cell_start, tsorted, flag, nn_idx, nn_d2, winner, tnrm, match, wd, tpos, nn_hint, mq, park)
+	return flat ? cert_class_flat<BLK, FLAT_TRIPS, true, SMALL, PARK, ACC>(CL, rp, ps, job, d, g, W, spos, snrm, cell_start, tsorted, flag, nn_idx, nn_d2, winner, tnrm, match, wd, tpos, nn_hint,
+																			mq, park, acc_partial)
 				: cert_class<BLK, true, SMALL>(CL, rp, ps, job, d, g, W, spos, snrm, cell_start, tsorted, flag, nn_idx, nn_d2, winner, tnrm, match, wd, tpos, nn_hint, mq);
 }
 
@@ -243,7 +244,7 @@
 															int32_t *__restrict__ nn_idx, float *__restrict__ nn_d2, unsigned long long *__restrict__ winner,
 															const float4 *__restrict__ tnrm, int32_t *__restrict__ match, float *__restrict__ wd,
 															const float4 *__restrict__ tpos, int32_t *__restrict__ nn_hint, float4 *__restrict__ mq,
-															uint32_t *__restrict__ wl, uint32_t *__restrict__ wl_ctr, uint32_t parity)
+															uint32_t *__restrict__ wl, uint32_t *__restrict__ wl_ctr, uint32_t parity, double *__restrict__ acc_partial)
 {
 	extern __shared__ __attribute__((aligned(16))) unsigned char lds_raw[];
 	uint32_t *W = reinterpret_cast<uint32_t *>(lds_raw);
@@ -257,8 +258,9 @@
 	const GridDesc g = grids[job.pair * MULLS_NC + job.cls];
 	__shared__ CertLds<SMALL> s_cert;
 	constexpr bool PARK = BLK == 512;
-	__shared__ uint32_t s_park[PARK ? 2 * TRIPS * BLK : 1];
-	if (!cert_job<BLK, SMALL, PARK, TRIPS>(s_cert, rp, ps, job, d, g, W, spos, snrm, cell_start, tsorted, flag, nn_idx, nn_d2, winner, tnrm, match, wd, tpos, nn_hint, mq, s_park))
+	__shared__ __attribute__((aligned(16))) uint32_t s_park[PARK ? 2 * TRIPS * BLK : 1];
+	if (!cert_job<BLK, SMALL, PARK, TRIPS, PARK>(s_cert, rp, ps, job, d, g, W, spos, snrm, cell_start, tsorted, flag, nn_idx, nn_d2, winner, tnrm, match, wd, tpos, nn_hint, mq, s_park,
+												  acc_partial))
 		if (threadIdx.x == 0)
 			wl[atomicAdd(&wl_ctr[2u * parity], 1u)] = blockIdx.x;
 }
@@ -529,7 +531,7 @@
 int launch_nn_lds(hipStream_t st, uint32_t njobs, const Job *jobs, CloudDesc *descs, const PairState *states, const RunParams &rp, float4 *spos,
 				  float4 *snrm, const GridDesc *grids, const uint32_t *cell_start, const float4 *tsorted, uint8_t *flag, int32_t *nn_idx,
 				  float *nn_d2, unsigned long long *winner, const float4 *tnrm, int32_t *match, float *wd, const float4 *tpos, int32_t *nn_hint, float4 *mq, uint32_t cap, uint32_t maxcells,
-				  uint32_t *wl, uint32_t *wl_ctr, uint32_t parity, bool first)
+				  uint32_t *wl, uint32_t *wl_ctr, uint32_t parity, bool first, double *acc_partial)
 {
 	const DevLaunch D = dev_launch<0>([](DevLaunch &d) {
 		if (hipFuncSetAttribute(reinterpret_cast<const void *>(k_nn_lds), hipFuncAttributeMaxDynamicSharedMemorySize, 160 * 1024) != hipSuccess)
@@ -564,13 +566,13 @@
 		;
 	else if (njobs <= 2u * n_cu)
 		hipLaunchKernelGGL(k_cert<1024>, dim3(njobs), dim3(1024), dedup ? ((size_t)cap * 2u + 3u) & ~(size_t)3 : 0u, st, jobs, descs, states, rp, spos, snrm, grids, cell_start, tsorted,
-						   flag, nn_idx, nn_d2, winner, tnrm, match, wd, tpos, nn_hint, mq, wl, wl_ctr, parity & 1u);
+						   flag, nn_idx, nn_d2, winner, tnrm, match, wd, tpos, nn_hint, mq, wl, wl_ctr, parity & 1u, nullptr);
 	else if (dedup && MULLS_CERT_BLOCK == 512 && D.dyn_max[1] && (((size_t)cap * 2u + 3u) & ~(size_t)3) + D.dyn_max[1] <= 40u * 1024u)
 		hipLaunchKernelGGL((k_cert<MULLS_CERT_BLOCK, 3, 768>), dim3(njobs), dim3(MULLS_CERT_BLOCK), ((size_t)cap * 2u + 3u) & ~(size_t)3, st, jobs, descs, states, rp, spos, snrm, grids,
-						   cell_start, tsorted, flag, nn_idx, nn_d2, winner, tnrm, match, wd, tpos, nn_hint, mq, wl, wl_ctr, parity & 1u);
+						   cell_start, tsorted, flag, nn_idx, nn_d2, winner, tnrm, match, wd, tpos, nn_hint, mq, wl, wl_ctr, parity & 1u, acc_partial);
 	else
 		hipLaunchKernelGGL(k_cert<MULLS_CERT_BLOCK>, dim3(njobs), dim3(MULLS_CERT_BLOCK), dedup ? ((size_t)cap * 2u + 3u) & ~(size_t)3 : 0u, st, jobs, descs, states, rp, spos, snrm, grids,
-						   cell_start, tsorted, flag, nn_idx, nn_d2, winner, tnrm, match, wd, tpos, nn_hint, mq, wl, wl_ctr, parity & 1u);
+						   cell_start, tsorted, flag, nn_idx, nn_d2, winner, tnrm, match, wd, tpos, nn_hint, mq, wl, wl_ctr, parity & 1u, acc_partial);
 	hipLaunchKernelGGL(k_nn_lds, dim3(njobs < n_cu ? njobs : n_cu), dim3(MULLS_LDS_BLOCK), nn_lds_bytes(cap, maxcells, dedup), st, jobs, descs, states, rp, spos, snrm,
 					   grids, cell_start, tsorted, flag, nn_idx, nn_d2, winner, tnrm, match, wd, tpos, nn_hint, mq, cap, wl, wl_ctr, parity & 1u, first ? njobs : 0u);
 	return 0;
diff --git a/mulls_amd/csrc/launch.h b/mulls_amd/csrc/launch.h
--- a/mulls_amd/csrc/launch.h
+++ b/mulls_amd/csrc/launch.h
@@ -53,7 +53,7 @@
 int launch_nn_lds(hipStream_t st, uint32_t njobs, const Job *jobs, CloudDesc *descs, const PairState *states, const RunParams &rp, float4 *spos,
 				  float4 *snrm, const GridDesc *grids, const uint32_t *cell_start, const float4 *tsorted, uint8_t *flag, int32_t *nn_idx,
 				  float *nn_d2, unsigned long long *winner, const float4 *tnrm, int32_t *match, float *wd, const float4 *tpos, int32_t *nn_hint, float4 *mq, uint32_t cap, uint32_t maxcells,
-				  uint32_t *wl, uint32_t *wl_ctr, uint32_t parity, bool first = false);
+				  uint32_t *wl, uint32_t *wl_ctr, uint32_t parity, bool first = false, double *acc_partial = nullptr);
 int launch_cert_mixed(hipStream_t st, uint32_t n_lds, const Job *cjobs, uint32_t n_big, const Job *bjobs, uint32_t max_wgs, uint32_t rounds, CloudDesc *descs, const PairState *states,
 					  const RunParams &rp, float4 *spos, float4 *snrm, const GridDesc *grids, const uint32_t *cell_start, const unsigned long long *bm, const uint32_t *pf,
 					  const uint32_t *cs, const float4 *tsorted, uint8_t *flag, int32_t *nn_idx, float *nn_d2, unsigned long long *winner, const float4 *tnrm, int32_t *match,
diff --git a/mulls_amd/csrc/lds_tier.h b/mulls_amd/csrc/lds_tier.h
--- a/mulls_amd/csrc/lds_tier.h
+++ b/mulls_amd/csrc/lds_tier.h
@@ -1,5 +1,6 @@
 #pragma once
 #include "device_util.h"
+#include "accum.h"
 struct FilterCtx
 {
 	bool gate, any_match, normal_check, dedup_done, strict;
@@ -998,12 +999,136 @@
 	return true;
 }
 
-template <int BLK, int TRIPS, bool W16, int SMALL, bool PARK = false>
+#ifndef MULLS_CERT_ACC_SUB
+#define MULLS_CERT_ACC_SUB 3
+#endif
+template <int BLK, int SMALL, typename TS, int MODE, int METRIC, int W0, int WN>
+__device__ __forceinline__ TS *cert_accum_buf(uint32_t *park, float4 *uq, int kk)
+{
+	constexpr int WP = (int)(2u * 3u * BLK * 4u / (BLK * sizeof(TS)));
+	return kk < WP ? reinterpret_cast<TS *>(park) + kk * BLK : reinterpret_cast<TS *>(uq) + (kk - WP) * BLK;
+}
+template <int BLK, int SMALL, typename TS, int MODE, int METRIC, int W0, int WN, int S0>
+__device__ __forceinline__ void cert_accum_eval(const AccumCtx &A, const float4 P, const float4 Q, const float4 N, float wi, float wpre, uint32_t *park, float4 *uq)
+{
+	constexpr int SUB = sizeof(TS) == 8 ? (MULLS_CERT_ACC_SUB + 1) / 2 : MULLS_CERT_ACC_SUB;
+	constexpr int SN = WN - S0 < SUB ? WN - S0 : SUB;
+	TS t[SN];
+#pragma unroll
+	for (int kk = 0; kk < SN; kk++)
+		t[kk] = (TS)0;
+	float wdg = wpre;
+	point_terms<TS, W0 + S0, SN, MODE, METRIC>(A, nullptr, P, Q, N, wi, wdg, t, &wpre);
+#pragma unroll
+	for (int kk = 0; kk < SN; kk++)
+		cert_accum_buf<BLK, SMALL, TS, MODE, METRIC, W0, WN>(park, uq, S0 + kk)[threadIdx.x] = t[kk];
+	if constexpr (S0 + SN < WN)
+		cert_accum_eval<BLK, SMALL, TS, MODE, METRIC, W0, WN, S0 + SN>(A, P, Q, N, wi, wpre, park, uq);
+}
+template <int BLK, int SMALL, typename TS, int NT, int MODE, int METRIC, int W0>
+__device__ __forceinline__ void cert_accum_window(const AccumCtx &A, bool valid, const float4 P, const float4 Q, const float4 N, float wi, float wpre, uint32_t *park,
+												  float4 *uq, uint32_t cm, double *acc)
+{
+	constexpr int NW = BLK / 64;
+	constexpr int WP = (int)(2u * 3u * BLK * 4u / (BLK * sizeof(TS))), WQ = (int)((size_t)SMALL * 16u / (BLK * sizeof(TS)));
+	constexpr int WN = NT - W0 < WP + WQ ? NT - W0 : WP + WQ;
+	__syncthreads();
+	if (valid)
+		cert_accum_eval<BLK, SMALL, TS, MODE, METRIC, W0, WN, 0>(A, P, Q, N, wi, wpre, park, uq);
+	__syncthreads();
+	const uint32_t lane = threadIdx.x & 63u, wave = (uint32_t)__builtin_amdgcn_readfirstlane((int)(threadIdx.x >> 6));
+#pragma unroll
+	for (int kk = 0; kk < WN; kk++)
+		if ((W0 + kk) % NW == (int)wave)
+		{
+			const TS *r = cert_accum_buf<BLK, SMALL, TS, MODE, METRIC, W0, WN>(park, uq, kk) + lane;
+			double a = acc[(W0 + kk) / NW];
+#pragma unroll
+			for (int i = 0; i < NW; i++)
+				if ((cm >> i) & 1u)
+					a += (double)r[64 * i];
+			acc[(W0 + kk) / NW] = a;
+		}
+	if constexpr (W0 + WN < NT)
+		cert_accum_window<BLK, SMALL, TS, NT, MODE, METRIC, W0 + WN>(A, valid, P, Q, N, wi, wpre, park, uq, cm, acc);
+}
+template <int BLK, int TRIPS, int SMALL, typename TS, int NT, int MODE, int METRIC>
+__device__ __forceinline__ void cert_accum(CertLds<SMALL> &CL, uint32_t *park, const AccumCtx &A, const CloudDesc &d, uint32_t vbits, const float4 *__restrict__ spos,
+										   const float4 *__restrict__ mq, float *__restrict__ wd, double *__restrict__ partial)
+{
+	constexpr int NW = BLK / 64, NA = (NT + NW - 1) / NW;
+	static_assert(BLK == 512 && TRIPS == 3, "two walk trips per accumulation trip; park holds 2 * TRIPS * BLK words");
+	static_assert(BLK <= 4 * SMALL && TRIPS * NW <= 32, "a byte per lane fits the leftover list's indices; a chain's bits fit a word");
+	const uint32_t lane = threadIdx.x & 63u, wave = (uint32_t)__builtin_amdgcn_readfirstlane((int)(threadIdx.x >> 6));
+	uint8_t *vb = reinterpret_cast<uint8_t *>(CL.us);
+	vb[threadIdx.x] = (uint8_t)vbits;
+	__syncthreads();
+	uint32_t cm = 0;
+#pragma unroll
+	for (int i = 0; i < NW; i++)
+	{
+		const uint32_t v = vb[64 * i + lane];
+#pragma unroll
+		for (int k = 0; k < TRIPS; k++)
+			cm |= ((v >> k) & 1u) << (k * NW + i);
+	}
+	const bool writes_w = METRIC != 2 || !A.faithful;
+	const uint32_t n_k = (d.src_n + (uint32_t)BLK - 1u) / (uint32_t)BLK;
+	double acc[NA];
+#pragma unroll
+	for (int a = 0; a < NA; a++)
+		acc[a] = -0.0;
+#pragma unroll
+	for (uint32_t k = 0; k < (uint32_t)TRIPS; k++)
+	{
+		if (k >= n_k)
+			break;
+		const bool valid = (vbits >> k) & 1u;
+		const uint32_t gi = d.src_off + threadIdx.x + k * (uint32_t)BLK;
+		float4 P = make_float4(0.0f, 0.0f, 0.0f, 0.0f), Q = P, N = P;
+		float wi = 1.0f, wpre = 0.0f;
+		if (valid)
+		{
+			P = spos[gi];
+			Q = mq[2u * gi];
+			const float3 n3 = *reinterpret_cast<const float3 *>(mq + 2u * gi + 1u);
+			N = make_float4(n3.x, n3.y, n3.z, 0.0f);
+			wi = A.inten_w ? point_wi(P, Q) : 1.0f;
+			wpre = corr_weight(A, METRIC, P, Q, N, wi);
+			if (writes_w)
+				wd[gi] = wpre;
+		}
+		cert_accum_window<BLK, SMALL, TS, NT, MODE, METRIC, 0>(A, valid, P, Q, N, wi, wpre, park, CL.uq, cm >> (k * NW), acc);
+		if ((k & 1u) || k + 1u == n_k)
+		{
+			double *out = partial + (size_t)(d.job_begin + 2u * (k >> 1)) * MULLS_NTERM;
+			if (wave == 0u)
+				wave_zero_missing<NT, MODE>(out);
+#pragma unroll
+			for (int a = 0; a < NA; a++)
+				if (a * NW + (int)wave < NT)
+					acc[a] = wave_trip_sum(acc[a]);
+			if (lane == 63u)
+			{
+#pragma unroll
+				for (int a = 0; a < NA; a++)
+					if (a * NW + (int)wave < NT)
+						out[MODE == 1 ? li_term(a * NW + (int)wave) : a * NW + (int)wave] = acc[a];
+			}
+#pragma unroll
+			for (int a = 0; a < NA; a++)
+				acc[a] = -0.0;
+		}
+	}
+}
+
+template <int BLK, int TRIPS, bool W16, int SMALL, bool PARK = false, bool ACC = false>
 __device__ __forceinline__ bool cert_class_flat(CertLds<SMALL> &CL, const RunParams &rp, const PairState &ps, const Job &job, CloudDesc &d, const GridDesc &g, uint32_t *W,
 												 float4 *__restrict__ spos, float4 *__restrict__ snrm, const uint32_t *__restrict__ cell_start,
 												 const float4 *__restrict__ tsorted, uint8_t *flag, int32_t *__restrict__ nn_idx, float *__restrict__ nn_d2,
 												 unsigned long long *__restrict__ winner, const float4 *__restrict__ tnrm, int32_t *__restrict__ match,
-												 float *__restrict__ wd, const float4 *__restrict__ tpos, int32_t *__restrict__ nn_hint, float4 *__restrict__ mq, uint32_t *park = nullptr)
+												 float *__restrict__ wd, const float4 *__restrict__ tpos, int32_t *__restrict__ nn_hint, float4 *__restrict__ mq, uint32_t *park = nullptr,
+												 double *__restrict__ acc_partial = nullptr)
 {
 	float4 *uq = CL.uq;
 	uint32_t *us = CL.us, *red = CL.red;
@@ -1237,7 +1362,7 @@
 
 	const float thr = ps.thr[job.cls], max_sqr = thr * thr;
 	const bool any_match = total_matched > 0u, strict = rp.rej_strict != 0;
-	uint32_t n_alive = 0, n_valid = 0;
+	uint32_t n_alive = 0, n_valid = 0, vbits = 0;
 #pragma unroll
 	for (int k = 0; k < TRIPS; k++)
 	{
@@ -1301,6 +1426,7 @@
 			flag[gi] = (uint8_t)nf;
 		n_alive += alive ? 1u : 0u;
 		n_valid += valid ? 1u : 0u;
+		vbits |= (valid ? 1u : 0u) << k;
 	}
 	for (int off = 32; off > 0; off >>= 1)
 	{
@@ -1326,6 +1452,18 @@
 		d.valid_next = tv;
 		d.n_search = U;
 	}
+	const int metric = metric_of(job.cls);
+	if constexpr (ACC)
+		if (acc_partial && !ps.want_residual && !rp.force_class_w && !(rp.w_balance && (job.cls == 0 || job.cls == 4)) && metric != 1)
+		{
+			if (threadIdx.x == 0)
+				d.acc_epoch = C.epoch;
+			const AccumCtx A = accum_ctx(rp, job.cls, ps.iter, false, 1.0f);
+			if (metric == 0)
+				cert_accum<BLK, TRIPS, SMALL, float, 27, 0, 0>(CL, park, A, d, vbits, spos, mq, wd, acc_partial);
+			else
+				cert_accum<BLK, TRIPS, SMALL, float, 27, 0, 2>(CL, park, A, d, vbits, spos, mq, wd, acc_partial);
+		}
 	FLAT_TICK(4)
 	if (rp.dbg_ticks && threadIdx.x == 0)
 		atomicAdd(&rp.dbg_ticks[6], 1ull);
diff --git a/mulls_amd/csrc/loop.cpp b/mulls_amd/csrc/loop.cpp
--- a/mulls_amd/csrc/loop.cpp
+++ b/mulls_amd/csrc/loop.cpp
@@ -216,7 +216,8 @@
 											rp.grid_maxcells, first) != 0;
 	if (!together && L.cjob_n &&
 		launch_nn_lds(sst, L.cjob_n, B->cjobs + L.cjob_lo, B->descs, B->states, rp, B->spos, B->snrm, B->grids, B->cell_start, B->tsorted, B->flag, B->nn_idx, B->nn_d2, B->winner,
-					  B->tnrm, B->match, B->wd, B->tpos, B->nn_hint, B->mq, lds_cap, rp.grid_maxcells, wl, wl_ctr, parity, first) != 0)
+					  B->tnrm, B->match, B->wd, B->tpos, B->nn_hint, B->mq, lds_cap, rp.grid_maxcells, wl, wl_ctr, parity, first,
+					  ctx->opt[MULLS_OPT_ACCUM_IN_CERT] != 0.0 ? B->partial : nullptr) != 0)
 	{
 		ctx->err = "could not raise the dynamic LDS limit of k_nn_lds";
 		return MULLS_E_HIP;
```

Result: no change. 268,500 (median of 5 runs) (-0.5%).
